# castacks/mvs_gi

Measured on AMD Instinct MI355X. Metric: stereo frames/sec/GPU (G16V, 3-cam, D=16) + inv-dist L1 vs reference, higher is better.
Workload: dtype f16x3 (split-fp16 MFMA operands: 11 + 11 significant bits, f32 accumulate/activations)

## Files before the change

### include/mvsgi.h

```cpp
#ifndef MVSGI_H
#define MVSGI_H

#include <stddef.h>
#include <stdint.h>

#ifdef __cplusplus
extern "C" {
#endif

#define MVSGI_ABI_VERSION 8

typedef void* mvsgi_stream_t;

#define MVSGI_CONV_AUTO   0
#define MVSGI_CONV_DIRECT 1
#define MVSGI_CONV_MFMA   2
#define MVSGI_CONV_BF16X3 3
#define MVSGI_CONV_BF16X3_C16 4
#define MVSGI_CONV_BF16X3_V32 5
#define MVSGI_CONV_BF16X3_D32 6

#define MVSGI_CONV_F16 0x100

#define MVSGI_SPLIT_F16 1
// ... 69 lines not shown
size_t mvsgi_conv2d_packed_weight_bytes_bf16x3(int Cout, int Cin);
int mvsgi_conv2d_pack_weights_bf16x3(const float* w_oihw, void* w_packed, int Cout, int Cin,
                                     mvsgi_stream_t stream);
int mvsgi_conv2d_f32(const float* x, const float* w_oihw, const void* w_packed,
                     const float* scale, const float* shift, const float* res, float* y,
                     int B, int Cin, int Hin, int Win, int Cout, int ksize, int stride,
                     float neg_slope, int impl, int in_nchw, mvsgi_stream_t stream);
const char* mvsgi_conv2d_variant_f32(int Cin, int Cout, int ksize, int stride, int impl, int in_nchw);

int mvsgi_resize_trilinear_f32(const float* x, float* y, int B, int C,
                               int Di, int Hi, int Wi, int Do, int Ho, int Wo,
                               mvsgi_stream_t stream);

int mvsgi_softargmin_f32(const float* costs, const float* inv_idx, float* inv_dist,
                         float* norm_costs, int B, int D, int H, int W, int scale,
                         mvsgi_stream_t stream);

int mvsgi_softargmin_div_f32(const float* costs, const float* inv_idx, float* inv_dist,
                             float* norm_costs, int B, int D, int H, int W, int scale,
                             float post_div, mvsgi_stream_t stream);

#define MVSGI_SA_AUTO  0
#define MVSGI_SA_PIXEL 1
#define MVSGI_SA_BAND  2
int mvsgi_softargmin_scaled_f32(const float* costs, const float* inv_idx, float* inv_dist,
                                float* norm_costs, int B, int D, int H, int W, double scale,
                                int OH, int OW, float post_div, int variant, mvsgi_stream_t stream);

int mvsgi_confidence_f32(const float* costs, const float* inv_idx, float* max_prob, float* entropy,
                         float* spread, int* argmax, int B, int D, int H, int W, double scale,
                         int OH, int OW, float post_div, int normalize_entropy, mvsgi_stream_t stream);

int mvsgi_ncv_to_nvc_f32(const float* x, float* y, int B, int C, long long V, mvsgi_stream_t stream);
int mvsgi_nvc_to_ncv_f32(const float* x, float* y, int B, int C, long long V, mvsgi_stream_t stream);

int mvsgi_resblock2d_f32(const float* x, const void* w_packed1, const float* scale1, const float* shift1,
                         const void* w_packed2, const float* scale2, const float* shift2, float* y,
                         int N, int H, int W, float neg_slope, mvsgi_stream_t stream);

size_t mvsgi_split2d_bytes(int N, int H, int W);
int mvsgi_f32_to_split2d(const float* x, void* y_split, int N, int H, int W, mvsgi_stream_t stream);
int mvsgi_split2d_to_f32(const void* x_split, float* y, int N, int H, int W, mvsgi_stream_t stream);
size_t mvsgi_resblock2d_split_packed_weight_bytes(void);
int mvsgi_resblock2d_split_pack_weights(const float* w_oihw, const float* scale, void* w_packed, mvsgi_stream_t stream);
int mvsgi_resblock2d_split(const void* x_split, const void* w_packed1, const float* shift1,
                           const void* w_packed2, const float* shift2, void* y, int y_is_split,
                           int N, int H, int W, float neg_slope, mvsgi_stream_t stream);
int mvsgi_conv2d_s2_split(const void* x_split, const void* w_packed, const float* shift, void* y_split,
                          int N, int H, int W, float neg_slope, mvsgi_stream_t stream);
int mvsgi_conv2d_f32_out_split2d(const float* x, const float* w_oihw, const void* w_packed,
                                 const float* scale, const float* shift, const float* res, void* y_split,
                                 int B, int Cin, int Hin, int Win, int Cout, int ksize, int stride,
                                 float neg_slope, int impl, int in_nchw, mvsgi_stream_t stream);

int mvsgi_rays_panorama_f32(const float* dist, float* rays, int N, int H, int W,
                            float lat0, float lat1, float lon0, float lon1, mvsgi_stream_t stream);
int mvsgi_transform_points_f32(const float* T , const float* points, float* out,
                               int B, long long M, mvsgi_stream_t stream);
int mvsgi_grid_double_sphere_f32(const float* points, float* grid, unsigned char* mask, int B, long long M,
                                 float xi, float alpha, float fx, float fy, float cx, float cy,
                                 int calib_h, int calib_w, float w2, mvsgi_stream_t stream);
int mvsgi_grid_equirect_f32(const float* points, float* grid, int B, long long M, mvsgi_stream_t stream);
int mvsgi_rays_equirect_surrogate_f32(float* rays, int H, int W, mvsgi_stream_t stream);

int mvsgi_resample_bilinear_u8_f32(const unsigned char* imgs, const float* grid, const unsigned char* valid, float* out,
                                   long long M, int T, int Hr, int Wr, int H, int W, float invalid_value, mvsgi_stream_t stream);
int mvsgi_resample_bilinear_f32(const float* imgs, const float* grid, const unsigned char* valid, float* out, long long M, int T,
                                int C, int Hr, int Wr, int H, int W, float invalid_value, mvsgi_stream_t stream);
int mvsgi_resample_validity_u8(const float* grid, const unsigned char* ds_mask, unsigned char* valid, long long n,
                               mvsgi_stream_t stream);
int mvsgi_resample_u8_table_f32(float* table256);

int mvsgi_reproject_f32(const float* inv, const float* rays, const void* imgs, int img_kind, const float* T_host,
                        const float* cams_host, float* xyz, float* warped, unsigned char* valid, float* grid,
                        long long B, int N, int C, int Hr, int Wr, int H, int W, float bf, float invalid_value,
                        mvsgi_stream_t stream);

int mvsgi_deform_conv2d_pack_weights_f32(const float* w_oihw, float* w_packed, int Cout, int Cin, int Kh, int Kw,
                                         mvsgi_stream_t stream);
int mvsgi_deform_conv2d_f32(const float* x, const float* offset, int offset_per_image, const float* w_packed,
                            const float* scale, const float* shift, const float* res, float* y,
                            int N, int Cin, int H, int W, int Cout, int Kh, int Kw, int stride_h, int stride_w,
                            int pad_h, int pad_w, int dil_h, int dil_w, float neg_slope, mvsgi_stream_t stream);

int mvsgi_sweep_std_nhwc_valid_split(const float* feats, const float* grids, const unsigned char* vmask,
                                     void* vol_split, int B, int N, int C, int Hi, int Wi, int D, int Ho, int Wo,
                                     int rig_batch, mvsgi_stream_t stream);

int mvsgi_conv3d_f32_out_split(const float* x, const float* w_packed_b3, const float* scale, const float* shift,
                               const float* res, void* y_split, int B, int Cin, int Din, int Hin, int Win, int Cout,
                               int stride, float neg_slope, mvsgi_stream_t stream);
int mvsgi_conv3d_rs16_split(const void* x_split, const void* w_packed_rs, const float* scale, const float* shift, float* y,
                            int B, int D, int H, int W, float neg_slope, mvsgi_stream_t stream);
int mvsgi_conv3d_rs16_split_out_split(const void* x_split, const void* w_packed_rs, const float* scale, const float* shift,
                                      void* y_split, int B, int D, int H, int W, float neg_slope, mvsgi_stream_t stream);
size_t mvsgi_conv3d_s2rs_packed_weight_bytes(void);
int mvsgi_conv3d_s2rs_pack_weights(const float* w_oidhw, const float* scale, void* w_packed, mvsgi_stream_t stream);
int mvsgi_conv3d_s2rs(const void* x_split, const void* w_packed, const float* shift, void* y_split,
                      int B, int D, int H, int W, float neg_slope, mvsgi_stream_t stream);
size_t mvsgi_conv3d_rs_packed_weight_bytes(int Cout, int Cin);
int mvsgi_conv3d_rs_pack_weights(const float* w_oidhw, void* w_packed, int Cout, int Cin, mvsgi_stream_t stream);
size_t mvsgi_act_split_bytes(int B, int C, int D, int H, int W);
int mvsgi_act_f32_to_split(const float* x, void* y_split, int B, int C, int D, int H, int W, mvsgi_stream_t stream);
int mvsgi_act_split_to_f32(const void* x_split, float* y, int B, int C, int D, int H, int W, mvsgi_stream_t stream);
int mvsgi_conv3d_rs_split(const void* x_split, const void* w_packed_rs, const float* scale, const float* shift,
                          const void* res_split, void* y, int y_is_f32, int B, int Cin, int D, int H, int W, int Cout,
                          float neg_slope, mvsgi_stream_t stream);

int mvsgi_conv3d_up2_f32_out_split(const float* x, const void* w_packed, int w_layout, const float* scale, const float* shift,
                                   const float* res, void* y_split, int B, int Cin, int Dl, int Hl, int Wl, int Cout,
                                   float neg_slope, mvsgi_stream_t stream);
int mvsgi_conv3d_up2_poly_split(const void* x_split, const void* plan_dev, const float* scale, const float* shift, void* y_split,
                                int B, int D, int H, int W, float neg_slope, mvsgi_stream_t stream);
size_t mvsgi_conv3d_head_split_packed_weight_bytes(int Cin);
int mvsgi_conv3d_head_split_pack_weights(const float* w_oidhw, void* w_packed, int Cin, mvsgi_stream_t stream);
int mvsgi_conv3d_head_split(const void* x_split, const void* w_packed, float scale, float shift, float* y, int B, int Cin,
                            int D, int H, int W, float neg_slope, mvsgi_stream_t stream);
int mvsgi_conv3d_head_split_pack_weights_f16(const float* w_oidhw, void* w_packed, int Cin, mvsgi_stream_t stream);
int mvsgi_conv3d_head_split_f16(const void* x_split, const void* w_packed, float scale, float shift, float* y, int B, int Cin,
                            int D, int H, int W, float neg_slope, mvsgi_stream_t stream);
int mvsgi_conv3d_up2_poly_rec32(const void* x_split, const void* plan_dev, const float* scale, const float* shift, void* y_rec32,
                                int B, int D, int H, int W, float neg_slope, mvsgi_stream_t stream);
int mvsgi_conv3d_head_rec32_f16(const void* x_rec32, const void* w_packed, float scale, float shift, float* y, int B, int Cin,
                                int D, int H, int W, float neg_slope, mvsgi_stream_t stream);
size_t mvsgi_conv3d_up2_poly_plan_bytes(int D, int H, int W);
int mvsgi_conv3d_up2_poly_plan(const float* w_oidhw_host, void* plan_host, int D, int H, int W);
int mvsgi_conv3d_up2_poly_f32(const void* x_split, const void* plan_dev, const float* scale, const float* shift, float* y,
                              int B, int D, int H, int W, float neg_slope, mvsgi_stream_t stream);

int mvsgi_act_f32_to_split_fmt(const float* x, void* y_split, int B, int C, int D, int H, int W, int fmt, mvsgi_stream_t stream);
int mvsgi_act_split_to_f32_fmt(const void* x_split, float* y, int B, int C, int D, int H, int W, int fmt, mvsgi_stream_t stream);
int mvsgi_sweep_std_nhwc_valid_split_fmt(const float* feats, const float* grids, const unsigned char* vmask, void* vol_split,
                                         int B, int N, int C, int Hi, int Wi, int D, int Ho, int Wo, int rig_batch, int fmt,
                                         mvsgi_stream_t stream);
int mvsgi_conv3d_f32_out_split_fmt(const float* x, const float* w_packed_b3, const float* scale, const float* shift,
                                   const float* res, void* y_split, int B, int Cin, int Din, int Hin, int Win, int Cout,
                                   int stride, float neg_slope, int fmt, mvsgi_stream_t stream);
int mvsgi_conv3d_rs_pack_weights_fmt(const float* w_oidhw, void* w_packed, int Cout, int Cin, int fmt, mvsgi_stream_t stream);
int mvsgi_conv3d_rs_split_fmt(const void* x_split, const void* w_packed_rs, const float* scale, const float* shift,
                              const void* res_split, void* y, int y_is_f32, int B, int Cin, int D, int H, int W, int Cout,
                              float neg_slope, int fmt, mvsgi_stream_t stream);
int mvsgi_conv3d_rs16_split_fmt(const void* x_split, const void* w_packed_rs, const float* scale, const float* shift, void* y,
                                int y_is_split, int B, int D, int H, int W, float neg_slope, int fmt, mvsgi_stream_t stream);
int mvsgi_conv3d_s2rs_pack_weights_fmt(const float* w_oidhw, const float* scale, void* w_packed, int fmt, mvsgi_stream_t stream);
int mvsgi_conv3d_s2rs_fmt(const void* x_split, const void* w_packed, const float* shift, void* y_split, int B, int D, int H, int W,
                          float neg_slope, float unscale, int fmt, mvsgi_stream_t stream);
int mvsgi_conv3d_s2rs_out_fmt(const void* x_split, const void* w_packed, const float* shift, void* y_split, int B, int D, int H, int W,
                              float neg_slope, float unscale, int fmt, int y_f32p, mvsgi_stream_t stream);
int mvsgi_conv3d_up2_poly_plan_fmt(const float* w_oidhw_host, void* plan_host, int D, int H, int W, int fmt);
int mvsgi_conv3d_up2_poly_fmt(const void* x_split, const void* plan_dev, const float* scale, const float* shift, void* y,
                              int y_is_split, int B, int D, int H, int W, float neg_slope, int fmt, mvsgi_stream_t stream);
int mvsgi_conv3d_up2_poly_wino_pays(int B, int D, int H, int W);

size_t mvsgi_conv3d_wino32_packed_weight_bytes(void);
int mvsgi_conv3d_wino32_applies(int Cin, int Cout, int D, int H, int W, int stride, float neg_slope);
int mvsgi_conv3d_wino32_pack_weights(const float* w_oidhw, void* w_packed, float* unscale, mvsgi_stream_t stream);
int mvsgi_conv3d_wino32_f16(const void* x_split, const void* w_packed, const float* scale, const float* shift, const void* res_split,
                            void* y, int y_is_f32, int act_f32p, int B, int D, int H, int W, float neg_slope, mvsgi_stream_t stream);

size_t mvsgi_instance_norm_ws_bytes(int B, int S, int C);
int mvsgi_instance_norm_f32(const float* x, const float* res, const float* gamma, const float* beta, float* y, float* ws,
                            int B, int S, int C, float eps, float neg_slope, mvsgi_stream_t stream);

#define MVSGI_METRICS_MASK_NONE   0
#define MVSGI_METRICS_MASK_TENSOR 1
#define MVSGI_METRICS_MASK_RANGE  2
#define MVSGI_METRICS_RANGE_FRAME 0
#define MVSGI_METRICS_RANGE_BATCH 1
size_t mvsgi_metrics_ws_bytes(int B, int H, int W);
int mvsgi_metrics_f32(const float* preds, const float* target, const unsigned char* mask, int mask_kind, float lo, float hi,
                      float bf, float cmin, float cmax, float thresh, float thresh_dist, int range_scope, void* ws,
                      size_t ws_bytes, double* out, int B, int H, int W, mvsgi_stream_t stream);

#define MVSGI_LOSSES_P_NONE       0
#define MVSGI_LOSSES_P_GIVEN      1
#define MVSGI_LOSSES_P_FUSED      2
#define MVSGI_LOSSES_VOL_NONE     0
#define MVSGI_LOSSES_VOL_PIXEL    1
#define MVSGI_LOSSES_VOL_VOLUME   2
#define MVSGI_LOSSES_PX_NONE      0
#define MVSGI_LOSSES_PX_TENSOR    1
#define MVSGI_LOSSES_PX_LABEL_MAX 2
size_t mvsgi_losses_ws_bytes(int B, int OH, int OW);
int mvsgi_losses_f32(const float* labels, const float* pred, const float* probs, int p_kind, const float* inv_list,
                     const unsigned char* vol_mask, int vol_kind, const unsigned char* px_mask, int px_kind, float label_max,
                     int inbounds, float near_inv, float far_inv, float* true_cost, void* ws, size_t ws_bytes, double* out,
                     int B, int D, int H, int W, double scale, int OH, int OW, mvsgi_stream_t stream);

size_t mvsgi_cloud_ws_bytes(long long B, int H, int W);
int mvsgi_cloud_pack_f32(const float* inv, const float* rays, const unsigned char* mask, int mask_per_frame,
                         const float* const* gates_host, const float* gate_lo_host, const float* gate_hi_host, int n_gates,
                         const float* warped, const unsigned char* valid, int N, int C, int require_colour, float no_colour,
                         const float* const* attrs_host, int A, float* points, int* counts, int* index, long long capacity,
                         void* ws, size_t ws_bytes, long long B, int H, int W, int sy, int sx, float bf, float d_min, float d_max,
                         mvsgi_stream_t stream);

size_t mvsgi_photo_ws_bytes(long long B, int H, int W);
int mvsgi_photo_consistency_f32(const float* inv, const float* rays, const void* imgs, int img_kind, const float* cam_masks,
                                const float* T_host, const float* cams_host, const unsigned char* mask, int mask_per_frame,
                                float thresh, unsigned char* n_views, float* photo_var, float* photo_std, float* mean_colour,
                                void* ws, size_t ws_bytes, double* table, long long B, int N, int C, int Hr, int Wr, int H, int W,
                                float bf, mvsgi_stream_t stream);
int mvsgi_photo_consistency_seen_f32(const float* inv, const float* rays, const void* imgs, int img_kind, const float* cam_masks,
                                     const float* T_host, const float* cams_host, const unsigned char* mask, int mask_per_frame,
                                     float thresh, unsigned char* n_views, float* photo_var, float* photo_std, float* mean_colour,
                                     void* ws, size_t ws_bytes, double* table, long long B, int N, int C, int Hr, int Wr, int H, int W,
                                     float bf, const unsigned char* cam_seen, mvsgi_stream_t stream);

int mvsgi_camera_range_f32(const float* inv, const float* rays, const float* T_host, const float* cams_host, const unsigned char* mask,
                           int mask_per_frame, int footprint, float* z2, long long B, int N, int H, int W, int Hz, int Wz, float bf,
                           mvsgi_stream_t stream);
int mvsgi_visibility_f32(const float* inv, const float* rays, const float* T_host, const float* cams_host, const float* z2, float k2,
                         unsigned char* visible, unsigned char* n_visible, float* range, long long B, int N, int H, int W, int Hz,
                         int Wz, float bf, mvsgi_stream_t stream);

int mvsgi_temporal_splat_f32(const float* prev_inv, const unsigned char* prev_age, const float* rays, const float* T,
                             unsigned long long* zkey, long long B, int H, int W, float bf, float au, float bu, float av, float bv,
                             int wrap, mvsgi_stream_t stream);
int mvsgi_temporal_fuse_f32(const unsigned long long* zkey, const float* prev_inv, const float* prev_var,
                            const unsigned char* prev_age, const float* cur_inv, const float* cur_std, float meas_std, float* fused,
                            float* var, unsigned char* age, float* warped_inv, float* warped_var, int* src, long long B, int H, int W,
                            float bf, float gate2, float q_var, mvsgi_stream_t stream);

int mvsgi_tsdf_integrate_f32(float* vol, const float* inv, const float* std, const unsigned char* mask, const float* T,
                             const int* origin, const int* origin_prev, float* range, long long B, int Nx, int Ny, int Nz, int H,
                             int W, float vs, float trunc, float t2, float w_max, float r_min, float r_max, float bf, float au,
                             float bu, float av, float bv, int wrap, mvsgi_stream_t stream);
int mvsgi_tsdf_raycast_f32(const float* vol, const float* rays, const float* P, const int* origin, float* inv, float* weight,
                           int* steps, long long B, int Nx, int Ny, int Nz, int H, int W, float inv_vs, float t0, float step, int K,
                           float w_min, float bf, mvsgi_stream_t stream);

#ifdef __cplusplus
}
#endif
#endif
```

### mvs_gi_amd/_lib.py

```python
from __future__ import annotations

import ctypes
import os
from ctypes import c_char_p, c_double, c_float, c_int, c_longlong, c_size_t, c_void_p

_HERE = os.path.dirname(os.path.abspath(__file__))
LIB_PATH = os.environ.get("MVSGI_LIB", os.path.join(_HERE, "libmvsgi_hip.so"))

ABI_VERSION = 8


class MvsgiLibraryMissing(RuntimeError):
    pass


_P = c_void_p
SIGNATURES = {
    "mvsgi_abi_version": (c_int, []),
    "mvsgi_last_error": (c_char_p, []),
    "mvsgi_saturation_flags": (c_int, [c_int, _P]),
    "mvsgi_saturation_words": (c_int, [_P]),
    "mvsgi_sweep_max_cams": (c_int, []),
    "mvsgi_sweep_std_f32": (c_int, [_P, _P, _P, c_int, _P, _P] + [c_int] * 10 + [_P]),
    "mvsgi_sweep_cat_f32": (c_int, [_P, _P, _P] + [c_int] * 8 + [_P]),
    "mvsgi_sweep_std_nhwc_f32": (c_int, [_P, _P, _P, c_int, _P, _P] + [c_int] * 10 + [_P]),
    "mvsgi_sweep_cat_nhwc_f32": (c_int, [_P, _P, _P] + [c_int] * 8 + [_P]),
    "mvsgi_sweep_validity_u8": (c_int, [_P, _P, c_int, _P, _P] + [c_int] * 7 + [_P]),
    "mvsgi_sweep_std_nhwc_valid_f32": (c_int, [_P, _P, _P, _P] + [c_int] * 8 + [_P]),
    "mvsgi_sweep_std_nhwc_valid_split": (c_int, [_P, _P, _P, _P] + [c_int] * 9 + [_P]),
    "mvsgi_sweep_std_nhwc_valid_rig_f32": (c_int, [_P, _P, _P, _P] + [c_int] * 8 + [_P]),
    "mvsgi_conv3d_packed_weight_floats": (c_size_t, [c_int, c_int]),
    "mvsgi_conv3d_pack_weights_f32": (c_int, [_P, _P, c_int, c_int, _P]),
    "mvsgi_conv3d_packed_weight_bytes_bf16x3": (c_size_t, [c_int, c_int]),
    "mvsgi_conv3d_pack_weights_bf16x3": (c_int, [_P, _P, c_int, c_int, _P]),
    "mvsgi_conv3d_pack_weights_split": (c_int, [_P, _P, c_int, c_int, c_int, _P]),
    "mvsgi_conv3d_f32": (c_int, [_P] * 7 + [c_int] * 7 + [c_float, c_int, _P]),
    "mvsgi_conv3d_variant_f32": (c_char_p, [c_int] * 8),
    "mvsgi_conv3d_up2_f32": (c_int, [_P, _P, c_int] + [_P] * 4 + [c_int] * 6 + [c_float, _P]),
    "mvsgi_conv3d_up2_variant_f32": (c_char_p, [c_int] * 7),
    "mvsgi_conv3d_v32_applies": (c_int, [c_int] * 7),
    "mvsgi_conv3d_d32_applies": (c_int, [c_int] * 7),
    "mvsgi_conv3d_up2_d32_applies": (c_int, [c_int] * 6),
    "mvsgi_conv3d_packed_weight_bytes_bf16x3_v32": (c_size_t, [c_int, c_int]),
    "mvsgi_conv3d_pack_weights_bf16x3_v32": (c_int, [_P, _P, c_int, c_int, _P]),
    "mvsgi_conv3d_packed_weight_bytes_bf16x3_c16": (c_size_t, [c_int]),
    "mvsgi_conv3d_pack_weights_bf16x3_c16": (c_int, [_P, _P, c_int, _P]),
    "mvsgi_conv2d_stem_packed_weight_bytes": (c_size_t, []),
    "mvsgi_conv2d_stem_pack_weights": (c_int, [_P, _P, _P]),
    "mvsgi_conv2d_packed_weight_floats": (c_size_t, [c_int, c_int]),
    "mvsgi_conv2d_pack_weights_f32": (c_int, [_P, _P, c_int, c_int, _P]),
    "mvsgi_conv2d_packed_weight_bytes_bf16x3": (c_size_t, [c_int, c_int]),
    "mvsgi_conv2d_pack_weights_bf16x3": (c_int, [_P, _P, c_int, c_int, _P]),
    "mvsgi_conv2d_f32": (c_int, [_P] * 7 + [c_int] * 7 + [c_float, c_int, c_int, _P]),
    "mvsgi_conv2d_variant_f32": (c_char_p, [c_int] * 6),
    "mvsgi_resblock2d_f32": (c_int, [_P] * 8 + [c_int] * 3 + [c_float, _P]),
    "mvsgi_split2d_bytes": (c_size_t, [c_int] * 3),
    "mvsgi_f32_to_split2d": (c_int, [_P, _P] + [c_int] * 3 + [_P]),
    "mvsgi_split2d_to_f32": (c_int, [_P, _P] + [c_int] * 3 + [_P]),
    "mvsgi_resblock2d_split_packed_weight_bytes": (c_size_t, []),
    "mvsgi_resblock2d_split_pack_weights": (c_int, [_P, _P, _P, _P]),
    "mvsgi_resblock2d_split": (c_int, [_P] * 6 + [c_int] * 4 + [c_float, _P]),
    "mvsgi_conv2d_s2_split": (c_int, [_P] * 4 + [c_int] * 3 + [c_float, _P]),
    "mvsgi_conv2d_f32_out_split2d": (c_int, [_P] * 7 + [c_int] * 7 + [c_float, c_int, c_int, _P]),
    "mvsgi_resize_trilinear_f32": (c_int, [_P, _P] + [c_int] * 8 + [_P]),
    "mvsgi_softargmin_f32": (c_int, [_P, _P, _P, _P] + [c_int] * 5 + [_P]),
    "mvsgi_softargmin_div_f32": (c_int, [_P, _P, _P, _P] + [c_int] * 5 + [c_float, _P]),
    "mvsgi_softargmin_scaled_f32": (c_int, [_P, _P, _P, _P] + [c_int] * 4 + [c_double, c_int, c_int, c_float, c_int, _P]),
    "mvsgi_confidence_f32": (c_int, [_P] * 6 + [c_int] * 4 + [c_double, c_int, c_int, c_float, c_int, _P]),
    "mvsgi_rays_panorama_f32": (c_int, [_P, _P, c_int, c_int, c_int] + [c_float] * 4 + [_P]),
    "mvsgi_transform_points_f32": (c_int, [_P, _P, _P, c_int, c_longlong, _P]),
    "mvsgi_grid_double_sphere_f32": (c_int, [_P, _P, _P, c_int, c_longlong] + [c_float] * 6 + [c_int, c_int, c_float, _P]),
    "mvsgi_grid_equirect_f32": (c_int, [_P, _P, c_int, c_longlong, _P]),
    "mvsgi_rays_equirect_surrogate_f32": (c_int, [_P, c_int, c_int, _P]),
    "mvsgi_resample_bilinear_u8_f32": (c_int, [_P, _P, _P, _P, c_longlong] + [c_int] * 5 + [c_float, _P]),
    "mvsgi_resample_bilinear_f32": (c_int, [_P, _P, _P, _P, c_longlong] + [c_int] * 6 + [c_float, _P]),
    "mvsgi_resample_validity_u8": (c_int, [_P, _P, _P, c_longlong, _P]),
    "mvsgi_resample_u8_table_f32": (c_int, [_P]),
    "mvsgi_reproject_f32": (c_int, [_P, _P, _P, c_int] + [_P] * 6 + [c_longlong] + [c_int] * 6 + [c_float, c_float, _P]),
    "mvsgi_deform_conv2d_pack_weights_f32": (c_int, [_P, _P] + [c_int] * 4 + [_P]),
    "mvsgi_deform_conv2d_f32": (c_int, [_P, _P, c_int] + [_P] * 5 + [c_int] * 13 + [c_float, _P]),
    "mvsgi_act_split_bytes": (c_size_t, [c_int] * 5),
    "mvsgi_act_f32_to_split": (c_int, [_P, _P] + [c_int] * 5 + [_P]),
    "mvsgi_act_split_to_f32": (c_int, [_P, _P] + [c_int] * 5 + [_P]),
    "mvsgi_conv3d_f32_out_split": (c_int, [_P] * 6 + [c_int] * 7 + [c_float, _P]),
    "mvsgi_conv3d_rs16_split": (c_int, [_P] * 5 + [c_int] * 4 + [c_float, _P]),
    "mvsgi_conv3d_rs16_split_out_split": (c_int, [_P] * 5 + [c_int] * 4 + [c_float, _P]),
    "mvsgi_conv3d_s2rs_packed_weight_bytes": (c_size_t, []),
    "mvsgi_conv3d_s2rs_pack_weights": (c_int, [_P, _P, _P, _P]),
    "mvsgi_conv3d_s2rs": (c_int, [_P] * 4 + [c_int] * 4 + [c_float, _P]),
    "mvsgi_conv3d_rs_packed_weight_bytes": (c_size_t, [c_int, c_int]),
    "mvsgi_conv3d_rs_pack_weights": (c_int, [_P, _P, c_int, c_int, _P]),
    "mvsgi_conv3d_rs_split": (c_int, [_P] * 6 + [c_int] * 7 + [c_float, _P]),
    "mvsgi_conv3d_up2_f32_out_split": (c_int, [_P, _P, c_int] + [_P] * 4 + [c_int] * 6 + [c_float, _P]),
    "mvsgi_conv3d_up2_poly_split": (c_int, [_P] * 5 + [c_int] * 4 + [c_float, _P]),
    "mvsgi_conv3d_head_split_packed_weight_bytes": (c_size_t, [c_int]),
    "mvsgi_conv3d_head_split_pack_weights": (c_int, [_P, _P, c_int, _P]),
    "mvsgi_conv3d_head_split": (c_int, [_P, _P, c_float, c_float, _P] + [c_int] * 5 + [c_float, _P]),
    "mvsgi_conv3d_head_split_pack_weights_f16": (c_int, [_P, _P, c_int, _P]),
    "mvsgi_conv3d_head_split_f16": (c_int, [_P, _P, c_float, c_float, _P] + [c_int] * 5 + [c_float, _P]),
    "mvsgi_conv3d_head_rec32_f16": (c_int, [_P, _P, c_float, c_float, _P] + [c_int] * 5 + [c_float, _P]),
    "mvsgi_conv3d_up2_poly_rec32": (c_int, [_P] * 5 + [c_int] * 4 + [c_float, _P]),
    "mvsgi_conv3d_up2_poly_plan_bytes": (c_size_t, [c_int] * 3),
    "mvsgi_conv3d_up2_poly_plan": (c_int, [_P, _P] + [c_int] * 3),
    "mvsgi_conv3d_up2_poly_f32": (c_int, [_P] * 5 + [c_int] * 4 + [c_float, _P]),
    "mvsgi_act_f32_to_split_fmt": (c_int, [_P, _P] + [c_int] * 6 + [_P]),
    "mvsgi_act_split_to_f32_fmt": (c_int, [_P, _P] + [c_int] * 6 + [_P]),
    "mvsgi_sweep_std_nhwc_valid_split_fmt": (c_int, [_P, _P, _P, _P] + [c_int] * 10 + [_P]),
    "mvsgi_conv3d_f32_out_split_fmt": (c_int, [_P] * 6 + [c_int] * 7 + [c_float, c_int, _P]),
    "mvsgi_conv3d_rs_pack_weights_fmt": (c_int, [_P, _P, c_int, c_int, c_int, _P]),
    "mvsgi_conv3d_rs_split_fmt": (c_int, [_P] * 6 + [c_int] * 7 + [c_float, c_int, _P]),
    "mvsgi_conv3d_rs16_split_fmt": (c_int, [_P] * 5 + [c_int] * 5 + [c_float, c_int, _P]),
    "mvsgi_conv3d_s2rs_pack_weights_fmt": (c_int, [_P, _P, _P, c_int, _P]),
    "mvsgi_conv3d_s2rs_fmt": (c_int, [_P] * 4 + [c_int] * 4 + [c_float, c_float, c_int, _P]),
    "mvsgi_conv3d_s2rs_out_fmt": (c_int, [_P] * 4 + [c_int] * 4 + [c_float, c_float, c_int, c_int, _P]),
    "mvsgi_conv3d_up2_poly_plan_fmt": (c_int, [_P, _P] + [c_int] * 4),
    "mvsgi_conv3d_wino32_packed_weight_bytes": (c_size_t, []),
    "mvsgi_conv3d_wino32_applies": (c_int, [c_int] * 6 + [c_float]),
    "mvsgi_conv3d_wino32_pack_weights": (c_int, [_P] * 4),
    "mvsgi_conv3d_wino32_f16": (c_int, [_P] * 6 + [c_int] * 6 + [c_float, _P]),
    "mvsgi_conv3d_up2_poly_fmt": (c_int, [_P] * 5 + [c_int] * 5 + [c_float, c_int, _P]),
    "mvsgi_conv3d_up2_poly_wino_pays": (c_int, [c_int] * 4),
    "mvsgi_ncv_to_nvc_f32": (c_int, [_P, _P, c_int, c_int, c_longlong, _P]),
    "mvsgi_nvc_to_ncv_f32": (c_int, [_P, _P, c_int, c_int, c_longlong, _P]),
    "mvsgi_instance_norm_ws_bytes": (c_size_t, [c_int] * 3),
    "mvsgi_instance_norm_f32": (c_int, [_P] * 6 + [c_int] * 3 + [c_float, c_float, _P]),
    "mvsgi_metrics_ws_bytes": (c_size_t, [c_int] * 3),
    "mvsgi_metrics_f32": (c_int, [_P, _P, _P, c_int] + [c_float] * 7 + [c_int, _P, c_size_t, _P] + [c_int] * 3 + [_P]),
    "mvsgi_losses_ws_bytes": (c_size_t, [c_int] * 3),
    "mvsgi_losses_f32": (c_int, [_P, _P, _P, c_int, _P, _P, c_int, _P, c_int, c_float, c_int, c_float, c_float, _P, _P, c_size_t, _P] +
                         [c_int] * 4 + [c_double, c_int, c_int, _P]),
    "mvsgi_cloud_ws_bytes": (c_size_t, [c_longlong, c_int, c_int]),
    "mvsgi_cloud_pack_f32": (c_int, [_P, _P, _P, c_int, _P, _P, _P, c_int, _P, _P, c_int, c_int, c_int, c_float, _P, c_int, _P, _P, _P,
                                     c_longlong, _P, c_size_t, c_longlong] + [c_int] * 4 + [c_float] * 3 + [_P]),
    "mvsgi_photo_ws_bytes": (c_size_t, [c_longlong, c_int, c_int]),
    "mvsgi_photo_consistency_f32": (c_int, [_P, _P, _P, c_int, _P, _P, _P, _P, c_int, c_float, _P, _P, _P, _P, _P, c_size_t, _P,
                                            c_longlong] + [c_int] * 6 + [c_float, _P]),
    "mvsgi_photo_consistency_seen_f32": (c_int, [_P, _P, _P, c_int, _P, _P, _P, _P, c_int, c_float, _P, _P, _P, _P, _P, c_size_t, _P,
                                                 c_longlong] + [c_int] * 6 + [c_float, _P, _P]),
    "mvsgi_camera_range_f32": (c_int, [_P] * 5 + [c_int, c_int, _P, c_longlong] + [c_int] * 5 + [c_float, _P]),
    "mvsgi_visibility_f32": (c_int, [_P] * 5 + [c_float, _P, _P, _P, c_longlong] + [c_int] * 5 + [c_float, _P]),
    "mvsgi_temporal_splat_f32": (c_int, [_P] * 5 + [c_longlong, c_int, c_int] + [c_float] * 5 + [c_int, _P]),
    "mvsgi_temporal_fuse_f32": (c_int, [_P] * 6 + [c_float] + [_P] * 6 + [c_longlong, c_int, c_int] + [c_float] * 3 + [_P]),
    "mvsgi_tsdf_integrate_f32": (c_int, [_P] * 8 + [c_longlong] + [c_int] * 5 + [c_float] * 11 + [c_int, _P]),
    "mvsgi_tsdf_raycast_f32": (c_int, [_P] * 7 + [c_longlong] + [c_int] * 5 + [c_float] * 3 + [c_int, c_float, c_float, _P]),
}

_lib = None


def load() -> ctypes.CDLL:
    global _lib
    if _lib is not None:
        return _lib
    if not os.path.isfile(LIB_PATH):
        raise MvsgiLibraryMissing(
            f"{LIB_PATH} not found: build the HIP library first (__graft_entry__.build()). "
            "mvs_gi_amd has no CPU fallback.")
    import torch
    lib = ctypes.CDLL(LIB_PATH)
    try:
        lib.mvsgi_abi_version.restype = c_int
        lib.mvsgi_abi_version.argtypes = []
        got = lib.mvsgi_abi_version()
    except AttributeError as e:
        raise MvsgiLibraryMissing(f"{LIB_PATH}: not a libmvsgi_hip ({e}); rebuild it (__graft_entry__.build())") from None
    if got != ABI_VERSION:
        raise MvsgiLibraryMissing(f"{LIB_PATH}: ABI version {got}, expected {ABI_VERSION}; rebuild it (__graft_entry__.build())")
    for name, (res, args) in SIGNATURES.items():
        try:
            fn = getattr(lib, name)
        except AttributeError:
            raise MvsgiLibraryMissing(f"{LIB_PATH}: symbol {name} missing although the ABI version matches; rebuild it "
                                      "(__graft_entry__.build())") from None
        fn.restype = res
        fn.argtypes = args
    lib.mvsgi_saturation_flags(0, None)
    _lib = lib
    return lib


def check(status: int, what: str) -> None:
    if status != 0:
        msg = load().mvsgi_last_error()
        raise RuntimeError(f"{what}: {msg.decode() if msg else 'unknown error'}")
```

### mvs_gi_amd/csrc/common.hpp

```cpp
#pragma once
#include <hip/hip_runtime.h>

#include <cstdarg>
#include <cstdio>
#include <cstdlib>
#include <cstring>
#include <string>

#include "../../include/mvsgi.h"

namespace mvsgi {

std::string& last_error_ref();

inline int fail(const char* fmt, ...) {
    char buf[512];
    va_list ap;
    va_start(ap, fmt);
    vsnprintf(buf, sizeof(buf), fmt, ap);
    va_end(ap);
    last_error_ref() = buf;
    return 1;
}

inline int check_launch(const char* what) {
    hipError_t e = hipGetLastError();
    if (e != hipSuccess) return fail("%s: launch failed: %s", what, hipGetErrorString(e));
    return 0;
}

#define MVSGI_REQUIRE(cond, ...)                      \
    do {                                              \
        if (!(cond)) return ::mvsgi::fail(__VA_ARGS__); \
    } while (0)

constexpr int kSatWords = 8;
unsigned* sat_words();
#define MVSGI_SAT_WORDS(VAR)                                                            \
    unsigned* VAR = ::mvsgi::sat_words();                                               \
    MVSGI_REQUIRE(VAR != nullptr, "cannot allocate the range report's pinned host words")

inline hipStream_t as_stream(mvsgi_stream_t s) { return reinterpret_cast<hipStream_t>(s); }

inline long long cdiv(long long a, long long b) { return (a + b - 1) / b; }

inline bool aligned(const void* p, unsigned a) { return (reinterpret_cast<uintptr_t>(p) & (a - 1)) == 0; }

constexpr int kMaxCams = 8;

constexpr int kMaxDevices = 32;
struct PersistentGeom {
    int wgs_per_cu;
    int cus;
};
template <class K>
inline int persistent_geometry(K kern, int threads, size_t lds_bytes, int max_wgs_per_cu,
                               PersistentGeom (&cache)[kMaxDevices], const char* what, PersistentGeom& out) {
    int dev = 0;
    hipError_t e = hipGetDevice(&dev);
    if (e != hipSuccess) return fail("%s: hipGetDevice: %s", what, hipGetErrorString(e));
    if (dev < 0 || dev >= kMaxDevices) return fail("%s: device ordinal %d not supported (max %d)", what, dev, kMaxDevices);
    PersistentGeom g = cache[dev];
    if (!g.wgs_per_cu) {
        e = hipFuncSetAttribute(reinterpret_cast<const void*>(kern), hipFuncAttributeMaxDynamicSharedMemorySize,
                                (int)lds_bytes);
        if (e != hipSuccess) return fail("%s: hipFuncSetAttribute: %s", what, hipGetErrorString(e));
        int occ = 0;
        e = hipOccupancyMaxActiveBlocksPerMultiprocessor(&occ, kern, threads, lds_bytes);
        if (e != hipSuccess || occ < 1) occ = 1;
        int cus = 0;
        e = hipDeviceGetAttribute(&cus, hipDeviceAttributeMultiprocessorCount, dev);
        if (e != hipSuccess || cus < 1) return fail("%s: cannot read the device's CU count", what);
        g.wgs_per_cu = occ > max_wgs_per_cu ? max_wgs_per_cu : occ;
        g.cus = cus;
        cache[dev] = g;
    }
    out = g;
    return 0;
}
inline unsigned persistent_grid(const PersistentGeom& geo, long long nb) {
    long long resident = ((long long)geo.cus * geo.wgs_per_cu) / 8 * 8;
    if (resident < 8) resident = 8;
    return (unsigned)(nb <= resident ? nb : resident);
}
template <class K, class A>
inline int launch_persistent(K kern, int threads, size_t lds_bytes, int max_wgs_per_cu, PersistentGeom (&cache)[kMaxDevices],
                             const char* what, long long nb, hipStream_t st, const A& args) {
    PersistentGeom geo;
    if (persistent_geometry(kern, threads, lds_bytes, max_wgs_per_cu, cache, what, geo)) return 1;
    hipLaunchKernelGGL(kern, dim3(persistent_grid(geo, nb)), dim3((unsigned)threads), lds_bytes, st, args);
    return check_launch(what);
}

inline int device_cus() {
    static int cache[kMaxDevices] = {};
    int dev = 0;
    if (hipGetDevice(&dev) != hipSuccess || dev < 0 || dev >= kMaxDevices) return 256;
    if (!cache[dev]) {
        int cus = 0;
        if (hipDeviceGetAttribute(&cus, hipDeviceAttributeMultiprocessorCount, dev) != hipSuccess || cus < 1) cus = 256;
        cache[dev] = cus;
    }
    return cache[dev];
}

constexpr size_t kRs32PackedBytes = (size_t)2 * 2 * 14 * 2 * 64 * 16;
void rs32_pack_weights_host(const float* w_oidhw_32x32x27, void* packed, bool f16);
int rs32_up2_launch(const void* x_split, const void* w_sets, const float* scale32, const float* shift32, void* y, int y_is_split,
                    int B, int D, int H, int W, float neg_slope, bool f16, hipStream_t st);

constexpr size_t kWinoUp2RoleBytes = (size_t)4 * 4 * 3 * 2 * 2 * 64 * 16;
void wino_up2_pack_role(const float* w32_oidhw, unsigned short* wp, float* unscale32);
bool wino_up2_applies(int D, int H, int W);
int wino_up2_launch(const void* x_split, const void* w_roles, const float* unw, const float* scale16, const float* shift16, void* y_split,
                    int B, int D, int H, int W, float neg_slope, bool out_f32, hipStream_t st);

}
```

### mvs_gi_amd/csrc/conv3d.hip

```cpp
#include "common.hpp"
#include "conv_common.hpp"
#include "conv3d_variants.hpp"
#ifdef MVSGI_STAMPS
#include <cstdio>
#include <cstdlib>
#endif

namespace {

__global__ void pack_head_weights_kernel(const float* __restrict__ w, float* __restrict__ wp, int Cin) {
    const int idx = blockIdx.x * 256 + threadIdx.x;
    if (idx >= 27 * Cin) return;
    const int tap = idx / Cin, ci = idx % Cin;
    wp[idx] = w[ci * 27 + tap];
}

#include "conv3d_f32mfma.hpp"
#include "conv3d_bf16x3.hpp"


__global__ __launch_bounds__(256) void conv3d_head_kernel(ConvArgs a, int dchunk, int nd) {
    constexpr int TH = 8, TW = 32, ITH = TH + 2, ITW = TW + 2, PV = ITH * ITW;
    constexpr int NT = (PV + 31) / 32;
    constexpr int TPW = (NT + 3) / 4;
// ... 528 lines not shown
extern "C" int mvsgi_conv3d_d32_applies(int B, int Cin, int Din, int Hin, int Win, int Cout, int stride) {
    ConvArgs a{};
    static const float dummy = 0.f;
    if (fill_args(a, &dummy, &dummy, &dummy, &dummy, &dummy, nullptr, nullptr, B, Cin, Din, Hin, Win, Cout, stride, 1.f))
        return 0;
    return d32_variant(a) != V_COUNT ? 1 : 0;
}

extern "C" int mvsgi_conv3d_v32_applies(int B, int Cin, int Din, int Hin, int Win, int Cout, int stride) {
    ConvArgs a{};
    static const float dummy = 0.f;
    if (fill_args(a, &dummy, &dummy, &dummy, &dummy, &dummy, nullptr, nullptr, B, Cin, Din, Hin, Win, Cout, stride, 1.f))
        return 0;
    return v32_applies(a) ? 1 : 0;
}

extern "C" size_t mvsgi_conv3d_packed_weight_bytes_bf16x3_c16(int Cin) { return (size_t)(Cin / 16) * 5 * 3 * 2 * 64 * 16; }

extern "C" int mvsgi_conv3d_pack_weights_bf16x3_c16(const float* w_oidhw, void* w_packed, int Cin, mvsgi_stream_t stream) {
    MVSGI_REQUIRE(w_oidhw && w_packed, "mvsgi_conv3d_pack_weights_bf16x3_c16: null pointer");
    MVSGI_REQUIRE(Cin > 0 && Cin % 16 == 0, "mvsgi_conv3d_pack_weights_bf16x3_c16: Cin=%d must be a positive multiple of 16", Cin);
    const int total = (Cin / 16) * 5 * 3 * 64;
    hipLaunchKernelGGL(pack_weights_bf16x3_c16_kernel, dim3((unsigned)mvsgi::cdiv(total, 256)), dim3(256), 0,
                       mvsgi::as_stream(stream), w_oidhw, reinterpret_cast<bf16x8*>(w_packed), Cin, false);
    return mvsgi::check_launch("mvsgi_conv3d_pack_weights_bf16x3_c16");
}

extern "C" int mvsgi_conv3d_pack_weights_f32(const float* w_oidhw, float* w_packed, int Cout, int Cin,
                                             mvsgi_stream_t stream) {
    MVSGI_REQUIRE(w_oidhw && w_packed, "mvsgi_conv3d_pack_weights_f32: null pointer");
    if (Cout == 1 && Cin > 0 && Cin % 16 == 0) {
        hipLaunchKernelGGL(pack_head_weights_kernel, dim3((unsigned)mvsgi::cdiv(27 * Cin, 256)), dim3(256), 0,
                           mvsgi::as_stream(stream), w_oidhw, w_packed, Cin);
        return mvsgi::check_launch("mvsgi_conv3d_pack_weights_f32");
    }
    MVSGI_REQUIRE(Cout > 0 && Cin > 0 && Cout % 16 == 0 && Cin % 16 == 0,
                  "mvsgi_conv3d_pack_weights_f32: Cout=%d Cin=%d must be positive multiples of 16 (or Cout == 1)",
                  Cout, Cin);
    const long long total = (long long)(Cin / 16) * 27 * (Cout / 16) * 64;
    hipLaunchKernelGGL(pack_weights_kernel, dim3((unsigned)mvsgi::cdiv(total, 256)), dim3(256), 0,
                       mvsgi::as_stream(stream), w_oidhw, reinterpret_cast<f32x4*>(w_packed), Cout, Cin, 27);
    return mvsgi::check_launch("mvsgi_conv3d_pack_weights_f32");
}

extern "C" int mvsgi_conv3d_f32(const float* x, const float* w_oidhw, const float* w_packed, const float* scale,
                                const float* shift, const float* res, float* y, int B, int Cin, int Din, int Hin,
                                int Win, int Cout, int stride, float neg_slope, int impl, mvsgi_stream_t stream) {
    MVSGI_REQUIRE(x && y && scale && shift, "mvsgi_conv3d_f32: null pointer");
    ConvArgs a{};
    if (fill_args(a, x, w_oidhw, w_packed, scale, shift, res, y, B, Cin, Din, Hin, Win, Cout, stride, neg_slope))
        return 1;
    if (split_flag(a, impl, "mvsgi_conv3d_f32")) return 1;
    const int v = select_variant(a, impl);
    if (v == V_COUNT) return 1;
    return launch_variant(v, a, mvsgi::as_stream(stream));
}

extern "C" int mvsgi_conv3d_f32_out_split_fmt(const float* x, const float* w_packed_b3, const float* scale, const float* shift,
                                              const float* res, void* y_split, int B, int Cin, int Din, int Hin, int Win, int Cout,
                                              int stride, float neg_slope, int fmt, mvsgi_stream_t stream) {
    MVSGI_REQUIRE(fmt == 0 || fmt == MVSGI_SPLIT_F16, "mvsgi_conv3d_f32_out_split: fmt %d not in {0, MVSGI_SPLIT_F16}", fmt);
    MVSGI_REQUIRE(x && y_split && scale && shift && w_packed_b3, "mvsgi_conv3d_f32_out_split: null pointer");
    MVSGI_REQUIRE(Cin % 16 == 0 && Cout % 16 == 0, "mvsgi_conv3d_f32_out_split: Cin, Cout must be multiples of 16");
    ConvArgs a{};
    if (fill_args(a, x, nullptr, w_packed_b3, scale, shift, res, reinterpret_cast<float*>(y_split), B, Cin, Din, Hin, Win, Cout,
                  stride, neg_slope))
        return 1;
    a.y_split = static_cast<unsigned char*>(y_split);
    a.f16 = fmt != 0;
    const int v = select_variant(a, MVSGI_CONV_BF16X3);
    if (v == V_COUNT) return 1;
    return launch_variant(v, a, mvsgi::as_stream(stream));
}
extern "C" int mvsgi_conv3d_f32_out_split(const float* x, const float* w_packed_b3, const float* scale, const float* shift,
                                          const float* res, void* y_split, int B, int Cin, int Din, int Hin, int Win, int Cout,
                                          int stride, float neg_slope, mvsgi_stream_t stream) {
    return mvsgi_conv3d_f32_out_split_fmt(x, w_packed_b3, scale, shift, res, y_split, B, Cin, Din, Hin, Win, Cout, stride, neg_slope, 0, stream);
}

extern "C" const char* mvsgi_conv3d_variant_f32(int B, int Cin, int Din, int Hin, int Win, int Cout, int stride,
                                                int impl) {
    ConvArgs a{};
    static const float dummy = 0.f;
    if (fill_args(a, &dummy, &dummy, &dummy, &dummy, &dummy, nullptr, nullptr, B, Cin, Din, Hin, Win, Cout, stride,
                  1.f))
        return nullptr;
    if (split_flag(a, impl, "mvsgi_conv3d_variant_f32")) return nullptr;
    const int v = select_variant(a, impl);
    return variant_name(v, a);
}

extern "C" int mvsgi_conv3d_up2_f32(const float* x, const void* w_packed, int w_layout, const float* scale,
                                    const float* shift, const float* res, float* y, int B, int Cin, int Dl, int Hl,
                                    int Wl, int Cout, float neg_slope, mvsgi_stream_t stream) {
    const bool f16 = (w_layout & MVSGI_CONV_F16) != 0;
    w_layout &= ~MVSGI_CONV_F16;
    MVSGI_REQUIRE(w_layout == MVSGI_CONV_BF16X3 || (w_layout == MVSGI_CONV_BF16X3_C16 && Cout == 16) ||
                      (w_layout == MVSGI_CONV_BF16X3_V32 && Cout % 32 == 0) || (w_layout == MVSGI_CONV_BF16X3_D32 && Cin % 32 == 0),
                  "mvsgi_conv3d_up2_f32: w_layout %d not valid for Cout %d", w_layout, Cout);
    MVSGI_REQUIRE(x && y && scale && shift && w_packed, "mvsgi_conv3d_up2_f32: null pointer");
    MVSGI_REQUIRE(Dl > 0 && Hl > 0 && Wl > 0 && Dl < (1 << 20) && Hl < (1 << 20) && Wl < (1 << 20),
                  "mvsgi_conv3d_up2_f32: bad dims");
    ConvArgs a{};
    if (fill_args(a, x, nullptr, static_cast<const float*>(w_packed), scale, shift, res, y, B, Cin, 2 * Dl, 2 * Hl,
                  2 * Wl, Cout, 1, neg_slope))
        return 1;
    a.f16 = f16;
    const int v = select_variant_up2(a, w_layout);
    if (v == V_COUNT) return 1;
    return launch_variant(v, a, mvsgi::as_stream(stream));
}

extern "C" int mvsgi_conv3d_up2_f32_out_split(const float* x, const void* w_packed, int w_layout, const float* scale, const float* shift,
                                              const float* res, void* y_split, int B, int Cin, int Dl, int Hl, int Wl, int Cout,
                                              float neg_slope, mvsgi_stream_t stream) {
    const bool f16 = (w_layout & MVSGI_CONV_F16) != 0;
    w_layout &= ~MVSGI_CONV_F16;
    MVSGI_REQUIRE(w_layout == MVSGI_CONV_BF16X3 || (w_layout == MVSGI_CONV_BF16X3_C16 && Cout == 16),
                  "mvsgi_conv3d_up2_f32_out_split: w_layout %d not valid for Cout %d", w_layout, Cout);
    MVSGI_REQUIRE(x && y_split && scale && shift && w_packed, "mvsgi_conv3d_up2_f32_out_split: null pointer");
    MVSGI_REQUIRE(Dl > 0 && Hl > 0 && Wl > 0 && Dl < (1 << 20) && Hl < (1 << 20) && Wl < (1 << 20),
                  "mvsgi_conv3d_up2_f32_out_split: bad dims");
    ConvArgs a{};
    if (fill_args(a, x, nullptr, static_cast<const float*>(w_packed), scale, shift, res, reinterpret_cast<float*>(y_split), B, Cin,
                  2 * Dl, 2 * Hl, 2 * Wl, Cout, 1, neg_slope))
        return 1;
    a.y_split = static_cast<unsigned char*>(y_split);
    a.f16 = f16;
    const int v = select_variant_up2(a, w_layout);
    if (v == V_COUNT) return 1;
    return launch_variant(v, a, mvsgi::as_stream(stream));
}

extern "C" int mvsgi_conv3d_up2_d32_applies(int B, int Cin, int Dl, int Hl, int Wl, int Cout) {
    ConvArgs a{};
    static const float dummy = 0.f;
    if (Cin % 32 || Cout % 16 || Dl <= 0 || Hl <= 0 || Wl <= 0 ||
        fill_args(a, &dummy, nullptr, &dummy, &dummy, &dummy, nullptr, nullptr, B, Cin, 2 * Dl, 2 * Hl, 2 * Wl, Cout, 1, 1.f))
        return 0;
    const int base = select_variant_up2(a, MVSGI_CONV_BF16X3);
    return (base == B3U_N64 || base == B3U_N96) ? 1 : 0;
}

extern "C" const char* mvsgi_conv3d_up2_variant_f32(int B, int Cin, int Dl, int Hl, int Wl, int Cout, int w_layout) {
    ConvArgs a{};
    static const float dummy = 0.f;
    if (fill_args(a, &dummy, nullptr, &dummy, &dummy, &dummy, nullptr, nullptr, B, Cin, 2 * Dl, 2 * Hl, 2 * Wl, Cout, 1,
                  1.f))
        return nullptr;
    a.f16 = (w_layout & MVSGI_CONV_F16) != 0;
    const int v = select_variant_up2(a, w_layout & ~MVSGI_CONV_F16);
    return variant_name(v, a);
}
```

### mvs_gi_amd/csrc/conv3d_bf16x3.hpp

```cpp
#pragma once
#ifndef MVSGI_ABL
#define MVSGI_ABL 0
#endif

#include "split_fmt.hpp"

constexpr int kVSB = 80;

__device__ __forceinline__ void split_bf16x4(const f32x4 x, u32x2& hi, u32x2& lo) {
#pragma unroll
    for (int p = 0; p < 2; ++p) {
        const f32x2 v = {x[2 * p], x[2 * p + 1]};
        const unsigned hb = __builtin_bit_cast(unsigned, __builtin_convertvector(v, bf16x2));
        const f32x2 hf = {__builtin_bit_cast(float, hb << 16), __builtin_bit_cast(float, hb & 0xffff0000u)};
        hi[p] = hb;
        float r0 = v[0] - hf[0], r1 = v[1] - hf[1];
        asm volatile("" : "+v"(r0));
        asm volatile("" : "+v"(r1));
        lo[p] = __builtin_bit_cast(unsigned, __builtin_convertvector(f32x2{r0, r1}, bf16x2));
    }
}
__device__ __forceinline__ f32x4 fma4(const f32x4 a, const f32x4 b, const f32x4 c) {
    f32x4 r;
#pragma unroll
// ... 11 lines not shown
        const f16x2 h = __builtin_convertvector(v, f16x2);
        hi[p] = __builtin_bit_cast(unsigned, h);
        float r0 = v[0] - (float)h[0], r1 = v[1] - (float)h[1];
        asm volatile("" : "+v"(r0));
        asm volatile("" : "+v"(r1));
        lo[p] = __builtin_bit_cast(unsigned, __builtin_convertvector(f32x2{r0, r1}, f16x2));
    }
}
template <bool F16>
__device__ __forceinline__ void split_x4(const f32x4 x, u32x2& hi, u32x2& lo) {
    if constexpr (F16) split_f16x4(x, hi, lo); else split_bf16x4(x, hi, lo);
}
template <bool F16>
__device__ __forceinline__ void split_x4(const f32x4 x, u32x2& hi, u32x2& lo, float& satm) {
    if constexpr (F16) {
        const f32x4 c = {__builtin_amdgcn_fmed3f(x[0], -65504.f, 65504.f), __builtin_amdgcn_fmed3f(x[1], -65504.f, 65504.f),
                         __builtin_amdgcn_fmed3f(x[2], -65504.f, 65504.f), __builtin_amdgcn_fmed3f(x[3], -65504.f, 65504.f)};
        satm = sf_sat_acc(sf_sat_acc(satm, c[0], c[1]), c[2], c[3]);
        split_f16x4(c, hi, lo);
    } else split_bf16x4(x, hi, lo);
}
template <bool F16>
__device__ __forceinline__ f32x4 mfma16(const bf16x8 a, const bf16x8 b, const f32x4 c) {
    if constexpr (F16) return __builtin_amdgcn_mfma_f32_16x16x32_f16(__builtin_bit_cast(f16x8, a), __builtin_bit_cast(f16x8, b), c, 0, 0, 0);
    else return __builtin_amdgcn_mfma_f32_16x16x32_bf16(a, b, c, 0, 0, 0);
}
template <bool F16>
__device__ __forceinline__ f32x16 mfma32(const bf16x8 a, const bf16x8 b, const f32x16 c) {
    if constexpr (F16) return __builtin_amdgcn_mfma_f32_32x32x16_f16(__builtin_bit_cast(f16x8, a), __builtin_bit_cast(f16x8, b), c, 0, 0, 0);
    else return __builtin_amdgcn_mfma_f32_32x32x16_bf16(a, b, c, 0, 0, 0);
}
__device__ __forceinline__ void split_weight(float v, bool f16, unsigned short& hi, unsigned short& lo) {
    if (f16) {
        const _Float16 h = (_Float16)v;
        hi = __builtin_bit_cast(unsigned short, h);
        lo = __builtin_bit_cast(unsigned short, (_Float16)(v - (float)h));
    } else {
        const __bf16 h = (__bf16)v;
        hi = __builtin_bit_cast(unsigned short, h);
        lo = __builtin_bit_cast(unsigned short, (__bf16)(v - (float)h));
    }
}

constexpr int pairs_of(int kd) { return (kd * 9 + 1) / 2; }

__global__ void pack_weights_bf16x3_kernel(const float* __restrict__ w, bf16x8* __restrict__ wp, int Cout, int Cin,
                                           int taps, bool f16 = false) {
    const int kPairs = (taps + 1) / 2;
    const int CT = Cout / 16;
    const long long total = (long long)(Cin / 16) * kPairs * CT * 64;
    const long long idx = (long long)blockIdx.x * 256 + threadIdx.x;
    if (idx >= total) return;
    const int lane = (int)(idx & 63);
    long long r = idx >> 6;
    const int ct = (int)(r % CT);
    r /= CT;
    const int p = (int)(r % kPairs);
    const int cc = (int)(r / kPairs);
    const int kg = lane >> 4;
    const int co = ct * 16 + (lane & 15);
    const int ci = cc * 16 + (kg >> 1) * 8;
    const int tap = 2 * p + (kg & 1);
    u16x8 hi, lo;
    for (int j = 0; j < 8; ++j) {
        const float v = tap < taps ? w[((long long)co * Cin + ci + j) * taps + tap] : 0.f;
        unsigned short h_, l_;
        split_weight(v, f16, h_, l_);
        hi[j] = h_;
        lo[j] = l_;
    }
    const long long o = ((((long long)cc * CT + ct) * kPairs + p) * 2) * 64 + lane;
    wp[o] = __builtin_bit_cast(bf16x8, hi);
    wp[o + 64] = __builtin_bit_cast(bf16x8, lo);
}

__global__ void pack_weights_bf16x3_d32_kernel(const float* __restrict__ w, bf16x8* __restrict__ wp, int Cout, int Cin, bool f16 = false) {
    const int CT = Cout / 16;
    const long long total = (long long)(Cin / 32) * CT * 27 * 64;
    const long long idx = (long long)blockIdx.x * 256 + threadIdx.x;
    if (idx >= total) return;
    const int lane = (int)(idx & 63);
    long long r = idx >> 6;
    const int tap = (int)(r % 27);
    r /= 27;
    const int ct = (int)(r % CT);
    const int cc = (int)(r / CT);
    const int kg = lane >> 4;
    const int co = ct * 16 + (lane & 15);
    const int ci = (2 * cc + (kg & 1)) * 16 + (kg >> 1) * 8;
    u16x8 hi, lo;
    for (int j = 0; j < 8; ++j) {
        unsigned short h_, l_;
        split_weight(w[((long long)co * Cin + ci + j) * 27 + tap], f16, h_, l_);
        hi[j] = h_;
        lo[j] = l_;
    }
    const long long o = ((((long long)cc * CT + ct) * 27 + tap) * 2) * 64 + lane;
    wp[o] = __builtin_bit_cast(bf16x8, hi);
    wp[o + 64] = __builtin_bit_cast(bf16x8, lo);
}

__global__ void pack_weights_bf16x3_c16_kernel(const float* __restrict__ w, bf16x8* __restrict__ wp, int Cin, bool f16 = false) {
    const int total = (Cin / 16) * 5 * 3 * 64;
    const int idx = blockIdx.x * 256 + threadIdx.x;
    if (idx >= total) return;
    const int lane = idx & 63;
    int r = idx >> 6;
    const int kd = r % 3;
    r /= 3;
    const int p = r % 5;
    const int cc = r / 5;
    const int kg = lane >> 4, co = lane & 15;
    const int ci = cc * 16 + (kg >> 1) * 8;
    const int t2 = 2 * p + (kg & 1);
    u16x8 hi, lo;
    for (int j = 0; j < 8; ++j) {
        const float v = t2 < 9 ? w[((long long)co * Cin + ci + j) * 27 + kd * 9 + t2] : 0.f;
        unsigned short h_, l_;
        split_weight(v, f16, h_, l_);
        hi[j] = h_;
        lo[j] = l_;
    }
    const long long o = ((long long)((cc * 5 + p) * 3 + kd) * 2) * 64 + lane;
    wp[o] = __builtin_bit_cast(bf16x8, hi);
    wp[o + 64] = __builtin_bit_cast(bf16x8, lo);
}

__global__ void pack_weights_bf16x3_v32_kernel(const float* __restrict__ w, bf16x8* __restrict__ wp, int Cout, int Cin, bool f16 = false) {
    const int CT = Cout / 32;
    const long long total = (long long)(Cin / 16) * CT * 27 * 64;
    const long long idx = (long long)blockIdx.x * 256 + threadIdx.x;
    if (idx >= total) return;
    const int lane = (int)(idx & 63);
    long long r = idx >> 6;
    const int tap = (int)(r % 27);
    r /= 27;
    const int ct = (int)(r % CT);
    const int cc = (int)(r / CT);
    const int co = ct * 32 + (lane & 31);
    const int ci = cc * 16 + (lane >> 5) * 8;
    u16x8 hi, lo;
    for (int j = 0; j < 8; ++j) {
        const float v = w[((long long)co * Cin + ci + j) * 27 + tap];
        unsigned short h_, l_;
        split_weight(v, f16, h_, l_);
        hi[j] = h_;
        lo[j] = l_;
    }
    const long long o = ((((long long)cc * CT + ct) * 27 + tap) * 2) * 64 + lane;
    wp[o] = __builtin_bit_cast(bf16x8, hi);
    wp[o + 64] = __builtin_bit_cast(bf16x8, lo);
}

template <int NW, int MW, int WM, int WN, int TD, int TH, int TW, int S, int KD, bool UPS, bool PLANE, bool V32, bool WLDS, bool F16, bool D32 = false, int DK = 3, int BRD = 0>
__device__ __forceinline__ void conv3d_x3_body(const ConvArgs& a) {
    static_assert(!WLDS || (WN == 1 && KD == 3 && !UPS && !PLANE && !V32 && S == 1 && NW == 1 && MW <= 2), "LDS-staged weights: one shared cout tile, one or two voxel tiles per wave");
    static_assert(!V32 || (S == 1 && KD == 3 && TW == 16 && TH % 2 == 0 && !PLANE), "32x32x16 schedule: stride 1, 16-wide even bricks");
    static_assert(!PLANE || (NW == 1 && WN == 1 && WM == 4 && TH == 4 && MW == TD && TW == 16 && S == 1 && KD == 3),
                  "plane schedule: Cout == 16, 4 h-rows x TD planes x 16 w per brick");
    static_assert(!UPS || (S == 1 && KD == 3 && TD % 2 == 0 && TH % 2 == 0 && TW % 2 == 0),
                  "fused upsample: stride 1, even bricks (halo bricks are whole 2x2x2 cells)");
    static_assert(WM * WN == 4, "4 consumer waves per workgroup");
    static_assert(WM * MW * (V32 ? 32 : 16) == TD * TH * TW, "brick must be covered by the voxel tiles");
    static_assert(KD == 3 || (KD == 1 && TD == 1), "2-D bricks are one plane thick");
    constexpr int SD = KD == 1 ? 1 : S;
    static_assert(!D32 || (KD == 3 && S == 1 && !PLANE && !V32 && !WLDS), "32-channel slices: stride-1 3x3x3 variants (plain or fused upsample) only");
    static_assert(DK == 3 || (D32 && DK >= 1 && (TD == 1 ? DK <= 2 : (TD == 2 && WM == 2 && MW * 16 == TH * TW))), "depth skip: one- or two-plane bricks whose waves own whole planes");
    constexpr bool DKU = D32 && TD == 1 && DK == 2;
    constexpr int kTaps = KD * 9, kPairs = D32 ? 9 * DK : pairs_of(KD);
    constexpr int kWBlk = D32 ? 27 : kPairs;
    constexpr int ITD = (TD - 1) * SD + KD, ITH = (TH - 1) * S + 3, ITW = (TW - 1) * S + 3;
    constexpr int IV = ITD * ITH * ITW;
    constexpr int QB = D32 ? 3 : 2;
    constexpr int NIT = (IV * (1 << QB) + 255) / 256;
    constexpr int ROWP = V32 ? ((ITW * kVSB + 255) / 256) * 256 : ITW * kVSB;
    constexpr int SUB = ITD * ITH * ROWP;
    constexpr int BUF = D32 ? 2 * SUB : SUB;
    constexpr int WB = WLDS ? (MW * NW == 1 ? 8 : 4) :
                       (KD == 3 && !PLANE && !V32 && MW * NW == 1) ? 16 : (KD == 3 && !PLANE && !V32 && MW * NW == 2) ? 8 :
                       (KD == 3 && !PLANE && !V32 && NW == 2 && MW == 4) ? 5 :
                       NW <= 2 ? 4 : 2;
    constexpr int LA = WB - 1;
    constexpr int NSLOT = ((kPairs + WB - 1) / WB) * WB;
    static_assert(NSLOT % WB == 0 && NSLOT >= kPairs, "pipeline geometry");
    constexpr bool RPRE = MW * NW <= 8;
#ifndef MVSGI_WARM
#define MVSGI_WARM 0
#endif
    constexpr bool WARM = MVSGI_WARM && KD == 3 && !UPS && !PLANE && !V32 && !WLDS && S == 1 && MW * NW <= 2;

    constexpr int WBYTES = WLDS ? NW * kPairs * 2048 : 0;
    constexpr int BUFW = BUF + WBYTES;
    constexpr int WARM_LDS = 2 * BUFW;
    extern __shared__ __attribute__((aligned(16))) unsigned char ldsb[];
    float satm = 0.f;

    const int tid = threadIdx.x, lane = tid & 63;
    const int wave = __builtin_amdgcn_readfirstlane(tid >> 6);
    const bool producer = wave >= 4;
    const int CT = a.Cout / (V32 ? 32 : 16);
    const int ny = (CT + WN * NW - 1) / (WN * NW);
    const int nchunks = a.Cin / (D32 ? 32 : 16);
    const int total = a.total_units;
    const int G = gridDim.x;
    const int nmine = (total - (int)blockIdx.x + G - 1) / G;
    const int U = nmine * nchunks;
#ifdef MVSGI_STAMPS
    int nst = 0;
#define STAMP()                                                                                     \
    if (a.dbg && blockIdx.x == 8 && nst < 120) {                                                    \
        unsigned long long t_;                                                                      \
        asm volatile("s_memtime %0\n\ts_waitcnt lgkmcnt(0)" : "=s"(t_)::"memory");                  \
        if (lane == 0) a.dbg[wave * 128 + nst] = t_;                                                \
        nst++;                                                                                      \
    }
#else
#define STAMP()
#endif
    STAMP()

#define MVSGI_DECODE_DH(T, OD, OH, B) { OD = (T % a.tiles_d) * TD + a.od_off; T /= a.tiles_d; OH = (T % a.tiles_h) * TH; B = T / a.tiles_h; }
#define MVSGI_DECODE(ID, CB, B, OD, OH, OW)                       \
    {                                                             \
        int t_ = xcd_remap((ID), total);                          \
        CB = t_ % ny;                                             \
        t_ /= ny;                                                 \
        OW = (t_ % a.tiles_w) * TW;                               \
        t_ /= a.tiles_w;                                          \
        MVSGI_DECODE_DH(t_, OD, OH, B)                            \
    }

    if (producer) {
        const int ptid = tid - 256;
        if constexpr (UPS) {
            constexpr int CD = ITD / 2, CH = ITH / 2, CW = ITW / 2, NC = CD * CH * CW;
            constexpr int NCQ = NC << QB;
            constexpr int NITU = (NCQ + 255) / 256;
            constexpr int RF = NCQ / 256, REM = NCQ - RF * 256;
            constexpr bool HALF = REM > 0 && 2 * REM <= 256;
#define MVSGI_UPS_CQ(IT) ((HALF && (IT) == RF) ? RF * 256 + (ptid >> 1) : ptid + (IT) * 256)
#define MVSGI_UPS_LIVE(IT) ((HALF && (IT) == RF) ? (ptid >> 1) < REM : ptid + (IT) * 256 < NCQ)
            const int Dl = a.Din >> 1, Hl = a.Hin >> 1, Wl = a.Win >> 1;
            const int sH_ = Wl * a.Cin, sD_ = Hl * sH_;
            int lo_d[NITU], lo_h[NITU], lo_w[NITU];
            unsigned inmask[NITU];
            const float* xb = a.x;
            f32x4 crA[NITU][8], crB[NITU][8];
            unsigned imA[NITU], imB[NITU];
#define MVSGI_PLAN_UPS(UNIT)                                                                            \
            {                                                                                           \
                int cb_, b_, od_, oh_, ow_;                                                             \
                MVSGI_DECODE(UNIT, cb_, b_, od_, oh_, ow_)                                              \
                (void)cb_;                                                                              \
                _Pragma("unroll") for (int it = 0; it < NITU; ++it) {                                   \
                    const int c = MVSGI_UPS_CQ(it) >> QB;                                               \
                    const int cw = c % CW, ch = (c / CW) % CH, cd = c / (CW * CH);                      \
                    const int gd = od_ - 1 + 2 * cd, gh = oh_ - 1 + 2 * ch, gw = ow_ - 1 + 2 * cw;      \
                    lo_d[it] = (gd - 1) >> 1;                                                           \
                    lo_h[it] = (gh - 1) >> 1;                                                           \
                    lo_w[it] = (gw - 1) >> 1;                                                           \
                    inmask[it] = (gd >= 0 && gd < a.Din ? 1u : 0u) | (gd + 1 < a.Din ? 2u : 0u) |       \
                                 (gh >= 0 && gh < a.Hin ? 4u : 0u) | (gh + 1 < a.Hin ? 8u : 0u) |       \
                                 (gw >= 0 && gw < a.Win ? 16u : 0u) | (gw + 1 < a.Win ? 32u : 0u);      \
                }                                                                                       \
                xb = a.x + (long long)b_ * Dl * Hl * Wl * a.Cin;                                        \
            }
#define MVSGI_CLAMP(V, N) ((V) < 0 ? 0 : ((V) > (N) - 1 ? (N) - 1 : (V)))
            int k2 = 0, cc2 = 0;
#define MVSGI_ISSUE_UPS_BEGIN()                                                                         \
            if (cc2 == 0 && k2 > 0) { MVSGI_PLAN_UPS((int)blockIdx.x + k2 * G) }
#define MVSGI_ISSUE_UPS1(CR, IM, IT)                                                                    \
            {                                                                                           \
                const int q = MVSGI_UPS_CQ(IT) & ((1 << QB) - 1);                                       \
                const bool live = MVSGI_UPS_LIVE(IT);                                                   \
                const int d0 = live ? MVSGI_CLAMP(lo_d[IT], Dl) : 0, d1 = live ? MVSGI_CLAMP(lo_d[IT] + 1, Dl) : 0; \
                const int h0 = live ? MVSGI_CLAMP(lo_h[IT], Hl) : 0, h1 = live ? MVSGI_CLAMP(lo_h[IT] + 1, Hl) : 0; \
                const int w0 = live ? MVSGI_CLAMP(lo_w[IT], Wl) : 0, w1 = live ? MVSGI_CLAMP(lo_w[IT] + 1, Wl) : 0; \
                const int cofs = cc2 * (D32 ? 32 : 16) + q * 4;                                         \
                 \
                const int od_[2] = {__mul24(d0, sD_), __mul24(d1, sD_)}, oh_[2] = {__mul24(h0, sH_), __mul24(h1, sH_)};   \
                const int ow_[2] = {__mul24(w0, a.Cin) + cofs, __mul24(w1, a.Cin) + cofs};              \
                _Pragma("unroll") for (int k = 0; k < 8; ++k)                                           \
                    CR[IT][k] = *reinterpret_cast<const f32x4*>(xb + (od_[(k >> 2) & 1] + oh_[(k >> 1) & 1] + ow_[k & 1])); \
                IM[IT] = inmask[IT];                                                                    \
            }
#define MVSGI_ISSUE_UPS_END()                                                                           \
            {                                                                                           \
                if (++cc2 == nchunks) { cc2 = 0; ++k2; }                                                \
                if (k2 >= nmine) { k2 = nmine - 1; cc2 = nchunks - 1; }                                 \
            }
#define MVSGI_ISSUE_UPS(CR, IM)                                                                         \
            {                                                                                           \
                MVSGI_ISSUE_UPS_BEGIN()                                                                 \
                _Pragma("unroll") for (int it = 0; it < NITU; ++it) MVSGI_ISSUE_UPS1(CR, IM, it)        \
                MVSGI_ISSUE_UPS_END()                                                                   \
            }
#define MVSGI_LERP2(A, B, O0, O1)    \
            {                                                                                           \
                const f32x4 d_ = fma4((A), f32x4{-1.f, -1.f, -1.f, -1.f}, (B));    \
                O0 = fma4(d_, f32x4{0.25f, 0.25f, 0.25f, 0.25f}, (A));             \
                O1 = fma4(d_, f32x4{0.75f, 0.75f, 0.75f, 0.75f}, (A));             \
            }
#define MVSGI_PUT_UPS1(CR, IM, DST, IT)                                                                 \
            if (HALF && (IT) == RF) {                                                                   \
                 \
                if (MVSGI_UPS_LIVE(IT)) {                                                               \
                    const int cq_ = MVSGI_UPS_CQ(IT), c = cq_ >> QB, q = cq_ & 3, kd = ptid & 1;        \
                    const int sub_ = D32 ? ((cq_ >> 2) & 1) * SUB : 0;                                  \
                    const int cw = c % CW, ch = (c / CW) % CH, cd = c / (CW * CH);                      \
                    const float f_ = kd ? 0.75f : 0.25f;                                                \
                    const f32x4 f4_ = {f_, f_, f_, f_};                                                 \
                    f32x4 xd[2][2], xh[2][2], xo[2][2];                                                 \
                    _Pragma("unroll") for (int j = 0; j < 4; ++j) {                                     \
                        const f32x4 d_ = fma4(CR[IT][j], f32x4{-1.f, -1.f, -1.f, -1.f}, CR[IT][4 + j]); \
                        xd[j >> 1][j & 1] = fma4(d_, f4_, CR[IT][j]);              \
                    }                                                                                   \
                    _Pragma("unroll") for (int kw = 0; kw < 2; ++kw)                                    \
                        MVSGI_LERP2(xd[0][kw], xd[1][kw], xh[0][kw], xh[1][kw])                         \
                    _Pragma("unroll") for (int kh = 0; kh < 2; ++kh)                                    \
                        MVSGI_LERP2(xh[kh][0], xh[kh][1], xo[kh][0], xo[kh][1])                         \
                    _Pragma("unroll") for (int kh = 0; kh < 2; ++kh)                                    \
                        _Pragma("unroll") for (int kw = 0; kw < 2; ++kw) {                              \
                            const bool ok = ((IM[IT] >> kd) & (IM[IT] >> (2 + kh)) & (IM[IT] >> (4 + kw)) & 1u) != 0; \
                            u32x2 hi, lo;                                                               \
                            split_x4<F16>(xo[kh][kw], hi, lo, satm);                                           \
                            if (!ok) hi = lo = u32x2{0u, 0u};                                           \
                            const int vo_ = ((2 * cd + kd) * ITH + 2 * ch + kh) * ROWP + (2 * cw + kw) * kVSB; \
                            *reinterpret_cast<u32x2*>((DST) + sub_ + vo_ + q * 8) = hi;                 \
                            *reinterpret_cast<u32x2*>((DST) + sub_ + vo_ + 32 + q * 8) = lo;            \
                        }                                                                               \
                }                                                                                       \
            } else {                                                                                    \
                const int e = ptid + (IT) * 256;                                                        \
                if (e < NCQ) {                                                                          \
                    const int c = e >> QB, q = e & 3, sub_ = D32 ? ((e >> 2) & 1) * SUB : 0;            \
                    const int cw = c % CW, ch = (c / CW) % CH, cd = c / (CW * CH);                      \
                     \
                    f32x4 xw[4][2], xh[2][2][2], xo[2][2][2];                                           \
                    _Pragma("unroll") for (int k = 0; k < 4; ++k)                                       \
                        MVSGI_LERP2(CR[IT][2 * k], CR[IT][2 * k + 1], xw[k][0], xw[k][1])               \
                    _Pragma("unroll") for (int kd = 0; kd < 2; ++kd)                                    \
                        _Pragma("unroll") for (int kw = 0; kw < 2; ++kw)                                \
                            MVSGI_LERP2(xw[2 * kd][kw], xw[2 * kd + 1][kw], xh[kd][0][kw], xh[kd][1][kw]) \
                    _Pragma("unroll") for (int kh = 0; kh < 2; ++kh)                                    \
                        _Pragma("unroll") for (int kw = 0; kw < 2; ++kw)                                \
                            MVSGI_LERP2(xh[0][kh][kw], xh[1][kh][kw], xo[0][kh][kw], xo[1][kh][kw])      \
                    _Pragma("unroll") for (int kd = 0; kd < 2; ++kd)                                    \
                        _Pragma("unroll") for (int kh = 0; kh < 2; ++kh)                                \
                            _Pragma("unroll") for (int kw = 0; kw < 2; ++kw) {                          \
                                const bool ok = ((IM[IT] >> kd) & (IM[IT] >> (2 + kh)) & (IM[IT] >> (4 + kw)) & 1u) != 0; \
                                u32x2 hi, lo;                                                           \
                                split_x4<F16>(xo[kd][kh][kw], hi, lo, satm);                                   \
                                if (!ok) hi = lo = u32x2{0u, 0u};                                       \
                                const int vo_ = ((2 * cd + kd) * ITH + 2 * ch + kh) * ROWP + (2 * cw + kw) * kVSB; \
                                *reinterpret_cast<u32x2*>((DST) + sub_ + vo_ + q * 8) = hi;             \
                                *reinterpret_cast<u32x2*>((DST) + sub_ + vo_ + 32 + q * 8) = lo;        \
                            }                                                                           \
                }                                                                                       \
            }
#define MVSGI_PUT_UPS(CR, IM, DST)                                                                      \
            { _Pragma("unroll") for (int it = 0; it < NITU; ++it) MVSGI_PUT_UPS1(CR, IM, DST, it) }
#define MVSGI_STEP_UPS(NEW, IMNEW, OLD, IMOLD, DST, DOPUT)                                              \
            {                                                                                           \
                MVSGI_ISSUE_UPS_BEGIN()                                                                 \
                _Pragma("unroll") for (int it = 0; it < NITU; ++it) {                                   \
                    MVSGI_ISSUE_UPS1(NEW, IMNEW, it)                                                    \
                    if (DOPUT) MVSGI_PUT_UPS1(OLD, IMOLD, DST, it)                                      \
                    __builtin_amdgcn_sched_barrier(0);                                                  \
                }                                                                                       \
                MVSGI_ISSUE_UPS_END()                                                                   \
            }
            STAMP()
            MVSGI_PLAN_UPS((int)blockIdx.x)
            MVSGI_ISSUE_UPS(crA, imA)
            MVSGI_PUT_UPS(crA, imA, ldsb)
            MVSGI_ISSUE_UPS(crA, imA)
            STAMP()
            __syncthreads();
            STAMP()
            for (int u = 0; u < U; u += 2) {
                MVSGI_STEP_UPS(crB, imB, crA, imA, ldsb + ((u + 1) & 1) * BUF, u + 1 < U)
                STAMP()
// ... 210 lines not shown
        {                                                                                              \
            const int off_ = (((T) / 9) * ITH + ((T) / 3) % 3) * ROWP + ((T) % 3) * kVSB;              \
            _Pragma("unroll") for (int i = 0; i < MW; ++i) {                                           \
                xh[BUFI][i] = *reinterpret_cast<const bf16x8*>(img + xbase[i] + off_);                 \
                xl[BUFI][i] = *reinterpret_cast<const bf16x8*>(img + xbase[i] + off_ + 32);            \
            }                                                                                          \
        }
#define MVSGI_V_MFMAS(WBUFI, BUFI)                                                                          \
        _Pragma("unroll") for (int tr = 0; tr < 3; ++tr)                                               \
            _Pragma("unroll") for (int i = 0; i < MW; ++i)                                             \
                _Pragma("unroll") for (int j = 0; j < NW; ++j)                                         \
                    acc[i][j] = mfma32<F16>(tr == 0 ? wl[WBUFI][j] : wh[WBUFI][j], tr == 1 ? xl[BUFI][i] : xh[BUFI][i], acc[i][j]);
        int cb_, b_, od0, oh0, ow0;
        MVSGI_DECODE((int)blockIdx.x, cb_, b_, od0, oh0, ow0)
        MVSGI_CTILES(ctc, cb_)
        {
            unsigned l16 = lane16;
#pragma unroll
            for (int t0 = 0; t0 < LAW; ++t0) { MVSGI_V_LOADW(t0, 0, t0, ctc) }
        }
        STAMP()
        __syncthreads();
        STAMP()
        int k = 0, cc = 0;
        for (int u = 0; u < U; ++u) {
            const unsigned char* img = ldsb + (u & 1) * BUF;
            const bool last = cc + 1 == nchunks;
            const bool more = u + 1 < U;
            const int ncc = last ? 0 : cc + 1;
            int ncb = cb_, nb = b_, nod0 = od0, noh0 = oh0, now0 = ow0;
            if (last && more) {
                MVSGI_DECODE((int)blockIdx.x + (k + 1) * G, ncb, nb, nod0, noh0, now0)
                MVSGI_CTILES(ctn, ncb)
            } else {
#pragma unroll
                for (int j = 0; j < NW; ++j) ctn[j] = ctc[j];
            }
            int eoff[MW];
            f32x4 rres[MW][NW][4], esc[NW][4], esh[NW][4];
            if (last) {
#pragma unroll
                for (int j = 0; j < NW; ++j)
#pragma unroll
                    for (int g = 0; g < 4; ++g) {
                        esc[j][g] = *reinterpret_cast<const f32x4*>(a.scale + ctc[j] * 32 + 8 * g + 4 * kh2);
                        esh[j][g] = *reinterpret_cast<const f32x4*>(a.shift + ctc[j] * 32 + 8 * g + 4 * kh2);
                    }
#pragma unroll
                for (int i = 0; i < MW; ++i) {
                    const int od = od0 + tdv[i], oh = oh0 + thv[i], ow = ow0 + twv[i];
                    const bool inside = od < a.Do && oh < a.Ho && ow < a.Wo;
                    eoff[i] = inside ? ((od * a.Ho + oh) * a.Wo + ow) * a.Cout + kh2 * 4 : -1;
                }
            }
            MVSGI_V_READX(0, 0)
            if (XA == 2) { MVSGI_V_READX(1, 1) }
#pragma unroll
            for (int t_ = 0; t_ < 27; ++t_) {
                const int cur = t_ % VB, nx2 = (t_ + XA) % VB, wcur = t_ % VWB;
                unsigned l16 = lane16;
                asm volatile("" : "+v"(l16));
                if (t_ + LAW < 27) {
                    MVSGI_V_LOADW((t_ + LAW) % VWB, cc, t_ + LAW, ctc)
                } else {
                    MVSGI_V_LOADW((t_ + LAW - 27) % VWB, ncc, t_ + LAW - 27, ctn)
                }
                if (t_ + XA < 27) { MVSGI_V_READX(nx2, t_ + XA) }
                if (t_ == 26 && last && a.res) {
                    const float* rb = a.res + (long long)b_ * frame_elems;
#pragma unroll
                    for (int i = 0; i < MW; ++i)
#pragma unroll
                        for (int j = 0; j < NW; ++j)
#pragma unroll
                            for (int g = 0; g < 4; ++g)
                                rres[i][j][g] = *reinterpret_cast<const f32x4*>(rb + (eoff[i] >= 0 ? eoff[i] + ctc[j] * 32 + 8 * g : 0));
                }
                MVSGI_V_MFMAS(wcur, cur)
                if (t_ + XA < 27) {
                    constexpr int NMEM = 2 * NW + 2 * MW, NMFMA = 3 * MW * NW;
                    constexpr int RATIO = NMFMA / NMEM > 0 ? NMFMA / NMEM : 1;
#pragma unroll
                    for (int q_ = 0; q_ < NMEM; ++q_) {
                        __builtin_amdgcn_sched_group_barrier(0x008, RATIO, 0);
                        __builtin_amdgcn_sched_group_barrier(0x120, 1, 0);
                    }
                    __builtin_amdgcn_sched_group_barrier(0x008, NMFMA, 0);
                }
                __builtin_amdgcn_sched_barrier(0);
            }
            STAMP()
            if (last) {
                const int ct0 = (cb_ * WN + wn) * NW;
                float* yb = a.y + (long long)b_ * frame_elems;
#pragma unroll
                for (int i = 0; i < MW; ++i)
#pragma unroll
                    for (int j = 0; j < NW; ++j)
#pragma unroll
                        for (int g = 0; g < 4; ++g) {
                            f32x4 r = f32x4{acc[i][j][4 * g], acc[i][j][4 * g + 1], acc[i][j][4 * g + 2], acc[i][j][4 * g + 3]} * esc[j][g] + esh[j][g];
                            if (a.res) r += rres[i][j][g];
#pragma unroll
                            for (int e = 0; e < 4; ++e) {
                                r[e] = r[e] > 0.f ? r[e] : r[e] * a.neg_slope;
                                acc[i][j][4 * g + e] = 0.f;
                            }
                            if (eoff[i] >= 0 && ct0 + j < CT) *reinterpret_cast<f32x4*>(yb + eoff[i] + (ct0 + j) * 32 + 8 * g) = r;
                        }
                k += 1;
                cb_ = ncb; b_ = nb; od0 = nod0; oh0 = noh0; ow0 = now0;
#pragma unroll
                for (int j = 0; j < NW; ++j) ctc[j] = ctn[j];
            }
            cc = ncc;
            STAMP()
            __syncthreads();
            STAMP()
        }
#undef MVSGI_CTILES
#undef MVSGI_V_LOADW
#undef MVSGI_V_READX
#undef MVSGI_V_MFMAS
    } else {
        const int wm = wave % WM, wn = wave / WM;
        const int col = lane & 15, kg = lane >> 4;
        constexpr bool BSK = D32 && DK == 3 && TD == 2 && WM == 2 && MW == 4 && TH == 4 && TW == 16 && S == 1;
        static_assert(BRD == 0 || BSK, "border-plane skip: the 2 x 4 x 16 bricks of the 32-channel-slice kernels");
        const bool second = kg & 1;
        const char* wpb = reinterpret_cast<const char*>(a.wp);
        const unsigned lane16 = lane * 16;
        int base[MW];
#pragma unroll
        for (int i = 0; i < MW; ++i) {
            const int v = (wm * MW + i) * 16 + col;
            const int w_ = v % TW, h_ = BSK ? 2 * wm + (i & 1) : (v / TW) % TH, d_ = BSK ? (BRD == 2 ? 1 - (i >> 1) : (i >> 1)) : v / (TW * TH);
            base[i] = (((d_ * SD) * ITH + h_ * S) * ITW + w_ * S) * kVSB + (kg >> 1) * 16;
        }
        int tdv[MW], thv[MW], twv[MW];
#pragma unroll
        for (int i = 0; i < MW; ++i) {
            const int v = PLANE ? (i * TH + wm) * TW + col : (wm * MW + i) * 16 + col;
            twv[i] = v % TW;
            thv[i] = BSK ? 2 * wm + (i & 1) : (v / TW) % TH;
            tdv[i] = BSK ? (BRD == 2 ? 1 - (i >> 1) : (i >> 1)) : v / (TW * TH);
        }
        if constexpr (D32 && DK < 3 && !DKU) {
            const int kd_lo = (TD == 2 ? wm : 0) == 0 ? 1 : 0;
            wpb += kd_lo * 9 * 2048;
#pragma unroll
            for (int i = 0; i < MW; ++i) base[i] += kd_lo * (ITH * ITW * kVSB);
        }
        const long long frame_elems = (long long)a.Do * a.Ho * a.Wo * a.Cout;
        int ctc[NW], ctn[NW];
#define MVSGI_CTILES(DST, CB)                                                         \
        _Pragma("unroll") for (int j = 0; j < NW; ++j) {                              \
            const int c_ = ((CB) * WN + wn) * NW + j;                                 \
            DST[j] = c_ < CT ? c_ : CT - 1;                                           \
        }
        bf16x8 wh[WB][NW], wl[WB][NW];
        constexpr int XB = (KD == 3 && !PLANE && !V32 && MW * NW == 1) ? 8 : (KD == 3 && !PLANE && !V32 && MW * NW == 2) ? 4 : MW <= 4 ? 2 : 1;
        constexpr int XLA = XB > 1 ? XB - 1 : 1;
        constexpr int MH = XB >= 2 ? MW : MW / 2;
        bf16x8 xh[XB][MW], xl[XB][MW];
#define MVSGI_TAP(P) (BRD == 2 ? (2 - (P) / 9) * 9 + (P) % 9 : (P))
#define MVSGI_LOADW(BUFI, CC, P, CTS) MVSGI_LOADWB(wpb, BUFI, CC, P, CTS)
#define MVSGI_LOADWB(WPB, BUFI, CC, P, CTS)                                                           \
        _Pragma("unroll") for (int j = 0; j < NW; ++j) {                                              \
            const char* q_ = (WPB) + (((long long)(CC) * CT + CTS[j]) * kWBlk) * 2048;   \
            wh[BUFI][j] = *reinterpret_cast<const bf16x8*>(q_ + (l16 + (unsigned)MVSGI_TAP(P) * 2048u));          \
            wl[BUFI][j] = *reinterpret_cast<const bf16x8*>(q_ + (l16 + (unsigned)MVSGI_TAP(P) * 2048u + 1024u));  \
        }
#define MVSGI_READX(BUFI, P, I0, I1)                                                                  \
        {                                                                                             \
            const int p_ = (P);                                                                       \
            const int t0_ = 2 * p_, t1_ = (2 * p_ + 1 < kTaps) ? 2 * p_ + 1 : 2 * p_;                 \
            const int o0_ = (((t0_ / 9) * ITH + (t0_ / 3) % 3) * ITW + t0_ % 3) * kVSB;               \
            const int o1_ = (((t1_ / 9) * ITH + (t1_ / 3) % 3) * ITW + t1_ % 3) * kVSB;               \
            const int tp_ = MVSGI_TAP(p_);                                                            \
            const int od_ = (((tp_ / 9) * ITH + (tp_ / 3) % 3) * ITW + tp_ % 3) * kVSB;    \
            const int off_ = D32 ? od_ + (second ? SUB : 0) : (second ? o1_ : o0_);                   \
            _Pragma("unroll") for (int i = (I0); i < (I1); ++i) {                                     \
                xh[BUFI][i] = *reinterpret_cast<const bf16x8*>(img + base[i] + off_);                 \
                xl[BUFI][i] = *reinterpret_cast<const bf16x8*>(img + base[i] + off_ + 32);            \
            }                                                                                         \
            if constexpr (WLDS) {    \
                _Pragma("unroll") for (int j = 0; j < NW; ++j) {                                      \
                    wh[BUFI][j] = *reinterpret_cast<const bf16x8*>(img + BUF + (j * kPairs + p_) * 2048 + (int)lane16);          \
                    wl[BUFI][j] = *reinterpret_cast<const bf16x8*>(img + BUF + (j * kPairs + p_) * 2048 + 1024 + (int)lane16);   \
                }                                                                                     \
            }                                                                                         \
        }
#define MVSGI_MFMAS(WBUF, XBUF, I0, I1)                                                               \
        _Pragma("unroll") for (int i = (I0); i < (I1); ++i)                                           \
            _Pragma("unroll") for (int j = 0; j < NW; ++j)                                            \
                acc[i][j] = mfma16<F16>(wl[WBUF][j], xh[XBUF][i], acc[i][j]); \
        _Pragma("unroll") for (int i = (I0); i < (I1); ++i)                                           \
            _Pragma("unroll") for (int j = 0; j < NW; ++j)                                            \
                (TACC ? acc1[i][j] : acc[i][j]) = mfma16<F16>(wh[WBUF][j], xl[XBUF][i], TACC ? acc1[i][j] : acc[i][j]); \
        _Pragma("unroll") for (int i = (I0); i < (I1); ++i)                                           \
            _Pragma("unroll") for (int j = 0; j < NW; ++j)                                            \
                (TACC ? acc2[i][j] : acc[i][j]) = mfma16<F16>(wh[WBUF][j], xh[XBUF][i], TACC ? acc2[i][j] : acc[i][j]);
        constexpr bool TACC = KD == 3 && !PLANE && !V32 && MW * NW <= 2;
        f32x4 acc[MW][NW], acc1[MW][NW], acc2[MW][NW];
#pragma unroll
        for (int i = 0; i < MW; ++i)
#pragma unroll
            for (int j = 0; j < NW; ++j) {
                acc[i][j] = f32x4{0.f, 0.f, 0.f, 0.f};
                if (TACC) acc1[i][j] = acc2[i][j] = f32x4{0.f, 0.f, 0.f, 0.f};
            }

        int cb_, b_, od0, oh0, ow0;
        MVSGI_DECODE((int)blockIdx.x, cb_, b_, od0, oh0, ow0)
        MVSGI_CTILES(ctc, cb_)
        constexpr int NPP = 5;
        constexpr int PD = PLANE ? TD + 2 : 1;
        bf16x8 pwh[3][PLANE ? 3 : 1], pwl[3][PLANE ? 3 : 1];
        bf16x8 pxh[2][PD], pxl[2][PD];
        const int pbase = (wm * ITW + col) * kVSB + (kg >> 1) * 16;
#define MVSGI_PL_LOADW(BUFI, CC, P)                                                                    \
        _Pragma("unroll") for (int kd = 0; kd < 3; ++kd) {                                             \
            const char* q_ = wpb + ((long long)(((CC) * NPP + (P)) * 3 + kd)) * 2048;    \
            pwh[BUFI][kd] = *reinterpret_cast<const bf16x8*>(q_ + l16);                                \
            pwl[BUFI][kd] = *reinterpret_cast<const bf16x8*>(q_ + l16 + 1024u);                        \
        }
#define MVSGI_PL_READX(BUFI, P)                                                                        \
        {                                                                                              \
            const int t0_ = 2 * (P), t1_ = 2 * (P) + 1 < 9 ? 2 * (P) + 1 : 2 * (P);                    \
            const int o0_ = ((t0_ / 3) * ITW + t0_ % 3) * kVSB, o1_ = ((t1_ / 3) * ITW + t1_ % 3) * kVSB; \
            const int off_ = pbase + (second ? o1_ : o0_);                                             \
            _Pragma("unroll") for (int ip = 0; ip < PD; ++ip) {                                        \
                pxh[BUFI][ip] = *reinterpret_cast<const bf16x8*>(img + off_ + ip * (ITH * ITW * kVSB)); \
                pxl[BUFI][ip] = *reinterpret_cast<const bf16x8*>(img + off_ + ip * (ITH * ITW * kVSB) + 32); \
            }                                                                                          \
        }
#define MVSGI_PL_MFMAS(WBUFI, BUFI)                                                                         \
        _Pragma("unroll") for (int tr = 0; tr < 3; ++tr)                                               \
            _Pragma("unroll") for (int kd = 0; kd < 3; ++kd)                                           \
                _Pragma("unroll") for (int i = 0; i < TD; ++i)                                         \
                    acc[i][0] = mfma16<F16>(tr == 0 ? pwl[WBUFI][kd] : pwh[WBUFI][kd], tr == 1 ? pxl[BUFI][i + kd] : pxh[BUFI][i + kd], acc[i][0]);
        if constexpr (PLANE) {
            unsigned l16 = lane16;
            MVSGI_PL_LOADW(0, 0, 0)
            MVSGI_PL_LOADW(1, 0, 1)
        } else if constexpr (!WLDS) {
            unsigned l16 = lane16;
#pragma unroll
            for (int s0 = 0; s0 < LA; ++s0) { MVSGI_LOADWB(wpb + (DKU && od0 == 0 ? 9 * 2048 : 0), s0, 0, s0, ctc) }
        }
        STAMP()
        __syncthreads();
        STAMP()
        int k = 0, cc = 0;
        for (int u = 0; u < U; ++u) {
            const unsigned char* img = ldsb + (u & 1) * BUFW + (DKU && od0 == 0 ? ITH * ITW * kVSB : 0);
            const bool last = cc + 1 == nchunks;
            const bool more = u + 1 < U;
            const int ncc = last ? 0 : cc + 1;
            int ncb = cb_, nb = b_, nod0 = od0, noh0 = oh0, now0 = ow0;
            if (last && more) {
                MVSGI_DECODE((int)blockIdx.x + (k + 1) * G, ncb, nb, nod0, noh0, now0)
                MVSGI_CTILES(ctn, ncb)
            } else {
#pragma unroll
                for (int j = 0; j < NW; ++j) ctn[j] = ctc[j];
            }
            const char* const wpc_ = wpb + (DKU && od0 == 0 ? 9 * 2048 : 0);
            const char* const wpn_ = wpb + (DKU && nod0 == 0 ? 9 * 2048 : 0);
            f32x4 esc[NW], esh[NW], rres[RPRE ? MW : 1][RPRE ? NW : 1];
            int eoff[MW];
            int soff[MW];
            const int ypd = a.ys_2d ? 0 : 1, ypp = a.ys_2d ? 2 : 1;
#pragma unroll
            for (int j = 0; j < NW; ++j) {
                esc[j] = *reinterpret_cast<const f32x4*>(a.scale + ctc[j] * 16 + kg * 4);
                esh[j] = *reinterpret_cast<const f32x4*>(a.shift + ctc[j] * 16 + kg * 4);
            }
            if (last) {
#pragma unroll
                for (int i = 0; i < MW; ++i) {
                    const int od = od0 + tdv[i], oh = oh0 + thv[i], ow = ow0 + twv[i];
                    const bool inside = od < a.Do && oh < a.Ho && ow < a.Wo;
                    eoff[i] = inside ? ((od * a.Ho + oh) * a.Wo + ow) * a.Cout + kg * 4 : -1;
                    soff[i] = ((((od + ypd) * (a.Ho + 2 * ypp) + oh + ypp) * (a.Wo + 2 * ypp) + ow + ypp) * a.Cout) * 4 + (kg >> 1) * 16 + (kg & 1) * 8;
                }
            }
            if constexpr (PLANE) {
                MVSGI_PL_READX(0, 0)
#pragma unroll
                for (int p_ = 0; p_ < NPP + 1; ++p_) {
                    const int cur = p_ & 1, nxt = cur ^ 1;
                    unsigned l16 = lane16;
                    asm volatile("" : "+v"(l16));
                    if (p_ + 2 < NPP) {
                        MVSGI_PL_LOADW((p_ + 2) % 3, cc, p_ + 2)
                    } else if (p_ + 2 > NPP) {
                        MVSGI_PL_LOADW(p_ + 2 - (NPP + 1), ncc, p_ + 2 - (NPP + 1))
                    }
                    if (p_ < NPP) {
                        if (p_ + 1 < NPP) {
                            MVSGI_PL_READX(nxt, p_ + 1)
                        } else if (last && a.res) {
                            const float* rb = a.res + (long long)b_ * frame_elems;
#pragma unroll
                            for (int i = 0; i < MW; ++i)
                                rres[i][0] = *reinterpret_cast<const f32x4*>(rb + (eoff[i] >= 0 ? eoff[i] : 0));
                        }
                        MVSGI_PL_MFMAS(p_ % 3, cur)
                        if (p_ + 1 < NPP) {
#pragma unroll
                            for (int q_ = 0; q_ < 6 + 2 * PD; ++q_) {
                                __builtin_amdgcn_sched_group_barrier(0x008, 36 / (6 + 2 * PD) > 0 ? 36 / (6 + 2 * PD) : 1, 0);
                                __builtin_amdgcn_sched_group_barrier(0x120, 1, 0);
                            }
                            __builtin_amdgcn_sched_group_barrier(0x008, 36, 0);
                        }
                    }
                    __builtin_amdgcn_sched_barrier(0);
                }
            } else {
            if (XB >= 2) {
#pragma unroll
                for (int p0 = 0; p0 < XLA; ++p0) { MVSGI_READX(p0 % XB, p0, 0, MW) }
            } else {
                MVSGI_READX(0, 0, 0, MW)
            }
#pragma unroll
            for (int s_ = 0; s_ < NSLOT; ++s_) {
                const int wcur = s_ % WB;
                unsigned l16 = lane16;
                asm volatile("" : "+v"(l16));
                const int xcur = XB >= 2 ? (s_ % XB) : 0, xnxt = XB >= 2 ? ((s_ + XLA) % XB) : 0;
                if (!(MVSGI_ABL & 1) && !WLDS) {
                    if (s_ + LA < NSLOT) {
                        if (s_ + LA < kPairs) { MVSGI_LOADWB(wpc_, (s_ + LA) % WB, cc, s_ + LA, ctc) }
                    } else {
                        MVSGI_LOADWB(wpn_, (s_ + LA - NSLOT) % WB, ncc, s_ + LA - NSLOT, ctn)
                    }
                }
                if (RPRE && s_ == kPairs - 1 && last && a.res) {
                    const float* rb = a.res + (long long)b_ * frame_elems;
#pragma unroll
                    for (int i = 0; i < MW; ++i)
#pragma unroll
                        for (int j = 0; j < NW; ++j)
                            rres[i][j] = *reinterpret_cast<const f32x4*>(rb + (eoff[i] >= 0 ? eoff[i] + ctc[j] * 16 : 0));
                }
                if (s_ < kPairs - ((MVSGI_ABL & 32) ? 1 : 0)) {
                    if (XB >= 2) {
#define MVSGI_T0(SL) ((BRD != 0 && (SL) < 9) ? MW / 2 : 0)
#define MVSGI_T1(SL) (MW)
                        if (s_ + XLA < kPairs && !(MVSGI_ABL & 2)) MVSGI_READX(xnxt, s_ + XLA, MVSGI_T0(s_ + XLA), MVSGI_T1(s_ + XLA))
                        if (!(MVSGI_ABL & 16)) { MVSGI_MFMAS(wcur, xcur, MVSGI_T0(s_), MVSGI_T1(s_)) }
                        constexpr int NMEM = 2 * NW + 2 * MW, NMFMA = 3 * MW * NW;
                        constexpr int RATIO = NMFMA / NMEM > 0 ? NMFMA / NMEM : 1;
                        const bool full_ = MVSGI_T1(s_) - MVSGI_T0(s_) == MW && (s_ + XLA >= kPairs || MVSGI_T1(s_ + XLA) - MVSGI_T0(s_ + XLA) == MW);
                        if (full_) {
#pragma unroll
                        for (int q_ = 0; q_ < NMEM; ++q_) {
                            __builtin_amdgcn_sched_group_barrier(0x008, RATIO, 0);
                            __builtin_amdgcn_sched_group_barrier(0x120, 1, 0);
                        }
                        __builtin_amdgcn_sched_group_barrier(0x008, NMFMA, 0);
                        }
                    } else {
                        __builtin_amdgcn_sched_barrier(0);
                        MVSGI_MFMAS(wcur, 0, 0, MH)
                        __builtin_amdgcn_sched_barrier(0);
                        if (s_ + 1 < kPairs) MVSGI_READX(0, s_ + 1, 0, MH)
                        __builtin_amdgcn_sched_barrier(0);
                        MVSGI_MFMAS(wcur, 0, MH, MW)
                        __builtin_amdgcn_sched_barrier(0);
                        if (s_ + 1 < kPairs) MVSGI_READX(0, s_ + 1, MH, MW)
                    }
                }
                __builtin_amdgcn_sched_barrier(0);
            }
            }
            STAMP()
            if (last) {
                const int ct0 = (cb_ * WN + wn) * NW;
                float* yb = a.y + (long long)b_ * frame_elems;
                f32x4 rl[RPRE ? 1 : MW][RPRE ? 1 : NW];
                if (!RPRE && a.res) {
                    const float* rb = a.res + (long long)b_ * frame_elems;
#pragma unroll
                    for (int i = 0; i < (RPRE ? 1 : MW); ++i)
#pragma unroll
                        for (int j = 0; j < (RPRE ? 1 : NW); ++j)
                            rl[i][j] = *reinterpret_cast<const f32x4*>(rb + (eoff[i] >= 0 ? eoff[i] + ctc[j] * 16 : 0));
                }
#pragma unroll
                for (int i = 0; i < MW; ++i) {
#pragma unroll
                    for (int j = 0; j < NW; ++j) {
                        if (TACC) acc[i][j] = (acc[i][j] + acc1[i][j]) + acc2[i][j];
                        f32x4 r = acc[i][j] * esc[j] + esh[j];
                        if (a.res) r += RPRE ? rres[RPRE ? i : 0][RPRE ? j : 0] : rl[RPRE ? 0 : i][RPRE ? 0 : j];
#pragma unroll
                        for (int e = 0; e < 4; ++e) r[e] = r[e] > 0.f ? r[e] : r[e] * a.neg_slope;
                        if (a.y_split) {
                            u32x2 hi, lo;
                            split_x4<F16>(r, hi, lo, satm);
                            if (eoff[i] >= 0 && ct0 + j < CT) {
                                unsigned char* q = a.y_split + (long long)b_ * ((long long)(a.Do + 2 * ypd) * (a.Ho + 2 * ypp) * (a.Wo + 2 * ypp) * a.Cout * 4) +
                                                   soff[i] + (ct0 + j) * 64;
                                *reinterpret_cast<u32x2*>(q) = hi;
                                *reinterpret_cast<u32x2*>(q + 32) = lo;
                            }
                        } else if (eoff[i] >= 0 && ct0 + j < CT) *reinterpret_cast<f32x4*>(yb + eoff[i] + (ct0 + j) * 16) = r;
                        acc[i][j] = f32x4{0.f, 0.f, 0.f, 0.f};
                        if (TACC) acc1[i][j] = acc2[i][j] = f32x4{0.f, 0.f, 0.f, 0.f};
                    }
                }
                k += 1;
                cb_ = ncb; b_ = nb; od0 = nod0; oh0 = noh0; ow0 = now0;
#pragma unroll
                for (int j = 0; j < NW; ++j) ctc[j] = ctn[j];
            }
            cc = ncc;
            STAMP()
            __syncthreads();
            STAMP()
        }
#undef MVSGI_T0
#undef MVSGI_T1
#undef MVSGI_TAP
#undef MVSGI_PL_LOADW
#undef MVSGI_PL_READX
#undef MVSGI_PL_MFMAS
#undef MVSGI_CTILES
#undef MVSGI_LOADW
#undef MVSGI_READX
#undef MVSGI_MFMAS
    }
#undef MVSGI_DECODE
    STAMP()
#undef STAMP
    if constexpr (F16) sf_sat_report(a.sat, kSatSplit, satm, 65504.f);
}

template <int NW, int MW, int WM, int WN, int TD, int TH, int TW, int S, int KD = 3, bool UPS = false, bool PLANE = false,
          bool V32 = false, bool WLDS = false>
__global__ __launch_bounds__(512, 2) void conv3d_bf16x3_kernel(ConvArgs a) {
    conv3d_x3_body<NW, MW, WM, WN, TD, TH, TW, S, KD, UPS, PLANE, V32, WLDS, false>(a);
}
template <int NW, int MW, int WM, int WN, int TD, int TH, int TW, int S, int KD = 3, bool UPS = false, bool PLANE = false,
          bool V32 = false, bool WLDS = false>
__global__ __launch_bounds__(512, 2) void conv3d_f16x3_kernel(ConvArgs a) {
    conv3d_x3_body<NW, MW, WM, WN, TD, TH, TW, S, KD, UPS, PLANE, V32, WLDS, true>(a);
}

template <int NW, int MW, int WM, int WN, int TD, int TH, int TW>
__global__ __launch_bounds__(512, 2) void conv3d_bf16x3_d32_kernel(ConvArgs a) {
    conv3d_x3_body<NW, MW, WM, WN, TD, TH, TW, 1, 3, false, false, false, false, false, true>(a);
}
template <int NW, int MW, int WM, int WN, int TD, int TH, int TW>
__global__ __launch_bounds__(512, 2) void conv3d_f16x3_d32_kernel(ConvArgs a) {
    conv3d_x3_body<NW, MW, WM, WN, TD, TH, TW, 1, 3, false, false, false, false, true, true>(a);
}

template <int NW, int MW, int WM, int WN, int TD, int TH, int TW>
__global__ __launch_bounds__(512, 2) void conv3d_bf16x3_d32_dk_kernel(ConvArgs a) {
    conv3d_x3_body<NW, MW, WM, WN, TD, TH, TW, 1, 3, false, false, false, false, false, true, TD>(a);
}
template <int NW, int MW, int WM, int WN, int TD, int TH, int TW>
__global__ __launch_bounds__(512, 2) void conv3d_f16x3_d32_dk_kernel(ConvArgs a) {
    conv3d_x3_body<NW, MW, WM, WN, TD, TH, TW, 1, 3, false, false, false, false, true, true, TD>(a);
}
template <int NW, int MW, int WM, int WN, int TD, int TH, int TW>
__global__ __launch_bounds__(512, 2) void conv3d_bf16x3_d32u_dk_kernel(ConvArgs a) {
    conv3d_x3_body<NW, MW, WM, WN, TD, TH, TW, 1, 3, true, false, false, false, false, true, TD>(a);
}
template <int NW, int MW, int WM, int WN, int TD, int TH, int TW>
__global__ __launch_bounds__(512, 2) void conv3d_f16x3_d32u_dk_kernel(ConvArgs a) {
    conv3d_x3_body<NW, MW, WM, WN, TD, TH, TW, 1, 3, true, false, false, false, true, true, TD>(a);
}

template <int NW, int MW, int WM, int WN, int TD, int TH, int TW>
__global__ __launch_bounds__(512, 2) void conv3d_bf16x3_d32_dk2_kernel(ConvArgs a) {
    conv3d_x3_body<NW, MW, WM, WN, TD, TH, TW, 1, 3, false, false, false, false, false, true, 2>(a);
}
template <int NW, int MW, int WM, int WN, int TD, int TH, int TW>
__global__ __launch_bounds__(512, 2) void conv3d_f16x3_d32_dk2_kernel(ConvArgs a) {
    conv3d_x3_body<NW, MW, WM, WN, TD, TH, TW, 1, 3, false, false, false, false, true, true, 2>(a);
}

template <int NW, int MW, int WM, int WN, int TD, int TH, int TW, int BRD>
__global__ __launch_bounds__(512, 2) void conv3d_bf16x3_d32_brd_kernel(ConvArgs a) {
    conv3d_x3_body<NW, MW, WM, WN, TD, TH, TW, 1, 3, false, false, false, false, false, true, 3, BRD>(a);
}
template <int NW, int MW, int WM, int WN, int TD, int TH, int TW, int BRD>
__global__ __launch_bounds__(512, 2) void conv3d_f16x3_d32_brd_kernel(ConvArgs a) {
    conv3d_x3_body<NW, MW, WM, WN, TD, TH, TW, 1, 3, false, false, false, false, true, true, 3, BRD>(a);
}
template <int NW, int MW, int WM, int WN, int TD, int TH, int TW, int BRD>
__global__ __launch_bounds__(512, 2) void conv3d_bf16x3_d32u_brd_kernel(ConvArgs a) {
    conv3d_x3_body<NW, MW, WM, WN, TD, TH, TW, 1, 3, true, false, false, false, false, true, 3, BRD>(a);
}
template <int NW, int MW, int WM, int WN, int TD, int TH, int TW, int BRD>
__global__ __launch_bounds__(512, 2) void conv3d_f16x3_d32u_brd_kernel(ConvArgs a) {
    conv3d_x3_body<NW, MW, WM, WN, TD, TH, TW, 1, 3, true, false, false, false, true, true, 3, BRD>(a);
}

template <int NW, int MW, int WM, int WN, int TD, int TH, int TW>
__global__ __launch_bounds__(512, 2) void conv3d_bf16x3_d32u_kernel(ConvArgs a) {
    conv3d_x3_body<NW, MW, WM, WN, TD, TH, TW, 1, 3, true, false, false, false, false, true>(a);
}
template <int NW, int MW, int WM, int WN, int TD, int TH, int TW>
__global__ __launch_bounds__(512, 2) void conv3d_f16x3_d32u_kernel(ConvArgs a) {
    conv3d_x3_body<NW, MW, WM, WN, TD, TH, TW, 1, 3, true, false, false, false, true, true>(a);
}

template <int NW, int MW, int WM, int WN, int TD, int TH, int TW, int S, int KD = 3, bool UPS = false, bool PLANE = false,
          bool V32 = false, bool WLDS = false, bool F16 = false, bool D32 = false, bool DSK = false, int BRD = 0>
int launch_bf16x3(ConvArgs a, hipStream_t st) {
    constexpr int ITD = (TD - 1) * (KD == 1 ? 1 : S) + KD, ITH = (TH - 1) * S + 3, ITW = (TW - 1) * S + 3;
    constexpr int ROWP = V32 ? ((ITW * kVSB + 255) / 256) * 256 : ITW * kVSB;
    constexpr bool WARM = MVSGI_WARM && KD == 3 && !UPS && !PLANE && !V32 && !WLDS && S == 1 && MW * NW <= 2;
    static_assert(!D32 || (S == 1 && KD == 3 && !PLANE && !V32 && !WLDS), "32-channel slices: stride-1 3x3x3 variants");
    constexpr size_t lds_bytes = (size_t)2 * ((D32 ? 2 : 1) * ITD * ITH * ROWP + (WLDS ? NW * pairs_of(KD) * 2048 : 0)) + (WARM ? 4096 : 0);
    static_assert(lds_bytes <= 160 * 1024, "LDS images too large");
    void (*kern)(ConvArgs);
    static_assert(!DSK || (D32 && TD <= 2), "depth skip: 32-channel slices, one- or two-plane bricks");
    constexpr bool DKU = DSK && BRD == 3;
    static_assert(!DKU || (TD == 1 && !UPS), "per-unit depth skip: one-plane bricks");
    MVSGI_REQUIRE(!DSK || a.Do == (DKU ? 2 : TD), "conv3d: the depth-skip kernels serve volumes exactly %d planes deep (got %d)", DKU ? 2 : TD, a.Do);
    if constexpr (DKU && F16) kern = conv3d_f16x3_d32_dk2_kernel<NW, MW, WM, WN, TD, TH, TW>;
    else if constexpr (DKU) kern = conv3d_bf16x3_d32_dk2_kernel<NW, MW, WM, WN, TD, TH, TW>;
    else if constexpr (BRD != 0 && UPS && F16) kern = conv3d_f16x3_d32u_brd_kernel<NW, MW, WM, WN, TD, TH, TW, BRD>;
    else if constexpr (BRD != 0 && UPS) kern = conv3d_bf16x3_d32u_brd_kernel<NW, MW, WM, WN, TD, TH, TW, BRD>;
    else if constexpr (BRD != 0 && F16) kern = conv3d_f16x3_d32_brd_kernel<NW, MW, WM, WN, TD, TH, TW, BRD>;
    else if constexpr (BRD != 0) kern = conv3d_bf16x3_d32_brd_kernel<NW, MW, WM, WN, TD, TH, TW, BRD>;
    else if constexpr (DSK && UPS && F16) kern = conv3d_f16x3_d32u_dk_kernel<NW, MW, WM, WN, TD, TH, TW>;
    else if constexpr (DSK && UPS) kern = conv3d_bf16x3_d32u_dk_kernel<NW, MW, WM, WN, TD, TH, TW>;
    else if constexpr (DSK && F16) kern = conv3d_f16x3_d32_dk_kernel<NW, MW, WM, WN, TD, TH, TW>;
    else if constexpr (DSK) kern = conv3d_bf16x3_d32_dk_kernel<NW, MW, WM, WN, TD, TH, TW>;
    else if constexpr (D32 && UPS && F16) kern = conv3d_f16x3_d32u_kernel<NW, MW, WM, WN, TD, TH, TW>;
    else if constexpr (D32 && UPS) kern = conv3d_bf16x3_d32u_kernel<NW, MW, WM, WN, TD, TH, TW>;
    else if constexpr (D32 && F16) kern = conv3d_f16x3_d32_kernel<NW, MW, WM, WN, TD, TH, TW>;
    else if constexpr (D32) kern = conv3d_bf16x3_d32_kernel<NW, MW, WM, WN, TD, TH, TW>;
    else if constexpr (F16) kern = conv3d_f16x3_kernel<NW, MW, WM, WN, TD, TH, TW, S, KD, UPS, PLANE, V32, WLDS>;
    else kern = conv3d_bf16x3_kernel<NW, MW, WM, WN, TD, TH, TW, S, KD, UPS, PLANE, V32, WLDS>;
    MVSGI_REQUIRE(!D32 || a.Cin % 32 == 0, "conv3d: the 32-channel-slice kernels need Cin %% 32 == 0 (got %d)", a.Cin);
    static mvsgi::PersistentGeom geo_cache[mvsgi::kMaxDevices] = {};
    mvsgi::PersistentGeom geo;
    if (mvsgi::persistent_geometry(kern, 512, lds_bytes, 2, geo_cache, "conv3d(bf16x3)", geo)) return 1;
    a.tiles_h = (int)mvsgi::cdiv(a.Ho, TH);
    a.tiles_w = (int)mvsgi::cdiv(a.Wo, TW);
    const int CT = a.Cout / (V32 ? 32 : 16);
    constexpr bool kBorderSplit = D32 && !DSK && BRD == 0 && TD == 2 && WM == 2 && MW == 4 && TH == 4 && TW == 16 && S == 1;
    if constexpr (kBorderSplit) {
        const long long layer = (long long)a.B * a.tiles_h * a.tiles_w * mvsgi::cdiv(CT, WN * NW);
        if (a.od_cnt == 0 && a.Do == 4 && layer >= 4ll * geo.cus) {
            ConvArgs b = a;
            b.od_cnt = 1;
            b.od_off = 0;
            if (launch_bf16x3<NW, MW, WM, WN, TD, TH, TW, S, KD, UPS, PLANE, V32, WLDS, F16, D32, DSK, 1>(b, st)) return 1;
            b.od_off = 2;
            return launch_bf16x3<NW, MW, WM, WN, TD, TH, TW, S, KD, UPS, PLANE, V32, WLDS, F16, D32, DSK, 2>(b, st);
        }
    }
    a.tiles_d = a.od_cnt > 0 ? a.od_cnt : (int)mvsgi::cdiv(a.Do, TD);
    const long long nb = (long long)a.B * a.tiles_d * a.tiles_h * a.tiles_w * mvsgi::cdiv(CT, WN * NW);
    MVSGI_REQUIRE(nb < (1ll << 31), "conv3d: too many units");
    MVSGI_REQUIRE((long long)a.Din * a.Hin * a.Win * a.Cin < (1ll << 29), "conv3d: volume too large for 32-bit byte offsets");
    MVSGI_REQUIRE(!UPS || (a.Din % 2 == 0 && a.Hin % 2 == 0 && a.Win % 2 == 0), "conv3d: fused upsample needs even sizes");
    MVSGI_REQUIRE(!UPS || (long long)(a.Hin / 2) * (a.Win / 2) * a.Cin < (1ll << 23), "conv3d: fused upsample: low-resolution plane too large for 24-bit strides");
    MVSGI_REQUIRE((long long)a.Do * a.Ho * a.Wo * a.Cout < (1ll << 31), "conv3d: output frame too large for 32-bit element offsets");
    MVSGI_REQUIRE(!a.y_split || (!V32 && (long long)(a.Do + 2) * (a.Ho + 4) * (a.Wo + 4) * a.Cout * 4 < (1ll << 31)),
                  "conv3d: split-padded output not available for this kernel / size");
    a.total_units = (int)nb;
    MVSGI_SAT_WORDS(sat_words_);
    a.sat = sat_words_;
#ifdef MVSGI_STAMPS
    {
        static unsigned long long* dbgbuf = nullptr;
        const char* e_ = getenv("MVSGI_STAMP");
        if (e_ && !dbgbuf) { (void)hipMalloc(&dbgbuf, 8 * 128 * 8); (void)hipMemset(dbgbuf, 0, 8 * 128 * 8); }
        a.dbg = dbgbuf;
        if (e_ && atoi(e_) == 2 && dbgbuf) {
            static unsigned long long h[8 * 128];
            (void)hipDeviceSynchronize();
            (void)hipMemcpy(h, dbgbuf, sizeof(h), hipMemcpyDeviceToHost);
            for (int w = 0; w < 8; ++w) {
                fprintf(stderr, "wave %d:", w);
                for (int i = 0; i < 120; ++i) fprintf(stderr, " %lld", (long long)(h[w * 128 + i] - h[0]));
                fprintf(stderr, "\n");
            }
        }
    }
#endif
    hipLaunchKernelGGL(kern, dim3(mvsgi::persistent_grid(geo, nb)), dim3(512), lds_bytes, st, a);
    return mvsgi::check_launch("mvsgi_conv3d_f32(bf16x3)");
}
```

### mvs_gi_amd/csrc/conv3d_f16.hip

```cpp
#include "common.hpp"
#include "conv_common.hpp"
#include "conv3d_variants.hpp"
#ifdef MVSGI_STAMPS
#include <cstdio>
#include <cstdlib>
#endif

namespace {
#include "conv3d_bf16x3.hpp"
}

namespace mvsgi {

int conv3d_launch_b3_f16(int variant, const void* args, hipStream_t st) {
    const ConvArgs& a = *static_cast<const ConvArgs*>(args);
    switch (variant) {
#define MVSGI_MFMA(V, ...)
#define MVSGI_B3(V, K, ...) case V: return MVSGI_B3_LAUNCH##K(true, __VA_ARGS__)(a, st);
#include "conv3d_variants.inc"
#undef MVSGI_MFMA
#undef MVSGI_B3
    }
    return fail("mvsgi_conv3d_f32: variant %d has no fp16-split form (MVSGI_CONV_F16 goes with MVSGI_CONV_BF16X3 / _C16 / _V32)", variant);
}

}
```

### mvs_gi_amd/csrc/conv3d_up2poly.hip

```cpp
#include "common.hpp"

#include <cstring>
#include <vector>

namespace {

#include "split_fmt.hpp"

enum { FIRST = 0, INT = 1, LAST = 2, ONLY = 3 };

struct M3 {
    double m[3][3];
};

M3 axis_matrix(int p, int i, int n) {
    M3 M{};
    for (int k = 0; k < 3; ++k) {
        const int v = 2 * i + p + k - 1;
        if (v < 0 || v >= 2 * n) continue;
        const int m = v >> 1, q = v & 1;
        const int src[2] = {q == 0 ? m - 1 : m, q == 0 ? m : m + 1};
        const double wgt[2] = {q == 0 ? 0.25 : 0.75, q == 0 ? 0.75 : 0.25};
        for (int e = 0; e < 2; ++e) {
            int s_ = src[e] < 0 ? 0 : (src[e] > n - 1 ? n - 1 : src[e]);
            M.m[s_ - i + 1][k] += wgt[e];
        }
    }
    return M;
}
M3 class_matrix(int p, int cls) {
    const int n = cls == ONLY ? 1 : 4;
    const int i = cls == FIRST || cls == ONLY ? 0 : (cls == INT ? 1 : n - 1);
    return axis_matrix(p, i, n);
}
M3 face_delta(int p, int cls) {
    const M3 a = class_matrix(p, cls), b = class_matrix(p, INT);
    M3 d{};
    for (int k = 0; k < 3; ++k) d.m[1][k] = a.m[1][k] - b.m[1][k];
    return d;
}
void fold(const M3& Md, const M3& Mh, const M3& Mw, const float* w, float* out) {
    for (int oi = 0; oi < 16 * 32; ++oi) {
        const float* ws = w + (size_t)oi * 27;
        double t1[27], t2[27], t3[27];
        for (int a = 0; a < 3; ++a)
            for (int l = 0; l < 3; ++l)
                for (int m = 0; m < 3; ++m) {
                    double s = 0;
                    for (int k = 0; k < 3; ++k) s += Md.m[a][k] * ws[k * 9 + l * 3 + m];
                    t1[a * 9 + l * 3 + m] = s;
                }
        for (int a = 0; a < 3; ++a)
            for (int b = 0; b < 3; ++b)
                for (int m = 0; m < 3; ++m) {
                    double s = 0;
                    for (int l = 0; l < 3; ++l) s += Mh.m[b][l] * t1[a * 9 + l * 3 + m];
                    t2[a * 9 + b * 3 + m] = s;
                }
        for (int a = 0; a < 3; ++a)
            for (int b = 0; b < 3; ++b)
                for (int c = 0; c < 3; ++c) {
                    double s = 0;
                    for (int m = 0; m < 3; ++m) s += Mw.m[c][m] * t2[a * 9 + b * 3 + m];
                    t3[a * 9 + b * 3 + c] = s;
                }
        for (int q = 0; q < 27; ++q) out[(size_t)oi * 27 + q] = (float)t3[q];
    }
}

struct Group {
    int cls, first, count;
};
std::vector<Group> groups_of(int n) {
    if (n == 1) return {{ONLY, 0, 1}};
    if (n == 2) return {{FIRST, 0, 1}, {LAST, 1, 1}};
    return {{FIRST, 0, 1}, {INT, 1, n - 2}, {LAST, n - 1, 1}};
}
struct Face {
    int idx, cls;
};
std::vector<Face> faces_of(int n) {
    if (n == 1) return {{0, ONLY}};
    return {{0, FIRST}, {n - 1, LAST}};
}

constexpr int kMagic = 0x50325032;
constexpr int kRoleInts = 32;
enum { R_WOFF = 0, R_NTAPS, R_TAP0, R_XBASE = 11, R_XS0, R_XSRUN, R_N0, R_NRUN, R_YS0, R_YSRUN, R_MFIRST, R_MLAST, R_YBASE0 = 20 };
enum { ST_WRITE = 0, ST_RMW = 1, ST_SKIP = 2 };
constexpr size_t kFaceRoleWBytes = (size_t)9 * 8 * 2 * 64 * 16;
constexpr size_t kEdgeSetFloats = (size_t)9 * 32 * 16;

struct PolyHeader {
    int magic, D, H, W;
    int n_roles, n_edge_cells, n_groups, max_tpf;
    long long off_main, off_facew, off_roles, off_edgew, off_edgecells, total;
    int sum_tpf;
    int pad0;
    long long off_roles_split;
    long long off_wino;
    long long off_wino_unscale;
    int pad[4];
};
static_assert(sizeof(PolyHeader) == 128, "header");

inline size_t align256(size_t v) { return (v + 255) & ~(size_t)255; }

PolyHeader layout(int D, int H, int W) {
    PolyHeader h{};
    h.magic = kMagic;
    h.D = D; h.H = H; h.W = W;
    const int ng = (int)groups_of(D).size(), nfh = (int)faces_of(H).size(), nfw = (int)faces_of(W).size();
    h.n_groups = ng;
    h.n_roles = (nfh + nfw) * ng;
    h.n_edge_cells = nfh * nfw;
    size_t o = sizeof(PolyHeader);
    h.off_main = (long long)(o = align256(o));
    o += 16 * mvsgi::kRs32PackedBytes;
    h.off_facew = (long long)(o = align256(o));
    o += (size_t)h.n_roles * kFaceRoleWBytes;
    h.off_roles = (long long)(o = align256(o));
    o += (size_t)h.n_roles * kRoleInts * 4;
    h.off_roles_split = (long long)(o = align256(o));
    o += (size_t)h.n_roles * kRoleInts * 4;
    h.off_edgew = (long long)(o = align256(o));
    o += (size_t)ng * h.n_edge_cells * 8 * kEdgeSetFloats * 4;
    h.off_edgecells = (long long)(o = align256(o));
    o += (size_t)h.n_edge_cells * 4 * 4;
    if (mvsgi::wino_up2_applies(D, H, W)) {
        h.off_wino = (long long)(o = align256(o));
        o += 2 * mvsgi::kWinoUp2RoleBytes;
        h.off_wino_unscale = (long long)(o = align256(o));
        o += 2 * 32 * 4;
    }
    h.total = (long long)align256(o);
    int tpf = 0, sum = 0;
    for (const Group& g : groups_of(D)) {
        const int a = g.count * (int)mvsgi::cdiv(W, 16), b = g.count * (int)mvsgi::cdiv(H, 16);
        tpf = a > tpf ? a : tpf;
        tpf = b > tpf ? b : tpf;
        sum += nfh * a + nfw * b;
    }
    h.max_tpf = tpf;
    h.sum_tpf = sum;
    return h;
}

void pack_face_weights(const float* wsrc, const int* taps, unsigned short* out, bool f16) {
    for (int t = 0; t < 9; ++t)
        for (int ph = 0; ph < 8; ++ph)
            for (int lane = 0; lane < 64; ++lane) {
                const int kg = lane >> 4, co = lane & 15;
                const size_t o = (((size_t)(t * 8 + ph) * 2) * 64 + lane) * 8;
                for (int e = 0; e < 8; ++e) {
                    const float v = wsrc[(((size_t)ph * 16 + co) * 32 + kg * 8 + e) * 27 + taps[t]];
                    sf_split_weight(v, f16, out[o + e], out[o + 64 * 8 + e]);
                }
            }
}

struct FaceGrid {
    int n_roles;
    int first[13];
};
template <bool F16>
__global__ __launch_bounds__(512, 2) void up2_face_kernel(const unsigned char* __restrict__ x, const unsigned char* __restrict__ plan,
                                                          unsigned char* __restrict__ y, int B, long long x_frame, long long y_frame,
                                                          long long off_facew, long long off_roles, FaceGrid fg) {
    extern __shared__ __attribute__((aligned(16))) unsigned char fw_lds[];
    int role = 0;
#pragma unroll
    for (int r = 1; r < 12; ++r) role += (r < fg.n_roles && (int)blockIdx.x >= fg.first[r]) ? 1 : 0;
    const int chunk = (int)blockIdx.x - fg.first[role], chunks = fg.first[role + 1] - fg.first[role];
    const int* R = reinterpret_cast<const int*>(plan + off_roles) + role * kRoleInts;
    const int n0 = R[R_N0], nrun = R[R_NRUN];
    const int tiles_run = (nrun + 15) >> 4, tpf = n0 * tiles_run;
    const int tid = threadIdx.x, lane = tid & 63, wave = __builtin_amdgcn_readfirstlane(tid >> 6);
    const int col = lane & 15, kg = lane >> 4;
    {
        const u32x4* src = reinterpret_cast<const u32x4*>(plan + off_facew) + (long long)R[R_WOFF];
        for (int i = tid; i < (int)(kFaceRoleWBytes / 16); i += 512) reinterpret_cast<u32x4*>(fw_lds)[i] = src[i];
    }
    __syncthreads();
    int tap[9], yb[8];
#pragma unroll
    for (int t = 0; t < 9; ++t) tap[t] = R[R_TAP0 + t];
#pragma unroll
    for (int p = 0; p < 8; ++p) yb[p] = R[R_YBASE0 + p];
    const int x_base = R[R_XBASE], x_s0 = R[R_XS0], x_srun = R[R_XSRUN];
    const int y_s0 = R[R_YS0], y_srun = R[R_YSRUN];
    const int m_first = R[R_MFIRST], m_last = R[R_MLAST];
    const int lane_x = (kg >> 1) * 64 + (kg & 1) * 16;
    const int total = B * tpf, stride = chunks * 8;
    for (int t = chunk * 8 + wave; t < total; t += stride) {
        const int rt = t % tiles_run;
// ... 179 lines not shown
            for (int td = 0; td < 3; ++td)
                for (int th = 0; th < 3; ++th) {
                    taps27[td * 3 + th] = td * 9 + th * 3 + 1;
                    tap_off[td * 3 + th] = ((td - 1) * Hp + (th - 1)) * Wp * 128;
                }
            emit(taps27, tap_off, (((g.first + 1) * Hp + 1) * Wp + fw.idx + 1) * 128, Hp * Wp * 128, Wp * 128, g.count, H, yb, ys0, ysr,
                 ST_SKIP, ST_SKIP);
        }
    }
    MVSGI_REQUIRE(r == h.n_roles, "mvsgi_conv3d_up2_poly_plan: internal role count mismatch");
    int* cells = reinterpret_cast<int*>(P + h.off_edgecells);
    float* ew = reinterpret_cast<float*>(P + h.off_edgew);
    int e = 0;
    for (const Face& fh : fhs)
        for (const Face& fw : fws) {
            cells[e * 4] = fh.idx;
            cells[e * 4 + 1] = fw.idx;
            for (size_t gi = 0; gi < gs.size(); ++gi)
                for (int phase = 0; phase < 8; ++phase) {
                    const int pd = phase >> 2, ph = (phase >> 1) & 1, pw = phase & 1;
                    fold(class_matrix(pd, gs[gi].cls), class_matrix(ph, fh.cls), face_delta(pw, fw.cls), w, f0.data());
                    float* dst = ew + ((gi * h.n_edge_cells + e) * 8 + phase) * kEdgeSetFloats;
                    for (int td = 0; td < 3; ++td)
                        for (int th = 0; th < 3; ++th)
                            for (int ci = 0; ci < 32; ++ci)
                                for (int co = 0; co < 16; ++co)
                                    dst[((size_t)(td * 3 + th) * 32 + ci) * 16 + co] = f0[((size_t)co * 32 + ci) * 27 + td * 9 + th * 3 + 1];
                }
            ++e;
        }
    return 0;
}
extern "C" int mvsgi_conv3d_up2_poly_plan(const float* w_oidhw_host, void* plan_host, int D, int H, int W) {
    return mvsgi_conv3d_up2_poly_plan_fmt(w_oidhw_host, plan_host, D, H, W, 0);
}

namespace {

int poly_launch(const void* x_split, const void* plan_dev, const float* scale, const float* shift, void* y, int ob, int B, int D, int H,
                int W, float neg_slope, int fmt, hipStream_t st, int form = 0, bool rec32 = false) {
    MVSGI_REQUIRE(x_split && plan_dev && scale && shift && y, "mvsgi_conv3d_up2_poly: null pointer");
    MVSGI_REQUIRE(fmt == 0 || fmt == MVSGI_SPLIT_F16, "mvsgi_conv3d_up2_poly: fmt %d not in {0, MVSGI_SPLIT_F16}", fmt);
    MVSGI_REQUIRE(B > 0 && D > 0 && H > 0 && W > 0, "mvsgi_conv3d_up2_poly: bad dims");
    MVSGI_REQUIRE(neg_slope >= 0.f && neg_slope <= 1.f, "mvsgi_conv3d_up2_poly: neg_slope %g not in [0, 1]", (double)neg_slope);
    MVSGI_REQUIRE((long long)(D + 2) * (H + 2) * (W + 2) * 128 < (1ll << 31) &&
                      (long long)(2 * D + 2) * (2 * H + 2) * (2 * W + 2) * 64 < (1ll << 31),
                  "mvsgi_conv3d_up2_poly: frame too large for 32-bit offsets");
    const PolyHeader h = layout(D, H, W);
    const unsigned char* P = static_cast<const unsigned char*>(plan_dev);
    const long long x_frame = (long long)(D + 2) * (H + 2) * (W + 2) * 128;
    const long long y_frame = (long long)(2 * D + 2 * ob) * (2 * H + 2 * ob) * (2 * W + 2 * ob) * 64;
    const long long n = (long long)B * D * h.n_edge_cells * 128;
    MVSGI_REQUIRE(mvsgi::cdiv(n, 256) < (1ll << 31), "mvsgi_conv3d_up2_poly: too many edge threads");
    if (fmt)
        hipLaunchKernelGGL(up2_edge_kernel<true>, dim3((unsigned)mvsgi::cdiv(n, 256)), dim3(256), 0, st, static_cast<const unsigned char*>(x_split), P,
                           static_cast<float*>(y), B, D, H, W, h.n_edge_cells, h.n_groups, h.off_edgew, h.off_edgecells, ob);
    else
        hipLaunchKernelGGL(up2_edge_kernel<false>, dim3((unsigned)mvsgi::cdiv(n, 256)), dim3(256), 0, st, static_cast<const unsigned char*>(x_split), P,
                           static_cast<float*>(y), B, D, H, W, h.n_edge_cells, h.n_groups, h.off_edgew, h.off_edgecells, ob);
    if (mvsgi::check_launch("mvsgi_conv3d_up2_poly(edges)")) return 1;
    int dev = 0, cus = 256;
    if (hipGetDevice(&dev) == hipSuccess) (void)hipDeviceGetAttribute(&cus, hipDeviceAttributeMultiprocessorCount, dev);
    static bool attr_set[mvsgi::kMaxDevices] = {};
    if (dev >= 0 && dev < mvsgi::kMaxDevices && !attr_set[dev]) {
        hipError_t e = hipFuncSetAttribute(reinterpret_cast<const void*>(up2_face_kernel<false>), hipFuncAttributeMaxDynamicSharedMemorySize,
                                           (int)kFaceRoleWBytes);
        if (e == hipSuccess)
            e = hipFuncSetAttribute(reinterpret_cast<const void*>(up2_face_kernel<true>), hipFuncAttributeMaxDynamicSharedMemorySize,
                                    (int)kFaceRoleWBytes);
        MVSGI_REQUIRE(e == hipSuccess, "mvsgi_conv3d_up2_poly: hipFuncSetAttribute: %s", hipGetErrorString(e));
        attr_set[dev] = true;
    }
    MVSGI_REQUIRE(h.n_roles <= 12, "mvsgi_conv3d_up2_poly: internal: %d face roles", h.n_roles);
    long long slots = (long long)cus - h.n_roles;
    if (slots < 8) slots = 8;
    long long tpw = mvsgi::cdiv((long long)B * h.sum_tpf, slots);
    if (tpw < 8) tpw = 8;
    FaceGrid fg{};
    fg.n_roles = h.n_roles;
    {
        int r = 0, acc = 0;
        for (const Group& g : groups_of(D)) {
            const int nfh = (int)faces_of(H).size(), nfw = (int)faces_of(W).size();
            for (int f = 0; f < nfh + nfw; ++f) {
                const long long tpf = (long long)g.count * mvsgi::cdiv(f < nfh ? W : H, 16);
                fg.first[r++] = acc;
                acc += (int)mvsgi::cdiv((long long)B * tpf, tpw);
            }
        }
        fg.first[r] = acc;
    }
    if (fmt)
        hipLaunchKernelGGL(up2_face_kernel<true>, dim3((unsigned)fg.first[h.n_roles]), dim3(512), kFaceRoleWBytes, st,
                           static_cast<const unsigned char*>(x_split), P, static_cast<unsigned char*>(y), B, x_frame, y_frame, h.off_facew,
                           ob ? h.off_roles_split : h.off_roles, fg);
    else
        hipLaunchKernelGGL(up2_face_kernel<false>, dim3((unsigned)fg.first[h.n_roles]), dim3(512), kFaceRoleWBytes, st,
                           static_cast<const unsigned char*>(x_split), P, static_cast<unsigned char*>(y), B, x_frame, y_frame, h.off_facew,
                           ob ? h.off_roles_split : h.off_roles, fg);
    if (mvsgi::check_launch("mvsgi_conv3d_up2_poly(faces)")) return 1;
    MVSGI_REQUIRE(form != 2 || (fmt && ob && h.off_wino), "mvsgi_conv3d_up2_poly: the Winograd form needs the fp16 split, a split-padded output, "
                  "D == 8, H %% 2 == 0 and W %% 32 == 0 (got D, H, W = %d, %d, %d)", D, H, W);
    if (form == 2)
        return mvsgi::wino_up2_launch(x_split, P + h.off_wino, reinterpret_cast<const float*>(P + h.off_wino_unscale), scale, shift, y,
                                      B, D, H, W, neg_slope, rec32, st);
    if (fmt && ob && form == 0 && h.off_wino) {
        const long long units = (long long)B * (H / 2) * (W / 32);
        long long nwalk = cus / 16;
        if (nwalk > mvsgi::cdiv(units, 8)) nwalk = mvsgi::cdiv(units, 8);
        if (nwalk < 1) nwalk = 1;
        const long long rounds = mvsgi::cdiv(mvsgi::cdiv(units, 8), nwalk);
        if (10 * units >= 7 * rounds * 8 * nwalk)
            return mvsgi::wino_up2_launch(x_split, P + h.off_wino, reinterpret_cast<const float*>(P + h.off_wino_unscale), scale, shift, y,
                                          B, D, H, W, neg_slope, false, st);
    }
    return mvsgi::rs32_up2_launch(x_split, P + h.off_main, scale, shift, y, ob, B, D, H, W, neg_slope, fmt != 0, st);
}

}

extern "C" int mvsgi_conv3d_up2_poly_f32(const void* x_split, const void* plan_dev, const float* scale, const float* shift, float* y,
                                         int B, int D, int H, int W, float neg_slope, mvsgi_stream_t stream) {
    return poly_launch(x_split, plan_dev, scale, shift, y, 0, B, D, H, W, neg_slope, 0, mvsgi::as_stream(stream));
}

extern "C" int mvsgi_conv3d_up2_poly_split(const void* x_split, const void* plan_dev, const float* scale, const float* shift, void* y_split,
                                           int B, int D, int H, int W, float neg_slope, mvsgi_stream_t stream) {
    return poly_launch(x_split, plan_dev, scale, shift, y_split, 1, B, D, H, W, neg_slope, 0, mvsgi::as_stream(stream));
}

extern "C" int mvsgi_conv3d_up2_poly_fmt(const void* x_split, const void* plan_dev, const float* scale, const float* shift, void* y,
                                         int y_is_split, int B, int D, int H, int W, float neg_slope, int fmt, mvsgi_stream_t stream) {
    MVSGI_REQUIRE(y_is_split == 0 || y_is_split == 1 || y_is_split == 3 || y_is_split == 5, "mvsgi_conv3d_up2_poly: y_is_split %d not in {0, 1, 3, 5}",
                  y_is_split);
    return poly_launch(x_split, plan_dev, scale, shift, y, y_is_split ? 1 : 0, B, D, H, W, neg_slope, fmt, mvsgi::as_stream(stream),
                       y_is_split == 3 ? 1 : (y_is_split == 5 ? 2 : 0));
}

extern "C" int mvsgi_conv3d_up2_poly_rec32(const void* x_split, const void* plan_dev, const float* scale, const float* shift, void* y_rec32,
                                           int B, int D, int H, int W, float neg_slope, mvsgi_stream_t stream) {
    return poly_launch(x_split, plan_dev, scale, shift, y_rec32, 1, B, D, H, W, neg_slope, MVSGI_SPLIT_F16, mvsgi::as_stream(stream), 2, true);
}

extern "C" int mvsgi_conv3d_up2_poly_wino_pays(int B, int D, int H, int W) {
    if (!mvsgi::wino_up2_applies(D, H, W) || B < 1) return 0;
    const int cus = mvsgi::device_cus();
    const long long units = (long long)B * (H / 2) * (W / 32);
    long long nwalk = cus / 16;
    if (nwalk > mvsgi::cdiv(units, 8)) nwalk = mvsgi::cdiv(units, 8);
    if (nwalk < 1) nwalk = 1;
    const long long rounds = mvsgi::cdiv(mvsgi::cdiv(units, 8), nwalk);
    return 10 * units >= 7 * rounds * 8 * nwalk ? 1 : 0;
}
```

### mvs_gi_amd/csrc/conv_common.hpp

```cpp
#pragma once
namespace {

#include "device_prims.hpp"

struct ConvArgs {
    const float* x;
    const float* w_oidhw;
    const f32x4* wp;
    const float* scale;
    const float* shift;
    const float* res;
    float* y;
    int B, Cin, Din, Hin, Win, Cout, Do, Ho, Wo, stride;
    float neg_slope;
    int tiles_d, tiles_h, tiles_w;
    int od_off, od_cnt;
    int total_units;
    unsigned char* y_split;
    unsigned long long* dbg;
    int f16;
    int ys_2d;
    unsigned* sat;
};

constexpr int kVS = 20;


}
```

### mvs_gi_amd/dropin/common_modules.py

```python
from __future__ import annotations

import os

import copy
from typing import Dict, NamedTuple, Optional, Type

import torch
from torch import nn, Tensor

from .. import hip_ops as H


def module_getstate(self):
    return {k: v for k, v in self.__dict__.items() if not k.startswith("_mvsgi_")}


def _owned_split_buffer(owner, attr: str, key: tuple, make):
    bufs = owner.__dict__.setdefault(attr, {})
    if key not in bufs:
        bufs[key] = make()
    return bufs[key]


def _owned_head_buffer(self, B, D, Hh, W, C, device):
    bufs = self.__dict__.setdefault("_mvsgi_head_bufs", {})
    key = (D, Hh, W, C, device)
    ent = bufs.get(key)
    if ent is None or ent[0].B < B:
        big = H.SplitAct(B, D, Hh, W, C, device)
        keep = ent[1] + [ent[0]] if ent is not None and (ent[2] or ent[1]) else []
        ent = bufs[key] = [big, keep, False]
    if torch.cuda.is_current_stream_capturing():
        ent[2] = True
    big = ent[0]
    if big.B == B:
        return big
    return H.SplitAct(B, D, Hh, W, C, device, buf=big.buf[:B])


class NoOp(nn.Identity):
    def infer_size(self, in_size):
        return in_size


RELU_TYPE: Dict[str, Type[nn.Module]] = {"original": nn.ReLU, "leaky": nn.LeakyReLU, "none": NoOp}
NORM2D_TYPE: Dict[str, Type[nn.Module]] = {"batch": nn.BatchNorm2d, "instance": nn.InstanceNorm2d, "none": NoOp}
NORM3D_TYPE: Dict[str, Type[nn.Module]] = {"batch": nn.BatchNorm3d, "instance": nn.InstanceNorm3d, "none": NoOp}


_USE_D32 = os.environ.get("MVSGI_D32", "1") != "0"
_D32_OK: Dict[tuple, bool] = {}


class Packed(NamedTuple):
    wp: Tensor
    scale: object
    shift: object
    unscale: float = 1.0


class ConvLaunch:
    __slots__ = ("w", "wp", "scale", "shift", "stride", "neg_slope", "cin", "cout", "key", "inorm", "_cache")

    def __init__(self, w: Tensor, scale: Tensor, shift: Tensor, stride: int, neg_slope: float, inorm=None, key=None):
        self.w = w
        self.wp = H.pack_conv_weights(w)
        self.scale, self.shift = scale.contiguous(), shift.contiguous()
        self.stride, self.neg_slope, self.inorm, self.key = int(stride), neg_slope, inorm, key
        self.cout, self.cin = int(w.shape[0]), int(w.shape[1])
        self._cache: Dict[tuple, Packed] = {}

    def _cached(self, key: tuple, make) -> Packed:
        ent = self._cache.get(key)
        if ent is None:
            ent = self._cache[key] = make()
        return ent

    def _entry(self, packed) -> Packed:
        wp, unscale = packed if isinstance(packed, tuple) else (packed, None)
        return Packed(wp, self.scale if unscale is None else (self.scale * unscale).contiguous(), self.shift)

    def run(self, x_ndhwc: Tensor, res: Optional[Tensor] = None, impl: Optional[int] = None) -> Tensor:
        if self.inorm is not None:
            return self.inorm.apply(self._run_conv(x_ndhwc, None, impl), res)
        return self._run_conv(x_ndhwc, res, impl)

    def _run_conv(self, x_ndhwc: Tensor, res: Optional[Tensor] = None, impl: Optional[int] = None) -> Tensor:
        wp, scale = self.wp, self.scale
        if impl is None:
            impl = H.CONV_AUTO
            if H.split_mode() and self.cin % 16 == 0 and self.cout % 16 == 0:
                impl, wp, scale = self._stream(self._stream_layout(x_ndhwc.shape[:4]), H.mode_fmt())
        elif impl == H.CONV_BF16X3:
            wp = self._stream_packed(H.CONV_BF16X3, "bf16").wp
        return H.conv3d(x_ndhwc, self.w, wp, scale, self.shift, res=res, stride=self.stride, neg_slope=self.neg_slope, impl=impl)

    def _stream_layout(self, dims=None, up2: bool = False) -> int:
        if self._c16():
            return H.CONV_BF16X3_C16
        if dims is not None and _USE_D32 and H.split_mode() and self.cin % 32 == 0 and (up2 or (self.stride == 1 and self.cout % 16 == 0)):
            key = (up2, self.cin, self.cout) + tuple(dims)
            ok = _D32_OK.get(key)
            if ok is None:
                ok = _D32_OK[key] = H.conv3d_up2_d32_applies(dims[0], self.cin, *dims[1:], self.cout) if up2 else \
                    H.conv3d_d32_applies(dims[0], self.cin, *dims[1:], self.cout, self.stride)
            if ok:
                return H.CONV_BF16X3_D32
        return H.CONV_BF16X3

    def _stream_packed(self, layout: int, fmt: str) -> Packed:
        return self._cached(("stream", layout, fmt), lambda: self._entry(H._pack_conv3d_split(self.w, layout, fmt)))

    def _stream(self, layout: int, fmt: str):
        p = self._stream_packed(layout, fmt)
        return layout | (H.CONV_F16 if fmt == "f16" else 0), p.wp, p.scale

    def _c16(self) -> bool:
        return self.cout == 16 and self.stride == 1 and self.cin % 16 == 0

    def rs_ok(self) -> bool:
        return self.inorm is None and H.conv3d_rs_applies(self.cin, self.cout, self.stride, self.neg_slope)

    def _rs(self, fmt: str) -> Packed:
        return self._cached(("rs", fmt), lambda: self._entry(H.pack_conv_weights_rs(self.w, fmt)))

    def wino_ok(self, D: int, Hh: int, W: int) -> bool:
        return self.inorm is None and H.conv3d_wino_applies(self.cin, self.cout, D, Hh, W, self.stride, self.neg_slope)

    def _wino(self) -> Packed:
        return self._cached(("wino",), lambda: self._entry(H.pack_conv_weights_wino(self.w)))

    def s2rs_ok(self) -> bool:
        return self.inorm is None and H.split_mode() and H.conv3d_s2rs_applies(self.cin, self.cout, self.stride, self.neg_slope)

    def _s2(self, fmt: str) -> Packed:
        def make():
            if fmt == "bf16":
                return Packed(H.pack_conv_weights_s2rs(self.w, self.scale), None, self.shift)
            wp, up, un = H.pack_conv_weights_s2rs(self.w, self.scale, "f16")
            return Packed(wp, None, (self.shift * up).contiguous(), un)
        return self._cached(("s2", fmt), make)

    def poly_ok(self) -> bool:
        return self.inorm is None and H.split_mode() and self.stride == 1 and H.conv3d_up2_poly_applies(self.cin, self.cout, self.neg_slope)

    def _poly_plan(self, x_split) -> Packed:
        D, Hh, W, fmt = x_split.D, x_split.H, x_split.W, x_split.fmt
        return self._cached(("poly", D, Hh, W, fmt), lambda: self._entry(H.conv3d_up2_poly_plan(self.w, D, Hh, W, fmt=fmt)))

    def head_split_ok(self) -> bool:
        return self.inorm is None and H.split_mode() and self.cout == 1 and self.cin % 16 == 0 and self.stride == 1

    def run_head_split(self, x_split) -> Tensor:
        def make():
            if x_split.fmt == "f16":
                wp, unscale = H.pack_head_split_weights_f16(self.w)
                return Packed(wp, float(self.scale[0]) * unscale, float(self.shift[0]))
            return Packed(H.pack_head_split_weights(self.w), float(self.scale[0]), float(self.shift[0]))
        p = self._cached(("head", x_split.fmt), make)
        return H.conv3d_head_split(x_split, p.wp, p.scale, p.shift, neg_slope=self.neg_slope, f16=x_split.fmt == "f16")

    def run_up2_poly_split(self, x_split, out) -> "H.SplitAct":
        p = self._poly_plan(x_split)
        return H.conv3d_up2_poly_split(x_split, p.wp, p.scale, self.shift, out=out, neg_slope=self.neg_slope)

    def run_up2_poly(self, x_split, out=None) -> Tensor:
        p = self._poly_plan(x_split)
        return H.conv3d_up2_poly(x_split, p.wp, p.scale, self.shift, neg_slope=self.neg_slope, out=out)

    def run_up2_split(self, x_lowres_ndhwc: Tensor, res: Optional[Tensor], out) -> "H.SplitAct":
        _no_inorm(self, "run_up2_split")
        w_layout, wp, scale = self._stream(self._stream_layout(), H.mode_fmt())
        return H.conv3d_up2_out_split(x_lowres_ndhwc, wp, scale, self.shift, out=out, res=res, neg_slope=self.neg_slope, w_layout=w_layout)

    def can_fuse_up2(self) -> bool:
        return H.split_mode() and self.stride == 1 and self.cin % 16 == 0 and self.cout % 16 == 0

    def run_up2(self, x_lowres_ndhwc: Tensor, res: Optional[Tensor] = None) -> Tensor:
        if self.inorm is not None:
            return self.inorm.apply(self._run_up2(x_lowres_ndhwc, None), res)
        return self._run_up2(x_lowres_ndhwc, res)

    def _run_up2(self, x_lowres_ndhwc: Tensor, res: Optional[Tensor] = None) -> Tensor:
        w_layout, wp, scale = self._stream(self._stream_layout(x_lowres_ndhwc.shape[:4], up2=True), H.mode_fmt())
        return H.conv3d_up2(x_lowres_ndhwc, wp, scale, self.shift, res=res, neg_slope=self.neg_slope, w_layout=w_layout)


def _is_identity(m) -> bool:
    return m is None or isinstance(m, nn.Identity)


def _fingerprint(blk) -> tuple:
    conv = blk.conv_layer
    parts = [conv.weight.data_ptr(), conv.weight._version, tuple(conv.stride)]
    if conv.bias is not None:
        parts += [conv.bias.data_ptr(), conv.bias._version]
    parts += norm_key(blk.norm_layer)
    act = blk.activation
    parts += [type(act).__name__, float(getattr(act, "negative_slope", 0.0))]
    return tuple(parts)


_BN = (nn.BatchNorm3d, nn.BatchNorm2d)
_IN = (nn.InstanceNorm3d, nn.InstanceNorm2d)


def norm_key(norm) -> list:
    parts = [type(norm).__name__]
    if isinstance(norm, _BN + _IN):
        parts += [bool(norm.training), float(norm.eps), bool(getattr(norm, "track_running_stats", True))]
        for t in (norm.weight, norm.bias, norm.running_mean, norm.running_var):
            parts += [None, None] if t is None else [t.data_ptr(), t._version]
    return parts


class InstanceNormLaunch:
    __slots__ = ("gamma", "beta", "eps", "neg_slope")

    def apply(self, y: Tensor, res: Optional[Tensor] = None) -> Tensor:
        return H.instance_norm(y, res=res, gamma=self.gamma, beta=self.beta, eps=self.eps, neg_slope=self.neg_slope, out=y)


def _no_inorm(L, what: str) -> None:
    if L.inorm is not None:
        raise RuntimeError(f"{what}: this layer has an instance norm (its epilogue does not fold); use the plain fp32 path")


def lower_norm(norm, conv_bias: Optional[Tensor], cout: int, device, slope: float, dims: int = 3):
    bias = conv_bias.detach().float() if conv_bias is not None else None
    name = type(norm).__name__
    use_running = isinstance(norm, _BN) or (isinstance(norm, _IN) and norm.track_running_stats)
    if use_running:
        if norm.training:
            raise RuntimeError(f"HIP path implements eval-mode {name} only: call model.eval()")
        if norm.running_mean is None or norm.running_var is None:
            raise NotImplementedError(f"{name} without running statistics")
        gamma = norm.weight.detach().float() if norm.weight is not None else torch.ones(cout, device=device)
        beta = norm.bias.detach().float() if norm.bias is not None else torch.zeros(cout, device=device)
        alpha = gamma / torch.sqrt(norm.running_var.detach().float() + norm.eps)
        scale = alpha
        shift = beta - norm.running_mean.detach().float() * alpha
        if bias is not None:
            shift = shift + bias * alpha
        return scale, shift, None
    scale = torch.ones(cout, device=device, dtype=torch.float32)
    shift = bias.clone() if bias is not None else torch.zeros(cout, device=device, dtype=torch.float32)
    if _is_identity(norm):
        return scale, shift, None
    if isinstance(norm, _IN):
        if norm.affine and norm.num_features != cout:
            raise ValueError(f"{name}({norm.num_features}) after a conv with {cout} output channels")
        rec = InstanceNormLaunch()
        rec.gamma = norm.weight.detach().float().contiguous() if norm.affine and norm.weight is not None else None
        rec.beta = norm.bias.detach().float().contiguous() if norm.affine and norm.bias is not None else None
        rec.eps, rec.neg_slope = float(norm.eps), float(slope)
        return scale, shift, rec
    raise NotImplementedError(f"norm layer {name} has no HIP implementation "
                              f"(only BatchNorm{dims}d in eval mode, InstanceNorm{dims}d and NoOp)")


def act_slope(act) -> float:
    if isinstance(act, nn.LeakyReLU):
        return float(act.negative_slope)
    if isinstance(act, nn.ReLU):
        return 0.0
    if _is_identity(act):
        return 1.0
    raise NotImplementedError(f"activation {type(act).__name__} has no HIP implementation")


def lower_conv_block(blk) -> ConvLaunch:
    key = _fingerprint(blk)
    cached = blk.__dict__.get("_mvsgi_launch")
    if cached is not None and cached.key == key:
        return cached
    conv: nn.Conv3d = blk.conv_layer
    if not isinstance(conv, nn.Conv3d):
        raise NotImplementedError(f"conv_layer is {type(conv).__name__}, expected nn.Conv3d")
    if tuple(conv.kernel_size) != (3, 3, 3) or tuple(conv.padding) != (1, 1, 1) or tuple(conv.dilation) != (1, 1, 1) \
            or conv.groups != 1 or conv.padding_mode != "zeros" or len(set(conv.stride)) != 1 \
            or conv.stride[0] not in (1, 2):
        raise NotImplementedError(
            f"HIP conv3d supports kernel 3, padding 1, stride 1|2, dense; got kernel {tuple(conv.kernel_size)}, "
            f"padding {tuple(conv.padding)}, stride {tuple(conv.stride)}, groups {conv.groups}")
    w = conv.weight.detach()
    if not w.is_cuda:
        raise RuntimeError("mvs_gi_amd modules run on the GPU only: call .cuda() on the model "
                           "(there is no CPU fallback)")
    w = w.to(torch.float32).contiguous()
    cout = w.shape[0]
    if isinstance(blk.norm_layer, (nn.BatchNorm2d, nn.InstanceNorm2d)):
        raise NotImplementedError(f"norm layer {type(blk.norm_layer).__name__} after a Conv3d")
    slope = act_slope(blk.activation)
    scale, shift, inorm = lower_norm(blk.norm_layer, conv.bias, cout, w.device, slope)
    if inorm is not None:
        slope = 1.0
    L = ConvLaunch(w, scale, shift, conv.stride[0], slope, inorm, key)
    blk.__dict__["_mvsgi_launch"] = L
    return L


def _to_ncdhw_view(y_ndhwc: Tensor) -> Tensor:
    return y_ndhwc.permute(0, 4, 1, 2, 3)


class BaseConvBlk3d(nn.Module):
    def __init__(self, in_chs: int, out_chs: int, kernel_size: int, stride: int = 1, extra_pad: int = 0,
                 bias_on: bool = False, norm_layer: nn.Module = NoOp(), activation: nn.Module = NoOp()):
        super().__init__()
        self.conv_layer = nn.Conv3d(in_chs, out_chs, kernel_size, padding=(kernel_size // 2) + extra_pad,
                                    bias=bias_on, stride=stride)
        self.norm_layer = norm_layer
        self.activation = activation

    __getstate__ = module_getstate

    def forward_ndhwc(self, x: Tensor, res: Optional[Tensor] = None) -> Tensor:
        return lower_conv_block(self).run(x, res)

    def forward(self, x: Tensor, res: Optional[Tensor] = None) -> Tensor:
        r = None if res is None else H.as_ndhwc(res)
        return _to_ncdhw_view(self.forward_ndhwc(H.as_ndhwc(x), r))


def res_block_ndhwc(blk, x: Tensor) -> Tensor:
    if not _is_identity(blk.one_by_one):
# ... 52 lines not shown
```

### mvs_gi_amd/hip_ops.py

```python
from __future__ import annotations

from typing import Optional

import torch

from . import _lib

import ctypes
import math
import os

CONV_AUTO, CONV_DIRECT, CONV_MFMA, CONV_BF16X3, CONV_BF16X3_C16, CONV_BF16X3_V32, CONV_BF16X3_D32 = 0, 1, 2, 3, 4, 5, 6
SPLIT_F16 = 1
CONV_F16 = 0x100

CONV_MODES = ("f32", "bf16x3", "f16x3")
_CONV_MODE = os.environ.get("MVSGI_CONV_MODE", "f16x3")
if _CONV_MODE not in CONV_MODES:
    raise ValueError(f"MVSGI_CONV_MODE={_CONV_MODE!r} not in {CONV_MODES}")




def set_conv_mode(mode: str) -> None:
# ... 270 lines not shown


def sweep_cat(feats, grids, layout: str = "auto") -> torch.Tensor:
    nhwc = layout == "auto" and feats.dim() == 5 and feats.shape[2] % 4 == 0
    f = _feats_nhwc(feats) if nhwc else _dev(feats, "feats")
    B, N, C, Hi, Wi = feats.shape
    grids = _dev(grids, "grids")
    Bg, Ng, D, Ho, Wo, two = grids.shape
    if (Bg, Ng, two) != (B, N, 2):
        raise AssertionError(f"grids {tuple(grids.shape)} do not match feats {tuple(feats.shape)}")
    vol = torch.empty((B, D, Ho, Wo, N * C), device=f.device, dtype=torch.float32)
    _call("mvsgi_sweep_cat_nhwc_f32" if nhwc else "mvsgi_sweep_cat_f32", f.data_ptr(), grids.data_ptr(), vol.data_ptr(), B, N, C, Hi, Wi,
          D, Ho, Wo, _stream_ptr(f))
    return vol


def pack_conv_weights(w_oidhw: torch.Tensor) -> Optional[torch.Tensor]:
    lib = _lib.load()
    w = _dev(w_oidhw, "conv weight")
    Cout, Cin = w.shape[:2]
    if tuple(w.shape[2:]) != (3, 3, 3):
        raise NotImplementedError(f"only 3x3x3 kernels are supported, got {tuple(w.shape[2:])}")
    if Cin % 16 or not (Cout % 16 == 0 or Cout == 1):
        return None
    wp = torch.empty(lib.mvsgi_conv3d_packed_weight_floats(Cout, Cin), device=w.device, dtype=torch.float32)
    _call("mvsgi_conv3d_pack_weights_f32", w.data_ptr(), wp.data_ptr(), Cout, Cin, _stream_ptr(w))
    return wp


def _pack_conv3d_split(w_oidhw: torch.Tensor, layout: int, fmt: str = "bf16"):
    lib = _lib.load()
    w = _dev(w_oidhw, "conv weight")
    Cout, Cin = w.shape[:2]
    if tuple(w.shape[2:]) != (3, 3, 3) or Cin % 16 or Cout % 16 or (layout == CONV_BF16X3_C16 and Cout != 16) or \
            (layout == CONV_BF16X3_V32 and Cout % 32) or (layout == CONV_BF16X3_D32 and Cin % 32):
        return None
    unscale = None
    if fmt == "f16":
        up, unscale = _pow2_unscale(w.abs().amax(dim=(1, 2, 3, 4)))
        w = (w * up.view(-1, 1, 1, 1, 1)).contiguous()
    n = {CONV_BF16X3: lambda: lib.mvsgi_conv3d_packed_weight_bytes_bf16x3(Cout, Cin),
         CONV_BF16X3_C16: lambda: lib.mvsgi_conv3d_packed_weight_bytes_bf16x3_c16(Cin),
         CONV_BF16X3_D32: lambda: lib.mvsgi_conv3d_packed_weight_bytes_bf16x3(Cout, Cin),
         CONV_BF16X3_V32: lambda: lib.mvsgi_conv3d_packed_weight_bytes_bf16x3_v32(Cout, Cin)}[layout]()
    wp = torch.empty(n, device=w.device, dtype=torch.uint8)
    _call("mvsgi_conv3d_pack_weights_split", w.data_ptr(), wp.data_ptr(), Cout, Cin, layout | (CONV_F16 if _fmt_code(fmt) else 0),
          _stream_ptr(w))
    return wp, (None if unscale is None else unscale.contiguous())


def _pack_bf16(w_oidhw: torch.Tensor, layout: int) -> Optional[torch.Tensor]:
    p = _pack_conv3d_split(w_oidhw, layout)
    return None if p is None else p[0]


def pack_conv_weights_bf16x3(w_oidhw: torch.Tensor) -> Optional[torch.Tensor]:
    return _pack_bf16(w_oidhw, CONV_BF16X3)


def pack_conv_weights_f16x3(w_oidhw: torch.Tensor, layout: int = CONV_BF16X3):
    return _pack_conv3d_split(w_oidhw, layout, "f16")


def pack_conv_weights_bf16x3_d32(w_oidhw: torch.Tensor) -> Optional[torch.Tensor]:
    return _pack_bf16(w_oidhw, CONV_BF16X3_D32)


def pack_conv_weights_bf16x3_v32(w_oidhw: torch.Tensor) -> Optional[torch.Tensor]:
    return _pack_bf16(w_oidhw, CONV_BF16X3_V32)


def pack_conv_weights_bf16x3_c16(w_oidhw: torch.Tensor) -> Optional[torch.Tensor]:
    return _pack_bf16(w_oidhw, CONV_BF16X3_C16)


def conv3d_d32_applies(B, Cin, Din, Hin, Win, Cout, stride=1) -> bool:
    return bool(_lib.load().mvsgi_conv3d_d32_applies(B, Cin, Din, Hin, Win, Cout, stride))


def conv3d_up2_d32_applies(B, Cin, Dl, Hl, Wl, Cout) -> bool:
    return bool(_lib.load().mvsgi_conv3d_up2_d32_applies(B, Cin, Dl, Hl, Wl, Cout))


def conv3d_v32_applies(B, Cin, Din, Hin, Win, Cout, stride=1) -> bool:
    return bool(_lib.load().mvsgi_conv3d_v32_applies(B, Cin, Din, Hin, Win, Cout, stride))


def _split_layout_bytes(layout: int, Cout: int, Cin: int) -> int:
    lib = _lib.load()
    layout &= ~CONV_F16
    if layout == CONV_BF16X3_C16:
        return lib.mvsgi_conv3d_packed_weight_bytes_bf16x3_c16(Cin)
    if layout == CONV_BF16X3_V32:
        return lib.mvsgi_conv3d_packed_weight_bytes_bf16x3_v32(Cout, Cin)
    if layout in (CONV_BF16X3, CONV_BF16X3_D32):
        return lib.mvsgi_conv3d_packed_weight_bytes_bf16x3(Cout, Cin)
    raise ValueError(f"w_layout {layout} is not one of the streaming split kernel's layouts")


def _conv3d_packed(w_packed, name: str, device, impl: int, Cout: int, Cin: int) -> Optional[int]:
    base = impl & ~CONV_F16
    split = base in (CONV_BF16X3_C16, CONV_BF16X3_V32, CONV_BF16X3_D32) or (base == CONV_BF16X3 and Cin % 16 == 0 and Cout % 16 == 0)
    if w_packed is None:
        if split:
            raise AssertionError(f"{name}: impl {impl} needs the packed weights of its layout")
        return None
    if split:
        return _arg(w_packed, name, device, torch.uint8, nbytes=_split_layout_bytes(base, Cout, Cin)).data_ptr()
    if base == CONV_DIRECT:
        return _arg(w_packed, name, device, _PACKED).data_ptr()
    packs = Cin % 16 == 0 and (Cout % 16 == 0 or Cout == 1)
    return _arg(w_packed, name, device, numel=_lib.load().mvsgi_conv3d_packed_weight_floats(Cout, Cin) if packs else None).data_ptr()


def conv3d(x, w_oidhw, w_packed, scale, shift, res=None, stride=1, neg_slope=0.01, impl=CONV_AUTO, out=None):
    x = _dev(x, "x")
    B, Din, Hin, Win, Cin = x.shape
    dev = x.device
    sc, sh, Cout = _scale_shift(scale, shift, dev)
    Do, Ho, Wo = (Din - 1) // stride + 1, (Hin - 1) // stride + 1, (Win - 1) // stride + 1
    shp = (B, Do, Ho, Wo, Cout)
    y = torch.empty(shp, device=dev, dtype=torch.float32) if out is None else _arg(out, "out", dev, shape=shp)
    _call("mvsgi_conv3d_f32", x.data_ptr(), _opt(w_oidhw, "w_oidhw", dev, shape=(Cout, Cin, 3, 3, 3)),
          _conv3d_packed(w_packed, "w_packed", dev, impl, Cout, Cin), sc, sh, _opt(res, "res", dev, shape=shp), y.data_ptr(), B, Cin, Din,
          Hin, Win, Cout, stride, float(neg_slope), impl, _stream_ptr(x))
    return y


def conv3d_up2(x, w_packed_b3, scale, shift, res=None, neg_slope=0.01, out=None, w_layout=CONV_BF16X3):
    x = _dev(x, "x")
    B, Dl, Hl, Wl, Cin = x.shape
    dev = x.device
    sc, sh, Cout = _scale_shift(scale, shift, dev)
    shp = (B, 2 * Dl, 2 * Hl, 2 * Wl, Cout)
    wp = _arg(w_packed_b3, "w_packed_b3", dev, torch.uint8, nbytes=_split_layout_bytes(w_layout, Cout, Cin))
    y = torch.empty(shp, device=dev, dtype=torch.float32) if out is None else _arg(out, "out", dev, shape=shp)
    _call("mvsgi_conv3d_up2_f32", x.data_ptr(), wp.data_ptr(), w_layout, sc, sh, _opt(res, "res", dev, shape=shp), y.data_ptr(), B, Cin, Dl,
          Hl, Wl, Cout, float(neg_slope), _stream_ptr(x))
    return y


def conv3d_up2_out_split(x, w_packed_b3, scale, shift, out: "SplitAct", res=None, neg_slope=0.01, w_layout=CONV_BF16X3) -> "SplitAct":
    x = _dev(x, "x")
    B, Dl, Hl, Wl, Cin = x.shape
    dev = x.device
    sc, sh, Cout = _scale_shift(scale, shift, dev)
    shp = (B, 2 * Dl, 2 * Hl, 2 * Wl, Cout)
    yp = _split_ptr(out, "out", dev, shp)
    wp = _arg(w_packed_b3, "w_packed_b3", dev, torch.uint8, nbytes=_split_layout_bytes(w_layout, Cout, Cin))
    _call("mvsgi_conv3d_up2_f32_out_split", x.data_ptr(), wp.data_ptr(), w_layout, sc, sh, _opt(res, "res", dev, shape=shp),
          yp, B, Cin, Dl, Hl, Wl, Cout, float(neg_slope), _stream_ptr(x))
    out.fmt = "f16" if w_layout & CONV_F16 else "bf16"
    return out


def conv3d_up2_poly_applies(cin: int, cout: int, neg_slope: float) -> bool:
    return cin == 32 and cout == 16 and 0.0 <= neg_slope <= 1.0


def conv3d_up2_poly_plan(w_oidhw: torch.Tensor, D: int, H: int, W: int, fmt: str = "bf16"):
    lib = _lib.load()
    if tuple(w_oidhw.shape) != (16, 32, 3, 3, 3):
        raise AssertionError(f"polyphase plan needs a [16, 32, 3, 3, 3] weight, got {tuple(w_oidhw.shape)}")
    n = lib.mvsgi_conv3d_up2_poly_plan_bytes(D, H, W)
    if not n:
        raise RuntimeError("mvsgi_conv3d_up2_poly_plan_bytes: bad dims")
    wh = w_oidhw.detach().to("cpu", torch.float32).contiguous()
    unscale = None
    if fmt == "f16":
        up, un = _pow2_unscale(wh.abs().amax(dim=(1, 2, 3, 4)))
        wh = (wh * up.view(-1, 1, 1, 1, 1)).contiguous()
        unscale = un.to(w_oidhw.device)
    plan = torch.empty(n, dtype=torch.uint8)
    _call("mvsgi_conv3d_up2_poly_plan_fmt", wh.data_ptr(), plan.data_ptr(), D, H, W, _fmt_code(fmt))
    plan = plan.to(w_oidhw.device)
    return (plan, unscale) if fmt == "f16" else plan


def _poly_plan_ptr(plan, device, x: "SplitAct") -> int:
    return _arg(plan, "plan", device, torch.uint8, nbytes=_lib.load().mvsgi_conv3d_up2_poly_plan_bytes(x.D, x.H, x.W)).data_ptr()


def conv3d_up2_poly(x: "SplitAct", plan: torch.Tensor, scale, shift, neg_slope=0.01, out=None) -> torch.Tensor:
    xp = _split_ptr(x, "x")
    dev = x.buf.device
    if x.C != 32:
        raise AssertionError("conv3d_up2_poly is the 32 -> 16 kernel")
    sc, sh, _ = _scale_shift(scale, shift, dev, 16)
    shp = (x.B, 2 * x.D, 2 * x.H, 2 * x.W, 16)
    y = torch.empty(shp, device=dev, dtype=torch.float32) if out is None else _arg(out, "out", dev, shape=shp)
    _call("mvsgi_conv3d_up2_poly_fmt", xp, _poly_plan_ptr(plan, dev, x), sc, sh, y.data_ptr(), 0, x.B, x.D, x.H, x.W,
          float(neg_slope), _fmt_code(x.fmt), _stream_ptr(x.buf))
    return y


POLY_WINO = os.environ.get("MVSGI_POLY_WINO", "1") != "0"


def conv3d_up2_poly_wino_pays(B: int, D: int, Hh: int, W: int) -> bool:
    return POLY_WINO and bool(_lib.load().mvsgi_conv3d_up2_poly_wino_pays(int(B), int(D), int(Hh), int(W)))


def conv3d_up2_poly_split(x: "SplitAct", plan: torch.Tensor, scale, shift, out: "SplitAct", neg_slope=0.01, direct: bool = False,
                          wino: bool = False) -> "SplitAct":
    xp = _split_ptr(x, "x")
    dev = x.buf.device
    if x.C != 32:
        raise AssertionError(f"conv3d_up2_poly_split: input {x.shape}: the 32 -> 16 kernel")
    yp = _split_ptr(out, "out", dev, (x.B, 2 * x.D, 2 * x.H, 2 * x.W, 16))
    sc, sh, _ = _scale_shift(scale, shift, dev, 16)
    pp = _poly_plan_ptr(plan, dev, x)
    if out.rec == "f32":
        if x.fmt != "f16" or direct or not POLY_WINO:
            raise AssertionError(f"conv3d_up2_poly_split: fp32 records need the fp16 split's Winograd form (input holds {x.fmt} pieces, direct={direct})")
        _call("mvsgi_conv3d_up2_poly_rec32", xp, pp, sc, sh, yp,
              x.B, x.D, x.H, x.W, float(neg_slope), _stream_ptr(x.buf))
        out.fmt = x.fmt
        return out
    _call("mvsgi_conv3d_up2_poly_fmt", xp, pp, sc, sh, yp,
          5 if wino else (3 if (direct or not POLY_WINO) else 1), x.B, x.D, x.H, x.W, float(neg_slope), _fmt_code(x.fmt), _stream_ptr(x.buf))
    out.fmt = x.fmt
    return out


def pack_head_split_weights(w_oidhw: torch.Tensor) -> Optional[torch.Tensor]:
    lib = _lib.load()
    w = _dev(w_oidhw, "conv weight")
    if w.shape[0] != 1 or tuple(w.shape[2:]) != (3, 3, 3) or w.shape[1] % 16:
        return None
    wp = torch.empty(lib.mvsgi_conv3d_head_split_packed_weight_bytes(int(w.shape[1])), device=w.device, dtype=torch.uint8)
    _call("mvsgi_conv3d_head_split_pack_weights", w.data_ptr(), wp.data_ptr(), int(w.shape[1]), _stream_ptr(w))
    return wp


def pack_head_split_weights_f16(w_oidhw: torch.Tensor):
    lib = _lib.load()
    w = _dev(w_oidhw, "conv weight")
    if w.shape[0] != 1 or tuple(w.shape[2:]) != (3, 3, 3) or w.shape[1] % 16:
        return None
    amax = float(w.abs().max())
    k = 0.0 if amax == 0.0 else float(torch.floor(torch.log2(torch.tensor(1024.0 / amax))))
    ws = (w * (2.0 ** k)).contiguous()
    wp = torch.empty(lib.mvsgi_conv3d_head_split_packed_weight_bytes(int(w.shape[1])), device=w.device, dtype=torch.uint8)
    _call("mvsgi_conv3d_head_split_pack_weights_f16", ws.data_ptr(), wp.data_ptr(), int(w.shape[1]), _stream_ptr(w))
    return wp, 2.0 ** -k


def conv3d_head_split(x: "SplitAct", w_packed, scale: float, shift: float, neg_slope=1.0, out=None, f16: bool = False) -> torch.Tensor:
    if x.fmt != ("f16" if f16 else "bf16"):
        raise AssertionError(f"conv3d_head_split(f16={f16}) on a split-padded buffer holding {x.fmt} pieces")
    if x.rec == "f32" and not f16:
        raise AssertionError("conv3d_head_split: fp32 records are read in the fp16 split only")
    xp = _split_ptr(x, "x")
    dev = x.buf.device
    shp = (x.B, x.D, x.H, x.W, 1)
    y = torch.empty(shp, device=dev, dtype=torch.float32) if out is None else _arg(out, "out", dev, shape=shp)
    wp = _arg(w_packed, "w_packed", dev, torch.uint8, nbytes=_lib.load().mvsgi_conv3d_head_split_packed_weight_bytes(x.C))
    _call("mvsgi_conv3d_head_rec32_f16" if x.rec == "f32" else ("mvsgi_conv3d_head_split_f16" if f16 else "mvsgi_conv3d_head_split"),
          xp, wp.data_ptr(), float(scale),
          float(shift), y.data_ptr(), x.B, x.C, x.D, x.H, x.W, float(neg_slope), _stream_ptr(x.buf))
    return y


def conv3d_up2_variant(B, Cin, Dl, Hl, Wl, Cout, w_layout=CONV_BF16X3) -> str:
    lib = _lib.load()
    name = lib.mvsgi_conv3d_up2_variant_f32(B, Cin, Dl, Hl, Wl, Cout, w_layout)
    if name is None:
        raise RuntimeError("mvsgi_conv3d_up2_variant_f32: " + lib.mvsgi_last_error().decode())
    return name.decode()


def conv3d_variant(B, Cin, Din, Hin, Win, Cout, stride=1, impl=CONV_AUTO) -> str:
    lib = _lib.load()
    name = lib.mvsgi_conv3d_variant_f32(B, Cin, Din, Hin, Win, Cout, stride, impl)
    if name is None:
        raise RuntimeError("mvsgi_conv3d_variant_f32: " + lib.mvsgi_last_error().decode())
    return name.decode()


class SplitAct:
    __slots__ = ("buf", "B", "D", "H", "W", "C", "fmt", "rec")

    def __init__(self, B, D, H, W, C, device, buf=None):
        self.B, self.D, self.H, self.W, self.C = int(B), int(D), int(H), int(W), int(C)
        self.fmt = "bf16"
        self.rec = "pairs"
        if buf is None:
            buf = torch.zeros((self.B, self.D + 2, self.H + 2, self.W + 2, self.C), device=device, dtype=torch.int32)
        else:
            _arg(buf, "buf", torch.device(device), torch.int32, shape=(self.B, self.D + 2, self.H + 2, self.W + 2, self.C))
        self.buf = buf

    @property
    def shape(self):
        return (self.B, self.D, self.H, self.W, self.C)

    @property
    def device(self):
        return self.buf.device


def _split_ptr(s, name: str, device=None, shape=None) -> int:
    if not isinstance(s, SplitAct):
        raise TypeError(f"{name}: expected a SplitAct, got {type(s)}")
    if shape is not None and s.shape != tuple(shape):
        raise AssertionError(f"{name}: split-padded buffer {s.shape} does not match {tuple(shape)}")
# ... 1292 lines not shown
```

Baseline: 6552.

## Add polyphase-folded streaming path for fused upsample-by-2 3D conv

```diff
diff --git a/include/mvsgi.h b/include/mvsgi.h
--- a/include/mvsgi.h
+++ b/include/mvsgi.h
@@ -245,6 +245,17 @@
                               int y_is_split, int B, int D, int H, int W, float neg_slope, int fmt, mvsgi_stream_t stream);
 int mvsgi_conv3d_up2_poly_wino_pays(int B, int D, int H, int W);
 
+size_t mvsgi_conv3d_up2_stream_plan_bytes(int Cin, int Cout);
+int mvsgi_conv3d_up2_stream_plan(const float* w_oidhw_host, void* plan_host, int Cin, int Cout, int fmt);
+int mvsgi_conv3d_up2_stream_fold(const float* w_oidhw_host, float* out_host, int Cin, int Cout, int cls);
+int mvsgi_conv3d_up2_stream_pays(int B, int Cin, int Cout, int Dl, int Hl, int Wl);
+int mvsgi_conv3d_up2_stream_f32(const float* x, const void* w_packed, int w_layout, const void* plan_dev, const float* scale,
+                                const float* shift, const float* res, float* y, int B, int Cin, int Dl, int Hl, int Wl, int Cout,
+                                float neg_slope, int form, mvsgi_stream_t stream);
+int mvsgi_conv3d_up2_stream_out_split(const float* x, const void* w_packed, int w_layout, const void* plan_dev, const float* scale,
+                                      const float* shift, const float* res, void* y_split, int B, int Cin, int Dl, int Hl, int Wl,
+                                      int Cout, float neg_slope, int form, mvsgi_stream_t stream);
+
 size_t mvsgi_conv3d_wino32_packed_weight_bytes(void);
 int mvsgi_conv3d_wino32_applies(int Cin, int Cout, int D, int H, int W, int stride, float neg_slope);
 int mvsgi_conv3d_wino32_pack_weights(const float* w_oidhw, void* w_packed, float* unscale, mvsgi_stream_t stream);
diff --git a/mvs_gi_amd/_lib.py b/mvs_gi_amd/_lib.py
--- a/mvs_gi_amd/_lib.py
+++ b/mvs_gi_amd/_lib.py
@@ -120,6 +120,12 @@
     "mvsgi_conv3d_wino32_f16": (c_int, [_P] * 6 + [c_int] * 6 + [c_float, _P]),
     "mvsgi_conv3d_up2_poly_fmt": (c_int, [_P] * 5 + [c_int] * 5 + [c_float, c_int, _P]),
     "mvsgi_conv3d_up2_poly_wino_pays": (c_int, [c_int] * 4),
+    "mvsgi_conv3d_up2_stream_plan_bytes": (c_size_t, [c_int, c_int]),
+    "mvsgi_conv3d_up2_stream_plan": (c_int, [_P, _P] + [c_int] * 3),
+    "mvsgi_conv3d_up2_stream_fold": (c_int, [_P, _P] + [c_int] * 3),
+    "mvsgi_conv3d_up2_stream_pays": (c_int, [c_int] * 6),
+    "mvsgi_conv3d_up2_stream_f32": (c_int, [_P, _P, c_int] + [_P] * 5 + [c_int] * 6 + [c_float, c_int, _P]),
+    "mvsgi_conv3d_up2_stream_out_split": (c_int, [_P, _P, c_int] + [_P] * 5 + [c_int] * 6 + [c_float, c_int, _P]),
     "mvsgi_ncv_to_nvc_f32": (c_int, [_P, _P, c_int, c_int, c_longlong, _P]),
     "mvsgi_nvc_to_ncv_f32": (c_int, [_P, _P, c_int, c_int, c_longlong, _P]),
     "mvsgi_instance_norm_ws_bytes": (c_size_t, [c_int] * 3),
diff --git a/mvs_gi_amd/csrc/common.hpp b/mvs_gi_amd/csrc/common.hpp
--- a/mvs_gi_amd/csrc/common.hpp
+++ b/mvs_gi_amd/csrc/common.hpp
@@ -115,4 +115,10 @@
 int wino_up2_launch(const void* x_split, const void* w_roles, const float* unw, const float* scale16, const float* shift16, void* y_split,
                     int B, int D, int H, int W, float neg_slope, bool out_f32, hipStream_t st);
 
+constexpr int kUp2StreamMagic = 0x50325333;
+constexpr size_t kUp2StreamHeaderBytes = 256;
+inline size_t up2_stream_set_bytes(int Cin, int Cout) { return (size_t)(Cin / 32) * (8 * Cout / 16) * 27 * 2 * 64 * 16; }
+int conv3d_up2_stream_main_f16(const void* args, hipStream_t st);
+int conv3d_up2_stream_border_f16(int variant, const void* args, hipStream_t st);
+
 }
diff --git a/mvs_gi_amd/csrc/conv3d.hip b/mvs_gi_amd/csrc/conv3d.hip
--- a/mvs_gi_amd/csrc/conv3d.hip
+++ b/mvs_gi_amd/csrc/conv3d.hip
@@ -704,3 +704,113 @@
     const int v = select_variant_up2(a, w_layout & ~MVSGI_CONV_F16);
     return variant_name(v, a);
 }
+
+namespace {
+
+struct Up2StreamGeo {
+    int tiles_h, tiles_w;
+    int oh0, oh1, ow0, ow1;
+    bool interior;
+};
+Up2StreamGeo up2_stream_geo(int Hl, int Wl) {
+    Up2StreamGeo g{};
+    g.tiles_h = (int)mvsgi::cdiv(2 * Hl, 4);
+    g.tiles_w = (int)mvsgi::cdiv(2 * Wl, 16);
+    g.interior = g.tiles_h > 2 && g.tiles_w > 2;
+    g.oh0 = 2; g.oh1 = 2 * (g.tiles_h - 1);
+    g.ow0 = 8; g.ow1 = 8 * (g.tiles_w - 1);
+    return g;
+}
+int up2_border_variant(int Cout, int w_layout) {
+    const int CT = Cout / 16;
+    if (CT == 1) return w_layout == MVSGI_CONV_BF16X3_C16 ? B3PU_N16 : B3U_N16;
+    if (CT == 2) return B3U_N32;
+    if (CT == 3) return B3U_N48;
+    return CT % 4 == 0 ? B3U_N64 : V_COUNT;
+}
+
+int launch_up2_border(int v, const ConvArgs& a, hipStream_t st) {
+    if (a.f16) return mvsgi::conv3d_up2_stream_border_f16(v, &a, st);
+    switch (v) {
+        case B3U_N16: return launch_bf16x3<1, 4, 4, 1, 4, 4, 16, 1, 3, true, false, false, false, false, false, false, 0, 2>(a, st);
+        case B3PU_N16: return launch_bf16x3<1, 4, 4, 1, 4, 4, 16, 1, 3, true, true, false, false, false, false, false, 0, 2>(a, st);
+        case B3U_N32: return launch_bf16x3<2, 4, 4, 1, 4, 4, 16, 1, 3, true, false, false, false, false, false, false, 0, 2>(a, st);
+        case B3U_N48: return launch_bf16x3<3, 4, 4, 1, 4, 4, 16, 1, 3, true, false, false, false, false, false, false, 0, 2>(a, st);
+        case B3U_N64: return launch_bf16x3<2, 4, 2, 2, 2, 4, 16, 1, 3, true, false, false, false, false, false, false, 0, 2>(a, st);
+    }
+    return mvsgi::fail("mvsgi_conv3d_up2_stream: variant %d has no border launch", v);
+}
+int launch_up2_main(const ConvArgs& a, hipStream_t st) {
+    if (a.f16) return mvsgi::conv3d_up2_stream_main_f16(&a, st);
+    return launch_bf16x3<2, 4, 1, 4, 1, 4, 16, 1, 3, false, false, false, false, false, true, false, 0, 1>(a, st);
+}
+
+long long up2_stream_units(int B, int Cout, int Dl, const Up2StreamGeo& g) {
+    return (long long)B * Dl * mvsgi::cdiv(g.oh1 - g.oh0, 4) * mvsgi::cdiv(g.ow1 - g.ow0, 16) * mvsgi::cdiv(8 * Cout / 16, 8);
+}
+
+int up2_stream(const char* who, const float* x, const void* w_packed, int w_layout, const void* plan_dev, const float* scale,
+               const float* shift, const float* res, float* y, void* y_split, int B, int Cin, int Dl, int Hl, int Wl, int Cout,
+               float neg_slope, int form, hipStream_t st) {
+    const bool f16 = (w_layout & MVSGI_CONV_F16) != 0;
+    w_layout &= ~MVSGI_CONV_F16;
+    MVSGI_REQUIRE(w_layout == MVSGI_CONV_BF16X3 || (w_layout == MVSGI_CONV_BF16X3_C16 && Cout == 16), "%s: w_layout %d not valid for Cout %d", who,
+                  w_layout, Cout);
+    MVSGI_REQUIRE(x && (y || y_split) && scale && shift && w_packed && plan_dev, "%s: null pointer", who);
+    MVSGI_REQUIRE(Dl > 0 && Hl > 0 && Wl > 0 && Dl < (1 << 20) && Hl < (1 << 20) && Wl < (1 << 20), "%s: bad dims", who);
+    MVSGI_REQUIRE(Cin > 0 && Cout > 0 && Cin % 32 == 0 && Cout % 16 == 0, "%s: Cin %d must be a multiple of 32, Cout %d of 16", who, Cin, Cout);
+    MVSGI_REQUIRE(form >= 0 && form <= 2, "%s: form %d not in {0, 1, 2}", who, form);
+    MVSGI_REQUIRE(mvsgi::aligned(plan_dev, 16), "%s: plan not 16-byte aligned", who);
+    ConvArgs a{};
+    if (fill_args(a, x, nullptr, static_cast<const float*>(w_packed), scale, shift, res, y_split ? reinterpret_cast<float*>(y_split) : y, B, Cin,
+                  2 * Dl, 2 * Hl, 2 * Wl, Cout, 1, neg_slope))
+        return 1;
+    a.y_split = static_cast<unsigned char*>(y_split);
+    a.f16 = f16;
+    const Up2StreamGeo g = up2_stream_geo(Hl, Wl);
+    const int v = up2_border_variant(Cout, w_layout);
+    MVSGI_REQUIRE(form == 0 || v != V_COUNT, "%s: no border launch for Cout %d (16, 32, 48 or a multiple of 64)", who, Cout);
+    const bool two = g.interior && v != V_COUNT && (form != 0 || mvsgi_conv3d_up2_stream_pays(B, Cin, Cout, Dl, Hl, Wl));
+    if (!two) {
+        const int v1 = select_variant_up2(a, w_layout);
+        if (v1 == V_COUNT) return 1;
+        return launch_variant(v1, a, st);
+    }
+    ConvArgs b = a;
+    b.bor_n = 2 * g.tiles_w + 2 * (g.tiles_h - 2);
+    ConvArgs m{};
+    if (fill_args(m, x, nullptr, reinterpret_cast<const float*>(static_cast<const unsigned char*>(plan_dev) + mvsgi::kUp2StreamHeaderBytes), scale,
+                  shift, res, a.y, B, Cin, Dl, Hl, Wl, 8 * Cout, 1, neg_slope))
+        return 1;
+    m.y_split = a.y_split;
+    m.f16 = f16;
+    m.poly_ctp = Cout / 16;
+    m.poly_oh0 = g.oh0; m.poly_oh1 = g.oh1; m.poly_ow0 = g.ow0; m.poly_ow1 = g.ow1;
+    m.poly_wset = (long long)mvsgi::up2_stream_set_bytes(Cin, Cout);
+    if (form == 2) return launch_up2_border(v, b, st) || launch_up2_main(m, st);
+    return launch_up2_main(m, st) || launch_up2_border(v, b, st);
+}
+
+}
+
+extern "C" int mvsgi_conv3d_up2_stream_pays(int B, int Cin, int Cout, int Dl, int Hl, int Wl) {
+    if (B < 1 || Cin < 32 || Cout < 16 || Cin % 32 || Cout % 16 || Dl < 1 || Hl < 1 || Wl < 1) return 0;
+    const Up2StreamGeo g = up2_stream_geo(Hl, Wl);
+    if (!g.interior) return 0;
+    if (Cout != 16) return 0;
+    return up2_stream_units(B, Cout, Dl, g) >= 16ll * mvsgi::device_cus() ? 1 : 0;
+}
+
+extern "C" int mvsgi_conv3d_up2_stream_f32(const float* x, const void* w_packed, int w_layout, const void* plan_dev, const float* scale,
+                                           const float* shift, const float* res, float* y, int B, int Cin, int Dl, int Hl, int Wl,
+                                           int Cout, float neg_slope, int form, mvsgi_stream_t stream) {
+    return up2_stream("mvsgi_conv3d_up2_stream_f32", x, w_packed, w_layout, plan_dev, scale, shift, res, y, nullptr, B, Cin, Dl, Hl, Wl, Cout,
+                      neg_slope, form, mvsgi::as_stream(stream));
+}
+
+extern "C" int mvsgi_conv3d_up2_stream_out_split(const float* x, const void* w_packed, int w_layout, const void* plan_dev, const float* scale,
+                                                 const float* shift, const float* res, void* y_split, int B, int Cin, int Dl, int Hl,
+                                                 int Wl, int Cout, float neg_slope, int form, mvsgi_stream_t stream) {
+    return up2_stream("mvsgi_conv3d_up2_stream_out_split", x, w_packed, w_layout, plan_dev, scale, shift, res, nullptr, y_split, B, Cin, Dl, Hl, Wl,
+                      Cout, neg_slope, form, mvsgi::as_stream(stream));
+}
diff --git a/mvs_gi_amd/csrc/conv3d_bf16x3.hpp b/mvs_gi_amd/csrc/conv3d_bf16x3.hpp
--- a/mvs_gi_amd/csrc/conv3d_bf16x3.hpp
+++ b/mvs_gi_amd/csrc/conv3d_bf16x3.hpp
@@ -187,8 +187,10 @@
     wp[o + 64] = __builtin_bit_cast(bf16x8, lo);
 }
 
-template <int NW, int MW, int WM, int WN, int TD, int TH, int TW, int S, int KD, bool UPS, bool PLANE, bool V32, bool WLDS, bool F16, bool D32 = false, int DK = 3, int BRD = 0>
+template <int NW, int MW, int WM, int WN, int TD, int TH, int TW, int S, int KD, bool UPS, bool PLANE, bool V32, bool WLDS, bool F16, bool D32 = false, int DK = 3, int BRD = 0, int POLY = 0>
 __device__ __forceinline__ void conv3d_x3_body(const ConvArgs& a) {
+    static_assert(POLY != 1 || (D32 && !UPS && TD == 1 && DK == 3 && BRD == 0 && MW * NW <= 8), "polyphase main launch: one-plane bricks on 32-channel slices");
+    static_assert(POLY != 2 || (UPS && !D32 && !V32 && DK == 3 && BRD == 0), "border launch: the tap-pair fused-upsample variants");
     static_assert(!WLDS || (WN == 1 && KD == 3 && !UPS && !PLANE && !V32 && S == 1 && NW == 1 && MW <= 2), "LDS-staged weights: one shared cout tile, one or two voxel tiles per wave");
     static_assert(!V32 || (S == 1 && KD == 3 && TW == 16 && TH % 2 == 0 && !PLANE), "32x32x16 schedule: stride 1, 16-wide even bricks");
     static_assert(!PLANE || (NW == 1 && WN == 1 && WM == 4 && TH == 4 && MW == TD && TW == 16 && S == 1 && KD == 3),
@@ -237,6 +239,8 @@
     const int ny = (CT + WN * NW - 1) / (WN * NW);
     const int nchunks = a.Cin / (D32 ? 32 : 16);
     const int total = a.total_units;
+    const int nbatch = a.B;
+    (void)nbatch;
     const int G = gridDim.x;
     const int nmine = (total - (int)blockIdx.x + G - 1) / G;
     const int U = nmine * nchunks;
@@ -256,13 +260,43 @@
 
 #define MVSGI_DECODE_DH(T, OD, OH, B) { OD = (T % a.tiles_d) * TD + a.od_off; T /= a.tiles_d; OH = (T % a.tiles_h) * TH; B = T / a.tiles_h; }
 #define MVSGI_DECODE(ID, CB, B, OD, OH, OW)                       \
-    {                                                             \
+    if constexpr (POLY == 1) {                                    \
+         \
+        int t_ = xcd_remap((ID), total);                          \
+        OW = (t_ % a.tiles_w) * TW + a.poly_ow0;                  \
+        t_ /= a.tiles_w;                                          \
+        OH = (t_ % a.tiles_h) * TH + a.poly_oh0;                  \
+        t_ /= a.tiles_h;                                          \
+        B = t_ % nbatch;                                          \
+        t_ /= nbatch;                                             \
+        CB = t_ % ny;                                             \
+        OD = t_ / ny;                                             \
+    } else {                                                      \
         int t_ = xcd_remap((ID), total);                          \
         CB = t_ % ny;                                             \
         t_ /= ny;                                                 \
-        OW = (t_ % a.tiles_w) * TW;                               \
-        t_ /= a.tiles_w;                                          \
-        MVSGI_DECODE_DH(t_, OD, OH, B)                            \
+        if constexpr (POLY == 2) {                                \
+             \
+            int r_ = t_ % a.bor_n;                                \
+            t_ /= a.bor_n;                                        \
+            int th_, tw_;                                         \
+            if (r_ < 2 * a.tiles_w) {                             \
+                th_ = r_ < a.tiles_w ? 0 : a.tiles_h - 1;         \
+                tw_ = r_ < a.tiles_w ? r_ : r_ - a.tiles_w;       \
+            } else {                                              \
+                r_ -= 2 * a.tiles_w;                              \
+                th_ = 1 + (r_ >> 1);                              \
+                tw_ = (r_ & 1) ? a.tiles_w - 1 : 0;               \
+            }                                                     \
+            OW = tw_ * TW;                                        \
+            OH = th_ * TH;                                        \
+            OD = (t_ % a.tiles_d) * TD + a.od_off;                \
+            B = t_ / a.tiles_d;                                   \
+        } else {                                                  \
+            OW = (t_ % a.tiles_w) * TW;                           \
+            t_ /= a.tiles_w;                                      \
+            MVSGI_DECODE_DH(t_, OD, OH, B)                        \
+        }                                                         \
     }
 
     if (producer) {
@@ -779,6 +813,7 @@
             for (int i = 0; i < MW; ++i) base[i] += kd_lo * (ITH * ITW * kVSB);
         }
         const long long frame_elems = (long long)a.Do * a.Ho * a.Wo * a.Cout;
+#define MVSGI_WSET(OD) (POLY == 1 ? (long long)(a.Do == 1 ? 3 : (OD) == 0 ? 0 : (OD) == a.Do - 1 ? 2 : 1) * a.poly_wset : 0ll)
         int ctc[NW], ctn[NW];
 #define MVSGI_CTILES(DST, CB)                                                         \
         _Pragma("unroll") for (int j = 0; j < NW; ++j) {                              \
@@ -874,7 +909,7 @@
         } else if constexpr (!WLDS) {
             unsigned l16 = lane16;
 #pragma unroll
-            for (int s0 = 0; s0 < LA; ++s0) { MVSGI_LOADWB(wpb + (DKU && od0 == 0 ? 9 * 2048 : 0), s0, 0, s0, ctc) }
+            for (int s0 = 0; s0 < LA; ++s0) { MVSGI_LOADWB(wpb + (DKU && od0 == 0 ? 9 * 2048 : 0) + MVSGI_WSET(od0), s0, 0, s0, ctc) }
         }
         STAMP()
         __syncthreads();
@@ -893,24 +928,45 @@
 #pragma unroll
                 for (int j = 0; j < NW; ++j) ctn[j] = ctc[j];
             }
-            const char* const wpc_ = wpb + (DKU && od0 == 0 ? 9 * 2048 : 0);
-            const char* const wpn_ = wpb + (DKU && nod0 == 0 ? 9 * 2048 : 0);
+            const char* const wpc_ = wpb + (DKU && od0 == 0 ? 9 * 2048 : 0) + MVSGI_WSET(od0);
+            const char* const wpn_ = wpb + (DKU && nod0 == 0 ? 9 * 2048 : 0) + MVSGI_WSET(nod0);
             f32x4 esc[NW], esh[NW], rres[RPRE ? MW : 1][RPRE ? NW : 1];
             int eoff[MW];
             int soff[MW];
             const int ypd = a.ys_2d ? 0 : 1, ypp = a.ys_2d ? 2 : 1;
 #pragma unroll
             for (int j = 0; j < NW; ++j) {
-                esc[j] = *reinterpret_cast<const f32x4*>(a.scale + ctc[j] * 16 + kg * 4);
-                esh[j] = *reinterpret_cast<const f32x4*>(a.shift + ctc[j] * 16 + kg * 4);
-            }
+                const int cs_ = POLY == 1 ? ctc[j] % a.poly_ctp : ctc[j];
+                esc[j] = *reinterpret_cast<const f32x4*>(a.scale + cs_ * 16 + kg * 4);
+                esh[j] = *reinterpret_cast<const f32x4*>(a.shift + cs_ * 16 + kg * 4);
+            }
+            int pe[POLY == 1 ? NW : 1], ps[POLY == 1 ? NW : 1];
+            (void)pe; (void)ps;
             if (last) {
+                if constexpr (POLY == 1) {
+                    const int Cr = a.poly_ctp * 16, Hh = 2 * a.Ho, Wh = 2 * a.Wo;
+#pragma unroll
+                    for (int j = 0; j < NW; ++j) {
+                        const int p_ = ctc[j] / a.poly_ctp, c_ = ctc[j] % a.poly_ctp;
+                        const int pd = p_ >> 2, ph = (p_ >> 1) & 1, pw = p_ & 1;
+                        pe[j] = ((pd * Hh + ph) * Wh + pw) * Cr + c_ * 16;
+                        ps[j] = ((pd * (Hh + 2) + ph) * (Wh + 2) + pw) * Cr * 4 + c_ * 64;
+                    }
+#pragma unroll
+                    for (int i = 0; i < MW; ++i) {
+                        const int od = od0 + tdv[i], oh = oh0 + thv[i], ow = ow0 + twv[i];
+                        const bool inside = od < a.Do && oh < a.poly_oh1 && ow < a.poly_ow1;
+                        eoff[i] = inside ? (((2 * od) * Hh + 2 * oh) * Wh + 2 * ow) * Cr + kg * 4 : -1;
+                        soff[i] = ((((2 * od + 1) * (Hh + 2) + 2 * oh + 1) * (Wh + 2) + 2 * ow + 1) * Cr) * 4 + (kg >> 1) * 16 + (kg & 1) * 8;
+                    }
+                } else {
 #pragma unroll
                 for (int i = 0; i < MW; ++i) {
                     const int od = od0 + tdv[i], oh = oh0 + thv[i], ow = ow0 + twv[i];
                     const bool inside = od < a.Do && oh < a.Ho && ow < a.Wo;
                     eoff[i] = inside ? ((od * a.Ho + oh) * a.Wo + ow) * a.Cout + kg * 4 : -1;
                     soff[i] = ((((od + ypd) * (a.Ho + 2 * ypp) + oh + ypp) * (a.Wo + 2 * ypp) + ow + ypp) * a.Cout) * 4 + (kg >> 1) * 16 + (kg & 1) * 8;
+                }
                 }
             }
             if constexpr (PLANE) {
@@ -972,7 +1028,7 @@
                     for (int i = 0; i < MW; ++i)
 #pragma unroll
                         for (int j = 0; j < NW; ++j)
-                            rres[i][j] = *reinterpret_cast<const f32x4*>(rb + (eoff[i] >= 0 ? eoff[i] + ctc[j] * 16 : 0));
+                            rres[i][j] = *reinterpret_cast<const f32x4*>(rb + (eoff[i] >= 0 ? eoff[i] + (POLY == 1 ? pe[POLY == 1 ? j : 0] : ctc[j] * 16) : 0));
                 }
                 if (s_ < kPairs - ((MVSGI_ABL & 32) ? 1 : 0)) {
                     if (XB >= 2) {
@@ -1030,12 +1086,22 @@
                         if (a.y_split) {
                             u32x2 hi, lo;
                             split_x4<F16>(r, hi, lo, satm);
+                            if constexpr (POLY == 1) {
+                                if (eoff[i] >= 0 && ct0 + j < CT) {
+                                    unsigned char* q = a.y_split + (long long)b_ * ((long long)(2 * a.Do + 2) * (2 * a.Ho + 2) * (2 * a.Wo + 2) * a.poly_ctp * 64) +
+                                                       soff[i] + ps[POLY == 1 ? j : 0];
+                                    *reinterpret_cast<u32x2*>(q) = hi;
+                                    *reinterpret_cast<u32x2*>(q + 32) = lo;
+                                }
+                            } else
                             if (eoff[i] >= 0 && ct0 + j < CT) {
                                 unsigned char* q = a.y_split + (long long)b_ * ((long long)(a.Do + 2 * ypd) * (a.Ho + 2 * ypp) * (a.Wo + 2 * ypp) * a.Cout * 4) +
                                                    soff[i] + (ct0 + j) * 64;
                                 *reinterpret_cast<u32x2*>(q) = hi;
                                 *reinterpret_cast<u32x2*>(q + 32) = lo;
                             }
+                        } else if (POLY == 1) {
+                            if (eoff[i] >= 0 && ct0 + j < CT) *reinterpret_cast<f32x4*>(yb + eoff[i] + pe[POLY == 1 ? j : 0]) = r;
                         } else if (eoff[i] >= 0 && ct0 + j < CT) *reinterpret_cast<f32x4*>(yb + eoff[i] + (ct0 + j) * 16) = r;
                         acc[i][j] = f32x4{0.f, 0.f, 0.f, 0.f};
                         if (TACC) acc1[i][j] = acc2[i][j] = f32x4{0.f, 0.f, 0.f, 0.f};
@@ -1053,6 +1119,7 @@
         }
 #undef MVSGI_T0
 #undef MVSGI_T1
+#undef MVSGI_WSET
 #undef MVSGI_TAP
 #undef MVSGI_PL_LOADW
 #undef MVSGI_PL_READX
@@ -1140,8 +1207,25 @@
     conv3d_x3_body<NW, MW, WM, WN, TD, TH, TW, 1, 3, true, false, false, false, true, true>(a);
 }
 
+template <int NW, int MW, int WM, int WN, int TD, int TH, int TW>
+__global__ __launch_bounds__(512, 2) void conv3d_bf16x3_up2poly_kernel(ConvArgs a) {
+    conv3d_x3_body<NW, MW, WM, WN, TD, TH, TW, 1, 3, false, false, false, false, false, true, 3, 0, 1>(a);
+}
+template <int NW, int MW, int WM, int WN, int TD, int TH, int TW>
+__global__ __launch_bounds__(512, 2) void conv3d_f16x3_up2poly_kernel(ConvArgs a) {
+    conv3d_x3_body<NW, MW, WM, WN, TD, TH, TW, 1, 3, false, false, false, false, true, true, 3, 0, 1>(a);
+}
+template <int NW, int MW, int WM, int WN, int TD, int TH, int TW, bool PLANE>
+__global__ __launch_bounds__(512, 2) void conv3d_bf16x3_up2border_kernel(ConvArgs a) {
+    conv3d_x3_body<NW, MW, WM, WN, TD, TH, TW, 1, 3, true, PLANE, false, false, false, false, 3, 0, 2>(a);
+}
+template <int NW, int MW, int WM, int WN, int TD, int TH, int TW, bool PLANE>
+__global__ __launch_bounds__(512, 2) void conv3d_f16x3_up2border_kernel(ConvArgs a) {
+    conv3d_x3_body<NW, MW, WM, WN, TD, TH, TW, 1, 3, true, PLANE, false, false, true, false, 3, 0, 2>(a);
+}
+
 template <int NW, int MW, int WM, int WN, int TD, int TH, int TW, int S, int KD = 3, bool UPS = false, bool PLANE = false,
-          bool V32 = false, bool WLDS = false, bool F16 = false, bool D32 = false, bool DSK = false, int BRD = 0>
+          bool V32 = false, bool WLDS = false, bool F16 = false, bool D32 = false, bool DSK = false, int BRD = 0, int POLY = 0>
 int launch_bf16x3(ConvArgs a, hipStream_t st) {
     constexpr int ITD = (TD - 1) * (KD == 1 ? 1 : S) + KD, ITH = (TH - 1) * S + 3, ITW = (TW - 1) * S + 3;
     constexpr int ROWP = V32 ? ((ITW * kVSB + 255) / 256) * 256 : ITW * kVSB;
@@ -1154,7 +1238,13 @@
     constexpr bool DKU = DSK && BRD == 3;
     static_assert(!DKU || (TD == 1 && !UPS), "per-unit depth skip: one-plane bricks");
     MVSGI_REQUIRE(!DSK || a.Do == (DKU ? 2 : TD), "conv3d: the depth-skip kernels serve volumes exactly %d planes deep (got %d)", DKU ? 2 : TD, a.Do);
-    if constexpr (DKU && F16) kern = conv3d_f16x3_d32_dk2_kernel<NW, MW, WM, WN, TD, TH, TW>;
+    static_assert(POLY == 0 || (!DSK && BRD == 0 && S == 1 && KD == 3 && !V32 && !WLDS && (POLY == 1 ? D32 && !UPS && !PLANE && TD == 1 : UPS && !D32)),
+                  "the two launches of a fused-upsample layer: a one-plane 32-channel-slice variant | a tap-pair fused-upsample variant");
+    if constexpr (POLY == 1 && F16) kern = conv3d_f16x3_up2poly_kernel<NW, MW, WM, WN, TD, TH, TW>;
+    else if constexpr (POLY == 1) kern = conv3d_bf16x3_up2poly_kernel<NW, MW, WM, WN, TD, TH, TW>;
+    else if constexpr (POLY == 2 && F16) kern = conv3d_f16x3_up2border_kernel<NW, MW, WM, WN, TD, TH, TW, PLANE>;
+    else if constexpr (POLY == 2) kern = conv3d_bf16x3_up2border_kernel<NW, MW, WM, WN, TD, TH, TW, PLANE>;
+    else if constexpr (DKU && F16) kern = conv3d_f16x3_d32_dk2_kernel<NW, MW, WM, WN, TD, TH, TW>;
     else if constexpr (DKU) kern = conv3d_bf16x3_d32_dk2_kernel<NW, MW, WM, WN, TD, TH, TW>;
     else if constexpr (BRD != 0 && UPS && F16) kern = conv3d_f16x3_d32u_brd_kernel<NW, MW, WM, WN, TD, TH, TW, BRD>;
     else if constexpr (BRD != 0 && UPS) kern = conv3d_bf16x3_d32u_brd_kernel<NW, MW, WM, WN, TD, TH, TW, BRD>;
@@ -1174,8 +1264,13 @@
     static mvsgi::PersistentGeom geo_cache[mvsgi::kMaxDevices] = {};
     mvsgi::PersistentGeom geo;
     if (mvsgi::persistent_geometry(kern, 512, lds_bytes, 2, geo_cache, "conv3d(bf16x3)", geo)) return 1;
-    a.tiles_h = (int)mvsgi::cdiv(a.Ho, TH);
-    a.tiles_w = (int)mvsgi::cdiv(a.Wo, TW);
+    a.tiles_h = (int)mvsgi::cdiv(POLY == 1 ? a.poly_oh1 - a.poly_oh0 : a.Ho, TH);
+    a.tiles_w = (int)mvsgi::cdiv(POLY == 1 ? a.poly_ow1 - a.poly_ow0 : a.Wo, TW);
+    MVSGI_REQUIRE(POLY != 1 || (a.poly_ctp > 0 && a.Cout == 8 * 16 * a.poly_ctp && a.poly_oh0 >= 0 && a.poly_oh0 < a.poly_oh1 && a.poly_oh1 <= a.Ho &&
+                                a.poly_ow0 >= 0 && a.poly_ow0 < a.poly_ow1 && a.poly_ow1 <= a.Wo && a.poly_wset > 0),
+                  "conv3d(up2 polyphase): internal: bad interior [%d, %d) x [%d, %d) of %d x %d", a.poly_oh0, a.poly_oh1, a.poly_ow0, a.poly_ow1, a.Ho, a.Wo);
+    MVSGI_REQUIRE(POLY != 2 || (a.tiles_h > 2 && a.tiles_w > 2 && a.bor_n == 2 * a.tiles_w + 2 * (a.tiles_h - 2)),
+                  "conv3d(up2 border): internal: %d border bricks of %d x %d", a.bor_n, a.tiles_h, a.tiles_w);
     const int CT = a.Cout / (V32 ? 32 : 16);
     constexpr bool kBorderSplit = D32 && !DSK && BRD == 0 && TD == 2 && WM == 2 && MW == 4 && TH == 4 && TW == 16 && S == 1;
     if constexpr (kBorderSplit) {
@@ -1190,7 +1285,7 @@
         }
     }
     a.tiles_d = a.od_cnt > 0 ? a.od_cnt : (int)mvsgi::cdiv(a.Do, TD);
-    const long long nb = (long long)a.B * a.tiles_d * a.tiles_h * a.tiles_w * mvsgi::cdiv(CT, WN * NW);
+    const long long nb = (long long)a.B * a.tiles_d * (POLY == 2 ? a.bor_n : a.tiles_h * a.tiles_w) * mvsgi::cdiv(CT, WN * NW);
     MVSGI_REQUIRE(nb < (1ll << 31), "conv3d: too many units");
     MVSGI_REQUIRE((long long)a.Din * a.Hin * a.Win * a.Cin < (1ll << 29), "conv3d: volume too large for 32-bit byte offsets");
     MVSGI_REQUIRE(!UPS || (a.Din % 2 == 0 && a.Hin % 2 == 0 && a.Win % 2 == 0), "conv3d: fused upsample needs even sizes");
diff --git a/mvs_gi_amd/csrc/conv3d_f16.hip b/mvs_gi_amd/csrc/conv3d_f16.hip
--- a/mvs_gi_amd/csrc/conv3d_f16.hip
+++ b/mvs_gi_amd/csrc/conv3d_f16.hip
@@ -24,4 +24,19 @@
     return fail("mvsgi_conv3d_f32: variant %d has no fp16-split form (MVSGI_CONV_F16 goes with MVSGI_CONV_BF16X3 / _C16 / _V32)", variant);
 }
 
+int conv3d_up2_stream_main_f16(const void* args, hipStream_t st) {
+    return launch_bf16x3<2, 4, 1, 4, 1, 4, 16, 1, 3, false, false, false, false, true, true, false, 0, 1>(*static_cast<const ConvArgs*>(args), st);
 }
+int conv3d_up2_stream_border_f16(int variant, const void* args, hipStream_t st) {
+    const ConvArgs& a = *static_cast<const ConvArgs*>(args);
+    switch (variant) {
+        case B3U_N16: return launch_bf16x3<1, 4, 4, 1, 4, 4, 16, 1, 3, true, false, false, false, true, false, false, 0, 2>(a, st);
+        case B3PU_N16: return launch_bf16x3<1, 4, 4, 1, 4, 4, 16, 1, 3, true, true, false, false, true, false, false, 0, 2>(a, st);
+        case B3U_N32: return launch_bf16x3<2, 4, 4, 1, 4, 4, 16, 1, 3, true, false, false, false, true, false, false, 0, 2>(a, st);
+        case B3U_N48: return launch_bf16x3<3, 4, 4, 1, 4, 4, 16, 1, 3, true, false, false, false, true, false, false, 0, 2>(a, st);
+        case B3U_N64: return launch_bf16x3<2, 4, 2, 2, 2, 4, 16, 1, 3, true, false, false, false, true, false, false, 0, 2>(a, st);
+    }
+    return fail("mvsgi_conv3d_up2_stream: variant %d has no border launch", variant);
+}
+
+}
diff --git a/mvs_gi_amd/csrc/conv3d_up2poly.hip b/mvs_gi_amd/csrc/conv3d_up2poly.hip
--- a/mvs_gi_amd/csrc/conv3d_up2poly.hip
+++ b/mvs_gi_amd/csrc/conv3d_up2poly.hip
@@ -39,8 +39,8 @@
     for (int k = 0; k < 3; ++k) d.m[1][k] = a.m[1][k] - b.m[1][k];
     return d;
 }
-void fold(const M3& Md, const M3& Mh, const M3& Mw, const float* w, float* out) {
-    for (int oi = 0; oi < 16 * 32; ++oi) {
+void fold(const M3& Md, const M3& Mh, const M3& Mw, const float* w, float* out, int n_oi = 16 * 32) {
+    for (int oi = 0; oi < n_oi; ++oi) {
         const float* ws = w + (size_t)oi * 27;
         double t1[27], t2[27], t3[27];
         for (int a = 0; a < 3; ++a)
@@ -526,3 +526,64 @@
     const long long rounds = mvsgi::cdiv(mvsgi::cdiv(units, 8), nwalk);
     return 10 * units >= 7 * rounds * 8 * nwalk ? 1 : 0;
 }
+
+namespace {
+
+struct StreamPlanHeader {
+    int magic, Cin, Cout, fmt;
+    long long set_bytes, total;
+    int pad[56];
+};
+static_assert(sizeof(StreamPlanHeader) == mvsgi::kUp2StreamHeaderBytes, "header");
+
+bool stream_dims_ok(int Cin, int Cout) { return Cin > 0 && Cout > 0 && Cin % 32 == 0 && Cout % 16 == 0 && Cin <= 4096 && Cout <= 4096; }
+
+void stream_fold(const float* w, float* out, int Cin, int Cout, int cls) {
+    for (int p = 0; p < 8; ++p)
+        fold(class_matrix(p >> 2, cls), class_matrix((p >> 1) & 1, INT), class_matrix(p & 1, INT), w, out + (size_t)p * Cout * Cin * 27, Cout * Cin);
+}
+
+}
+
+extern "C" size_t mvsgi_conv3d_up2_stream_plan_bytes(int Cin, int Cout) {
+    if (!stream_dims_ok(Cin, Cout)) return 0;
+    return mvsgi::kUp2StreamHeaderBytes + 4 * mvsgi::up2_stream_set_bytes(Cin, Cout);
+}
+
+extern "C" int mvsgi_conv3d_up2_stream_fold(const float* w_oidhw_host, float* out_host, int Cin, int Cout, int cls) {
+    MVSGI_REQUIRE(w_oidhw_host && out_host, "mvsgi_conv3d_up2_stream_fold: null pointer");
+    MVSGI_REQUIRE(stream_dims_ok(Cin, Cout), "mvsgi_conv3d_up2_stream_fold: Cin %d must be a multiple of 32, Cout %d of 16", Cin, Cout);
+    MVSGI_REQUIRE(cls >= 0 && cls <= 3, "mvsgi_conv3d_up2_stream_fold: depth class %d not in [0, 3]", cls);
+    stream_fold(w_oidhw_host, out_host, Cin, Cout, cls);
+    return 0;
+}
+
+extern "C" int mvsgi_conv3d_up2_stream_plan(const float* w_oidhw_host, void* plan_host, int Cin, int Cout, int fmt) {
+    MVSGI_REQUIRE(w_oidhw_host && plan_host, "mvsgi_conv3d_up2_stream_plan: null pointer");
+    MVSGI_REQUIRE(fmt == 0 || fmt == MVSGI_SPLIT_F16, "mvsgi_conv3d_up2_stream_plan: fmt %d not in {0, MVSGI_SPLIT_F16}", fmt);
+    MVSGI_REQUIRE(stream_dims_ok(Cin, Cout), "mvsgi_conv3d_up2_stream_plan: Cin %d must be a multiple of 32, Cout %d of 16", Cin, Cout);
+    const size_t set_bytes = mvsgi::up2_stream_set_bytes(Cin, Cout);
+    StreamPlanHeader h{};
+    h.magic = mvsgi::kUp2StreamMagic;
+    h.Cin = Cin; h.Cout = Cout; h.fmt = fmt;
+    h.set_bytes = (long long)set_bytes;
+    h.total = (long long)(mvsgi::kUp2StreamHeaderBytes + 4 * set_bytes);
+    unsigned char* P = static_cast<unsigned char*>(plan_host);
+    memcpy(P, &h, sizeof(h));
+    const int C8 = 8 * Cout, CT = C8 / 16;
+    std::vector<float> f((size_t)C8 * Cin * 27);
+    for (int cls = 0; cls < 4; ++cls) {
+        stream_fold(w_oidhw_host, f.data(), Cin, Cout, cls);
+        unsigned short* out = reinterpret_cast<unsigned short*>(P + mvsgi::kUp2StreamHeaderBytes + (size_t)cls * set_bytes);
+        for (int cc = 0; cc < Cin / 32; ++cc)
+            for (int ct = 0; ct < CT; ++ct)
+                for (int tap = 0; tap < 27; ++tap)
+                    for (int lane = 0; lane < 64; ++lane) {
+                        const int kg = lane >> 4, co = ct * 16 + (lane & 15), ci = (2 * cc + (kg & 1)) * 16 + (kg >> 1) * 8;
+                        const size_t o = (((((size_t)cc * CT + ct) * 27 + tap) * 2) * 64 + lane) * 8;
+                        for (int j = 0; j < 8; ++j)
+                            sf_split_weight(f[((size_t)co * Cin + ci + j) * 27 + tap], fmt != 0, out[o + j], out[o + 64 * 8 + j]);
+                    }
+    }
+    return 0;
+}
diff --git a/mvs_gi_amd/csrc/conv_common.hpp b/mvs_gi_amd/csrc/conv_common.hpp
--- a/mvs_gi_amd/csrc/conv_common.hpp
+++ b/mvs_gi_amd/csrc/conv_common.hpp
@@ -21,6 +21,8 @@
     int f16;
     int ys_2d;
     unsigned* sat;
+    int poly_ctp, poly_oh0, poly_ow0, poly_oh1, poly_ow1, bor_n;
+    long long poly_wset;
 };
 
 constexpr int kVS = 20;
diff --git a/mvs_gi_amd/dropin/common_modules.py b/mvs_gi_amd/dropin/common_modules.py
--- a/mvs_gi_amd/dropin/common_modules.py
+++ b/mvs_gi_amd/dropin/common_modules.py
@@ -52,6 +52,10 @@
 _D32_OK: Dict[tuple, bool] = {}
 
 
+_USE_UP2_STREAM = os.environ.get("MVSGI_UP2_STREAM", "1") != "0"
+_UP2_STREAM_OK: Dict[tuple, bool] = {}
+
+
 class Packed(NamedTuple):
     wp: Tensor
     scale: object
@@ -171,7 +175,19 @@
     def run_up2_split(self, x_lowres_ndhwc: Tensor, res: Optional[Tensor], out) -> "H.SplitAct":
         _no_inorm(self, "run_up2_split")
         w_layout, wp, scale = self._stream(self._stream_layout(), H.mode_fmt())
+        if self._up2_stream_pays(x_lowres_ndhwc.shape[:4]):
+            plan = self._cached(("up2s", H.mode_fmt()), lambda: self._entry(H.conv3d_up2_stream_plan(self.w, H.mode_fmt())))
+            return H.conv3d_up2_stream(x_lowres_ndhwc, wp, plan.wp, scale, self.shift, res=res, neg_slope=self.neg_slope, out=out, w_layout=w_layout)
         return H.conv3d_up2_out_split(x_lowres_ndhwc, wp, scale, self.shift, out=out, res=res, neg_slope=self.neg_slope, w_layout=w_layout)
+
+    def _up2_stream_pays(self, dims) -> bool:
+        if not (_USE_UP2_STREAM and H.split_mode() and self.stride == 1 and self.cin % 32 == 0 and self.cout % 16 == 0):
+            return False
+        key = (self.cin, self.cout) + tuple(int(d) for d in dims)
+        ok = _UP2_STREAM_OK.get(key)
+        if ok is None:
+            ok = _UP2_STREAM_OK[key] = H.conv3d_up2_stream_pays(key[2], self.cin, self.cout, *key[3:])
+        return ok
 
     def can_fuse_up2(self) -> bool:
         return H.split_mode() and self.stride == 1 and self.cin % 16 == 0 and self.cout % 16 == 0
diff --git a/mvs_gi_amd/hip_ops.py b/mvs_gi_amd/hip_ops.py
--- a/mvs_gi_amd/hip_ops.py
+++ b/mvs_gi_amd/hip_ops.py
@@ -446,6 +446,63 @@
           yp, B, Cin, Dl, Hl, Wl, Cout, float(neg_slope), _stream_ptr(x))
     out.fmt = "f16" if w_layout & CONV_F16 else "bf16"
     return out
+
+
+def conv3d_up2_stream_applies(cin: int, cout: int) -> bool:
+    return bool(_lib.load().mvsgi_conv3d_up2_stream_plan_bytes(int(cin), int(cout)))
+
+
+def conv3d_up2_stream_pays(B: int, cin: int, cout: int, Dl: int, Hl: int, Wl: int) -> bool:
+    return bool(_lib.load().mvsgi_conv3d_up2_stream_pays(int(B), int(cin), int(cout), int(Dl), int(Hl), int(Wl)))
+
+
+def conv3d_up2_stream_plan(w_oidhw: torch.Tensor, fmt: str = "bf16"):
+    lib = _lib.load()
+    Cout, Cin = int(w_oidhw.shape[0]), int(w_oidhw.shape[1])
+    n = lib.mvsgi_conv3d_up2_stream_plan_bytes(Cin, Cout)
+    if tuple(w_oidhw.shape[2:]) != (3, 3, 3) or not n:
+        raise AssertionError(f"conv3d_up2_stream_plan needs a [Cout % 16 == 0, Cin % 32 == 0, 3, 3, 3] weight, got {tuple(w_oidhw.shape)}")
+    wh = w_oidhw.detach().to("cpu", torch.float32).contiguous()
+    unscale = None
+    if fmt == "f16":
+        up, un = _pow2_unscale(wh.abs().amax(dim=(1, 2, 3, 4)))
+        wh = (wh * up.view(-1, 1, 1, 1, 1)).contiguous()
+        unscale = un.to(w_oidhw.device)
+    plan = torch.empty(n, dtype=torch.uint8)
+    _call("mvsgi_conv3d_up2_stream_plan", wh.data_ptr(), plan.data_ptr(), Cin, Cout, _fmt_code(fmt))
+    plan = plan.to(w_oidhw.device)
+    return (plan, unscale) if fmt == "f16" else plan
+
+
+UP2_STREAM_FORMS = {"auto": 0, "main_first": 1, "border_first": 2}
+
+
+def conv3d_up2_stream(x, w_packed_b3, plan, scale, shift, res=None, neg_slope=0.01, out=None, w_layout=CONV_BF16X3, form: str = "auto"):
+    x = _dev(x, "x")
+    B, Dl, Hl, Wl, Cin = x.shape
+    dev = x.device
+    sc, sh, Cout = _scale_shift(scale, shift, dev)
+    shp = (B, 2 * Dl, 2 * Hl, 2 * Wl, Cout)
+    if w_layout & ~CONV_F16 not in (CONV_BF16X3, CONV_BF16X3_C16):
+        raise ValueError(f"conv3d_up2_stream: w_layout {w_layout} is not CONV_BF16X3 / CONV_BF16X3_C16 (| CONV_F16)")
+    if form not in UP2_STREAM_FORMS:
+        raise ValueError(f"conv3d_up2_stream: form {form!r} not in {sorted(UP2_STREAM_FORMS)}")
+    nplan = _lib.load().mvsgi_conv3d_up2_stream_plan_bytes(Cin, Cout)
+    if not nplan:
+        raise AssertionError(f"conv3d_up2_stream: x has {Cin} channels, scale {Cout}: needs Cin % 32 == 0 and Cout % 16 == 0")
+    wp = _arg(w_packed_b3, "w_packed_b3", dev, torch.uint8, nbytes=_split_layout_bytes(w_layout, Cout, Cin))
+    pp = _arg(plan, "plan", dev, torch.uint8, nbytes=nplan).data_ptr()
+    rp = _opt(res, "res", dev, shape=shp)
+    if isinstance(out, SplitAct):
+        yp = _split_ptr(out, "out", dev, shp)
+        _call("mvsgi_conv3d_up2_stream_out_split", x.data_ptr(), wp.data_ptr(), w_layout, pp, sc, sh, rp, yp, B, Cin, Dl, Hl, Wl, Cout,
+              float(neg_slope), UP2_STREAM_FORMS[form], _stream_ptr(x))
+        out.fmt = "f16" if w_layout & CONV_F16 else "bf16"
+        return out
+    y = torch.empty(shp, device=dev, dtype=torch.float32) if out is None else _arg(out, "out", dev, shape=shp)
+    _call("mvsgi_conv3d_up2_stream_f32", x.data_ptr(), wp.data_ptr(), w_layout, pp, sc, sh, rp, y.data_ptr(), B, Cin, Dl, Hl, Wl, Cout,
+          float(neg_slope), UP2_STREAM_FORMS[form], _stream_ptr(x))
+    return y
 
 
 def conv3d_up2_poly_applies(cin: int, cout: int, neg_slope: float) -> bool:
```

Result: no change. 6559, median of 3 (+0.1%).
